# klausondrag/FOSVOS

Measured on AMD Instinct MI355X. Metric: online fine-tune frames/sec (854x480), higher is better.
Workload: dtype bf16; 1 GPU; OSVOS_VGG train_online one-shot fine-tune: 1x3x480x854 frame per step, fwd + class-balanced BCE + bwd, fused SGD step every 5 steps (BASELINE.json configs[1]); batch=1, avg_grad_every_n=5, activations=bf16 NHWC, fp32 accumulate, fp32 master weights, parallelism=single GPU

## Files before the change

fosvos_amd/csrc/common.hpp:

```cpp
#pragma once
#include <hip/hip_runtime.h>
#include <stdarg.h>
#include <algorithm>
#include <stdint.h>
#include <stdio.h>
#include <stdlib.h>
#include <string.h>

#include "../../include/fosvos_hip.h"

namespace fosvos {

extern thread_local char g_err[512];

inline int fail(int code, const char *fmt, ...) __attribute__((format(printf, 2, 3)));
inline int fail(int code, const char *fmt, ...) {
    va_list ap;
    va_start(ap, fmt);
    vsnprintf(g_err, sizeof(g_err), fmt, ap);
    va_end(ap);
    return code;
}

#define FOSVOS_HIP_CHECK(expr)                                                                         \
    do {                                                                                               \
        hipError_t e_ = (expr);                                                                        \
        if (e_ != hipSuccess)                                                                          \
            return ::fosvos::fail(FOSVOS_E_HIP, "%s: %s (%s:%d)", #expr, hipGetErrorString(e_), __FILE__, \
                                  __LINE__);                                                           \
    } while (0)

#define FOSVOS_REQUIRE(cond, code, ...)                    \
    do {                                                   \
        if (!(cond)) return ::fosvos::fail(code, __VA_ARGS__); \
    } while (0)

#define FOSVOS_ENTER(device) FOSVOS_HIP_CHECK(hipSetDevice(device))
extern bool g_prof_on;
void prof_begin(const char *name, hipStream_t st, double flops);
void prof_end();
#define FOSVOS_PROF(name, st, flops)                                        \
    do {                                                                    \
        if (::fosvos::g_prof_on) ::fosvos::prof_begin(name, (hipStream_t)(st), flops); \
    } while (0)
#define FOSVOS_LAUNCH_CHECK()                            \
    do {                                                 \
        if (::fosvos::g_prof_on) ::fosvos::prof_end();   \
        FOSVOS_HIP_CHECK(hipGetLastError());             \
    } while (0)

struct WgradReduceEntry {
    const float *slabs;
    float *dw, *db;
    const float *bias_part;
    int64_t E_real, E_pad;
    int S, S_bias, Co, Cor, accumulate;
    int block_begin, n_blocks;
    int fold_begin, fold_blocks;
};
constexpr int kWgradReduceMax = 20;
struct WgradReduceTable {
    int n;
    WgradReduceEntry e[kWgradReduceMax];
};
int wgrad_impl(const uint16_t *x, const uint16_t *dy, float *dw, float *db, int N, int H, int W, int Ci, int Co,
               int accumulate, void *workspace, size_t workspace_bytes, int device, void *stream,
               WgradReduceTable *reduce, bool alone = false);
int first_wgrad_impl(const float *frame, const uint16_t *dy, float *dw, float *db, int N, int H, int W, int Co,
                     int accumulate, void *workspace, size_t workspace_bytes, int device, void *stream,
                     WgradReduceTable *reduce);
int wgrad_reduce_all(WgradReduceTable *reduce, int device, void *stream);
int wgrad_queue_reduce(const float *slabs, const float *bias_part, float *dw, float *db, int S, int S_bias, int64_t E_real,
                       int64_t E_pad, int Co, int Cor, int accumulate, WgradReduceTable *reduce, int device, void *stream);
struct HeadBwdArgs {
    const float *const *side;
    const int *hs, *ws;
    const float *const *filt, *const *filt1;
    const float *dsn_w, *fuse_w, *d_fused;
    const float *const *d_side_out;
    uint16_t *const *d_side;
    float *d_fuse_w, *d_fuse_b, *d_dsn_w, *d_dsn_b;
    int N, H, W, accumulate;
    void *workspace;
    size_t workspace_bytes;
    int device;
    int filt_uniform;
};
int head_bwd_check(const HeadBwdArgs &a);
int head_bwd_scale(const HeadBwdArgs &a, int s, void *stream);
int head_bwd_finish(const HeadBwdArgs &a, void *stream);

}
constexpr int kFosvosVggEvents = 25, kFosvosResnetEvents = 12;
struct fosvos_ctx {
    uint32_t magic;
    int device;
    hipEvent_t vgg_ev[kFosvosVggEvents];
    hipEvent_t resnet_ev[kFosvosResnetEvents];
    bool buckets_recorded;
};
constexpr uint32_t kFosvosCtxMagic = 0x58544346u;
namespace fosvos {
inline int ctx_check(const fosvos_ctx *ctx, const char *who) {
    FOSVOS_REQUIRE(ctx != nullptr, FOSVOS_E_ARG, "%s: null context (fosvos_ctx_create)", who);
    FOSVOS_REQUIRE(ctx->magic == kFosvosCtxMagic, FOSVOS_E_ARG, "%s: not a live fosvos_ctx", who);
    return FOSVOS_OK;
}

#ifdef FOSVOS_LAB_BUILD
inline const char *lab_env(const char *name) { return getenv(name); }
#else
inline const char *lab_env(const char *) { return nullptr; }
#endif
inline int lab_env_int(const char *name, int dflt) {
    const char *e = lab_env(name);
    return e ? atoi(e) : dflt;
}

bool conv_pp_applicable(int N, int H, int W, int in_ch, int out_ch);
int conv_pp_workgroups();
int conv_pp_forward(const uint16_t *x, const uint16_t *w_packed, const float *bias, uint16_t *y, uint16_t *y_pool, int N,
                    int H, int W, int Cin_pad, int Cout, int Co_pad, bool relu, hipStream_t st,
                    const uint8_t *mask_bits = nullptr);

inline int64_t cdiv(int64_t a, int64_t b) { return (a + b - 1) / b; }
inline int roundup(int a, int b) { return (a + b - 1) / b * b; }

typedef uint16_t bf16_t;
typedef __attribute__((ext_vector_type(8))) __bf16 bf16x8;
typedef __attribute__((ext_vector_type(4))) float f32x4;
typedef __attribute__((ext_vector_type(4))) short s16x4;
typedef unsigned int u32x4 __attribute__((__vector_size__(16)));

__device__ __forceinline__ uint16_t f2bf(float f) {
    __bf16 b = (__bf16)f;
    return __builtin_bit_cast(uint16_t, b);
}
__device__ __forceinline__ float bf2f(uint16_t v) { return __uint_as_float(((uint32_t)v) << 16); }
__device__ __forceinline__ uint4 repack8(const float (&f)[8]) {
    uint4 v;
    v.x = __builtin_amdgcn_perm(__float_as_uint(f[1]), __float_as_uint(f[0]), 0x07060302u);
    v.y = __builtin_amdgcn_perm(__float_as_uint(f[3]), __float_as_uint(f[2]), 0x07060302u);
    v.z = __builtin_amdgcn_perm(__float_as_uint(f[5]), __float_as_uint(f[4]), 0x07060302u);
    v.w = __builtin_amdgcn_perm(__float_as_uint(f[7]), __float_as_uint(f[6]), 0x07060302u);
    return v;
}
typedef float fosvos_f32x2 __attribute__((ext_vector_type(2)));
typedef __bf16 fosvos_bf16x2 __attribute__((ext_vector_type(2)));
__device__ __forceinline__ uint32_t pack2bf(float lo, float hi) {
    const fosvos_f32x2 v = {lo, hi};
    return __builtin_bit_cast(uint32_t, __builtin_convertvector(v, fosvos_bf16x2));
}
__device__ __forceinline__ float relu_f(float v) { return __int_as_float(max(__float_as_int(v), 0)); }
__device__ __forceinline__ void unpack8(const uint4 &v, float (&f)[8]) {
    f[0] = __uint_as_float(v.x << 16);
    f[1] = __uint_as_float(v.x & 0xffff0000u);
    f[2] = __uint_as_float(v.y << 16);
    f[3] = __uint_as_float(v.y & 0xffff0000u);
    f[4] = __uint_as_float(v.z << 16);
    f[5] = __uint_as_float(v.z & 0xffff0000u);
    f[6] = __uint_as_float(v.w << 16);
    f[7] = __uint_as_float(v.w & 0xffff0000u);
}
__device__ __forceinline__ uint4 pack8(const float (&f)[8]) {
    uint4 v;
    v.x = pack2bf(f[0], f[1]);
    v.y = pack2bf(f[2], f[3]);
    v.z = pack2bf(f[4], f[5]);
    v.w = pack2bf(f[6], f[7]);
    return v;
}

typedef short fosvos_i16x2 __attribute__((ext_vector_type(2)));
typedef unsigned short fosvos_u16x2 __attribute__((ext_vector_type(2)));
__device__ __forceinline__ uint32_t keep_where_pos_bf16x2(uint32_t f, uint32_t m) {
    const fosvos_i16x2 zero = {0, 0}, one = {1, 1};
    const fosvos_i16x2 t = __builtin_elementwise_min(
        __builtin_elementwise_max(__builtin_bit_cast(fosvos_i16x2, m), zero), one);
    const fosvos_u16x2 all = {0xffff, 0xffff};
    return f & __builtin_bit_cast(uint32_t, __builtin_bit_cast(fosvos_u16x2, t) * all);
}
__device__ __forceinline__ uint4 keep_where_pos_bf16x8(const uint4 &f, const uint4 &m) {
    return make_uint4(keep_where_pos_bf16x2(f.x, m.x), keep_where_pos_bf16x2(f.y, m.y),
                      keep_where_pos_bf16x2(f.z, m.z), keep_where_pos_bf16x2(f.w, m.w));
}
__device__ __forceinline__ uint32_t max_nonneg_bf16x2(uint32_t a, uint32_t b) {
    return __builtin_bit_cast(uint32_t, __builtin_elementwise_max(__builtin_bit_cast(fosvos_u16x2, a),
                                                                 __builtin_bit_cast(fosvos_u16x2, b)));
}
__device__ __forceinline__ uint4 max_nonneg_bf16x8(const uint4 &a, const uint4 &b) {
    return make_uint4(max_nonneg_bf16x2(a.x, b.x), max_nonneg_bf16x2(a.y, b.y), max_nonneg_bf16x2(a.z, b.z),
                      max_nonneg_bf16x2(a.w, b.w));
}

__device__ __forceinline__ float wave_sum(float v) {
#pragma unroll
    for (int o = 32; o > 0; o >>= 1) v += __shfl_xor(v, o, 64);
    return v;
}
__device__ __forceinline__ double wave_sum(double v) {
#pragma unroll
    for (int o = 32; o > 0; o >>= 1) v += __shfl_xor(v, o, 64);
    return v;
}

}
```

fosvos_amd/csrc/conv_igemm.hip:

```cpp
#include <stdlib.h>

#include "common.hpp"

using namespace fosvos;

namespace {

constexpr unsigned kReluAfterAdd = 0x100u;
constexpr unsigned kSubsample2 = 0x200u;
constexpr unsigned kNoSplitK = 0x400u;

struct ConvArgs {
    const uint16_t *x;
    const uint16_t *w;
    const float *bias;
    const uint16_t *relu_src;
    const uint8_t *relu_bits;
    const uint16_t *addend;
    void *y;
    uint16_t *y_pool;
    const uint16_t *unpool_g;
    int N, H, W, Cin, Cout, Co_pad;
    int tiles_x, tiles_y;
    unsigned flags;
    int swizzle;
    int k_splits;
    int chunks_per_split;
    float *partial;
    unsigned m_ncb, m_nt, m_tx, m_ty;
    int n_t;
#ifdef FOSVOS_STAMP
    unsigned long long *stamps;
#endif
};

#ifdef FOSVOS_STAMP
unsigned long long *g_stamps = nullptr;
#define FOSVOS_STAMP_AT(i)                                                                               \
    if (a.stamps && threadIdx.x == 0)                                                                    \
        a.stamps[((((int64_t)blockIdx.z * gridDim.y + blockIdx.y) * gridDim.x + blockIdx.x) << 4) + (i)] = \
            __builtin_amdgcn_s_memtime();
#define FOSVOS_STAMP_RT(i)                                                                               \
    if (a.stamps && threadIdx.x == 0)                                                                    \
        a.stamps[((((int64_t)blockIdx.z * gridDim.y + blockIdx.y) * gridDim.x + blockIdx.x) << 4) + (i)] = \
            __builtin_amdgcn_s_memrealtime();
#else
#define FOSVOS_STAMP_AT(i)
#define FOSVOS_STAMP_RT(i)
#endif

__device__ __forceinline__ unsigned fast_div(unsigned n, unsigned d, unsigned m) { return m ? __umulhi(n, m) : n / d; }
unsigned recip_mul(int64_t n_max, int64_t d) {
    return (d >= 2 && n_max * d < (int64_t(1) << 32)) ? (unsigned)((int64_t(1) << 32) / d + 1) : 0u;
}

template <int TH_, int TW_, int BN_, int WM_, int WN_>
struct Tile {
    static constexpr int TH = TH_, TW = TW_, BN = BN_, WM = WM_, WN = WN_;
    static constexpr int BM = TH * TW;
    static constexpr int HALO_W = TW + 2, HALO_H = TH + 2;
    static constexpr int NPIX = HALO_W * HALO_H;
    static constexpr int NPIX8 = (NPIX + 7) / 8 * 8;
    static constexpr int NPIX_PAD = (NPIX + 15) / 16 * 16;
    static constexpr int WAVE_M = BM / WM, WAVE_N = BN / WN;
    static constexpr int MF = WAVE_M / 16, NF = WAVE_N / 16;
    static constexpr int A_SLOTS = 4 * NPIX_PAD;
    static constexpr int B_SLOTS = 36 * BN;
    static constexpr int NT = 64 * WM * WN;
    static constexpr int A_IT = (NPIX8 * 4 + NT - 1) / NT;
    static constexpr int B_IT = (B_SLOTS + NT - 1) / NT;
    static constexpr int OUT_LD = BN + 8;
    static constexpr int LDS_MAIN = (A_SLOTS + B_SLOTS) * 16;
    static constexpr int LDS_OUT = BM * OUT_LD * 2;
    static constexpr int LDS_BYTES = LDS_MAIN > LDS_OUT ? LDS_MAIN : LDS_OUT;
#ifndef FOSVOS_MID_WPE
#define FOSVOS_MID_WPE 3
#endif
    static constexpr int WPE = (BM >= 256 || BN < 64) ? 2 : FOSVOS_MID_WPE;
    static_assert(WM * WN == 4 || WM * WN == 8, "4 or 8 waves per workgroup");
    static_assert(TW % 16 == 0 && WAVE_M % 16 == 0 && WAVE_N % 16 == 0, "fragment alignment");
    static_assert(BM % WM == 0 && BN % WN == 0, "wave split");
};

template <int MF, int NF>
struct TapPlan {
    static constexpr int rows_b = MF / 2 > 0 ? MF / 2 : 1;
    static constexpr int per_row = (NF + rows_b - 1) / rows_b;
    static constexpr int nb(int i) {
        const int left = NF - i * per_row;
        return left <= 0 ? 0 : (left < per_row ? left : per_row);
    }
};
template <int MF, int NF, int I, bool NEXT, int V>
__device__ __forceinline__ void sched_row() {
    if constexpr (I < MF) {
        __builtin_amdgcn_sched_group_barrier(0x008, NF, 0);
        if constexpr (NEXT) __builtin_amdgcn_sched_group_barrier(0x100, 1 + TapPlan<MF, NF>::nb(I), 0);
        constexpr int rows_v = V < MF ? V : MF;
        constexpr int nv = I < MF - rows_v ? 0 : (I == MF - 1 ? V - (rows_v - 1) : 1);
        if constexpr (nv > 0) __builtin_amdgcn_sched_group_barrier(0x020, nv, 0);
    }
}
template <int MF, int NF, bool NEXT, int V>
__device__ __forceinline__ void sched_tap() {
    static_assert(MF <= 8, "sched_tap rows");
    sched_row<MF, NF, 0, NEXT, V>(); sched_row<MF, NF, 1, NEXT, V>(); sched_row<MF, NF, 2, NEXT, V>();
    sched_row<MF, NF, 3, NEXT, V>(); sched_row<MF, NF, 4, NEXT, V>(); sched_row<MF, NF, 5, NEXT, V>();
    sched_row<MF, NF, 6, NEXT, V>(); sched_row<MF, NF, 7, NEXT, V>();
}

template <class T, bool OUT_F32, bool UNPOOL = false>
__global__ __launch_bounds__(T::NT) __attribute__((amdgpu_waves_per_eu(2, T::WPE))) void k_conv3x3_igemm(const ConvArgs a) {
    extern __shared__ __attribute__((aligned(16))) uint4 smem[];
    uint4 *sA = smem;
    uint4 *sB = smem + T::A_SLOTS;
#ifdef FOSVOS_IGEMM_PRIO
    __builtin_amdgcn_s_setprio(FOSVOS_IGEMM_PRIO);
#endif

    const int tid = threadIdx.x, lane = tid & 63;
    const int wave = __builtin_amdgcn_readfirstlane(tid >> 6);
    const int wm = wave / T::WN, wn = wave % T::WN;
    int t = blockIdx.x;
    int cb = blockIdx.y;
    if (a.swizzle) {
        const int n_wg = gridDim.x, n_cb = a.Cout / T::BN, n_t = a.n_t;
        const int q8 = n_wg >> 3, r8 = n_wg & 7, xcd = t & 7;
        const int swz = (xcd < r8 ? xcd * (q8 + 1) : r8 * (q8 + 1) + (xcd - r8) * q8) + (t >> 3);
        if (a.swizzle == 1) { t = fast_div(swz, n_cb, a.m_ncb); cb = swz - t * n_cb; }
        else { cb = fast_div(swz, n_t, a.m_nt); t = swz - cb * n_t; }
    }
    const int t_row = fast_div(t, a.tiles_x, a.m_tx);
    const int tx_i = t - t_row * a.tiles_x;
    const int n = fast_div(t_row, a.tiles_y, a.m_ty);
    const int ty_i = t_row - n * a.tiles_y;
    const int y0 = ty_i * T::TH, x0 = tx_i * T::TW;
    const int n0 = cb * T::BN;
    const int H = a.H, W = a.W, Cin = a.Cin;
    const int n_chunks = Cin >> 5;
    const uint16_t *xn = a.x + (int64_t)n * H * W * Cin;

    int a_goff[T::A_IT];
    int a_slot[T::A_IT];
#pragma unroll
    for (int it = 0; it < T::A_IT; ++it) {
        const int idx = it * T::NT + tid;
        const int oct = idx >> 5, within = idx & 31;
        const int kg = within >> 3;
        const int P = oct * 8 + (within & 7);
        a_slot[it] = -1;
        a_goff[it] = -1;
        if (P < T::NPIX) {
            const int hy = P / T::HALO_W, hx = P - hy * T::HALO_W;
            const int gy = y0 + hy - 1, gx = x0 + hx - 1;
            a_slot[it] = kg * T::NPIX_PAD + P;
            if (gy >= 0 && gy < H && gx >= 0 && gx < W) a_goff[it] = ((gy * W + gx) * Cin + kg * 8) * 2;
        }
    }

    f32x4 acc[T::MF][T::NF];
#pragma unroll
    for (int i = 0; i < T::MF; ++i)
#pragma unroll
        for (int j = 0; j < T::NF; ++j) acc[i][j] = f32x4{0.f, 0.f, 0.f, 0.f};

    int a_base[T::MF];
#pragma unroll
    for (int i = 0; i < T::MF; ++i) {
        const int pb = wm * T::WAVE_M + i * 16;
        const int ty = pb / T::TW, tx = pb % T::TW;
        a_base[i] = (lane >> 4) * T::NPIX_PAD + ty * T::HALO_W + tx + (lane & 15);
    }
// ... 138 lines not shown
        return;
    }
    constexpr int VEC_PER_PIX = T::BN / 8;
    constexpr int OUT_N = T::BM * VEC_PER_PIX;
    constexpr int OUT_IT = (OUT_N + T::NT - 1) / T::NT;
    constexpr int PIX_STEP = T::NT / VEC_PER_PIX;
    static_assert(T::NT % VEC_PER_PIX == 0 && PIX_STEP % T::TW == 0, "a thread's output vectors must share a column");
    constexpr int ROW_STEP = PIX_STEP / T::TW;
    const int o_cg = tid % VEC_PER_PIX, o_pix = tid / VEC_PER_PIX;
    const int o_ly = o_pix / T::TW, o_gx = x0 + o_pix % T::TW;
    const int img_bytes = H * W * a.Cout * 2;
    uint16_t *yo = reinterpret_cast<uint16_t *>(a.y);
    int voff[OUT_IT];
#pragma unroll
    for (int it = 0; it < OUT_IT; ++it) {
        const int gy = y0 + o_ly + it * ROW_STEP;
        const bool ok = it * T::NT + tid < OUT_N && gy < H && o_gx < W;
        voff[it] = ok ? ((gy * W + o_gx) * a.Cout + n0 + o_cg * 8) * 2 : -1;
    }
    const bool masked = (a.relu_src || a.relu_bits || a.addend) && !(a.flags & kSubsample2);
    uint4 mk[OUT_IT], ad[OUT_IT];
#pragma unroll
    for (int it = 0; it < OUT_IT; ++it) mk[it] = ad[it] = make_uint4(0, 0, 0, 0);
    if constexpr (UNPOOL) {
        const int OH = (H + 1) >> 1, OW = (W + 1) >> 1;
        auto m_rsrc = __builtin_amdgcn_make_buffer_rsrc(const_cast<uint16_t *>(a.relu_src + (int64_t)n * H * W * a.Cout), 0,
                                                        img_bytes, 0x00020000);
        auto g_rsrc = __builtin_amdgcn_make_buffer_rsrc(const_cast<uint16_t *>(a.unpool_g + (int64_t)n * OH * OW * a.Cout), 0,
                                                        OH * OW * a.Cout * 2, 0x00020000);
#pragma unroll
        for (int it = 0; it < OUT_IT; ++it)
            mk[it] = __builtin_bit_cast(uint4, __builtin_amdgcn_raw_buffer_load_b128(m_rsrc, voff[it], 0, 0));
#pragma unroll
        for (int it = 0; it < OUT_IT; ++it) {
            const int gy = y0 + o_ly + it * ROW_STEP;
            const int goff = voff[it] < 0 ? -1 : (((gy >> 1) * OW + (o_gx >> 1)) * a.Cout + n0 + o_cg * 8) * 2;
            ad[it] = __builtin_bit_cast(uint4, __builtin_amdgcn_raw_buffer_load_b128(g_rsrc, goff, 0, 0));
        }
    } else if (masked && a.relu_bits) {
        auto b_rsrc = __builtin_amdgcn_make_buffer_rsrc(const_cast<uint8_t *>(a.relu_bits + (int64_t)n * H * W * (a.Cout >> 3)), 0,
                                                        img_bytes >> 4, 0x00020000);
#pragma unroll
        for (int it = 0; it < OUT_IT; ++it) {
            const unsigned b = __builtin_amdgcn_raw_buffer_load_b8(b_rsrc, voff[it] < 0 ? -1 : voff[it] >> 4, 0, 0);
            mk[it] = make_uint4((b & 1u) | ((b & 2u) << 15), ((b >> 2) & 1u) | ((b & 8u) << 13), ((b >> 4) & 1u) | ((b & 32u) << 11),
                                ((b >> 6) & 1u) | ((b & 128u) << 9));
        }
        if (a.addend) {
            auto ad_rsrc = __builtin_amdgcn_make_buffer_rsrc(const_cast<uint16_t *>(a.addend + (int64_t)n * H * W * a.Cout), 0,
                                                             img_bytes, 0x00020000);
#pragma unroll
            for (int it = 0; it < OUT_IT; ++it)
                ad[it] = __builtin_bit_cast(uint4, __builtin_amdgcn_raw_buffer_load_b128(ad_rsrc, voff[it], 0, 0));
        }
    } else if (masked) {
        auto m_rsrc = __builtin_amdgcn_make_buffer_rsrc(
            const_cast<uint16_t *>(a.relu_src ? a.relu_src + (int64_t)n * H * W * a.Cout : yo), 0,
            a.relu_src ? img_bytes : 0, 0x00020000);
        auto ad_rsrc = __builtin_amdgcn_make_buffer_rsrc(
            const_cast<uint16_t *>(a.addend ? a.addend + (int64_t)n * H * W * a.Cout : yo), 0,
            a.addend ? img_bytes : 0, 0x00020000);
#pragma unroll
        for (int it = 0; it < OUT_IT; ++it)
            mk[it] = __builtin_bit_cast(uint4, __builtin_amdgcn_raw_buffer_load_b128(m_rsrc, voff[it], 0, 0));
#pragma unroll
        for (int it = 0; it < OUT_IT; ++it)
            ad[it] = __builtin_bit_cast(uint4, __builtin_amdgcn_raw_buffer_load_b128(ad_rsrc, voff[it], 0, 0));
    }
    float4 bias_r[T::NF];
#pragma unroll
    for (int j = 0; j < T::NF; ++j)
        bias_r[j] = a.bias ? *reinterpret_cast<const float4 *>(a.bias + n0 + wn * T::WAVE_N + j * 16 + q * 4)
                           : make_float4(0.f, 0.f, 0.f, 0.f);
    __syncthreads();
    uint16_t *sO = reinterpret_cast<uint16_t *>(smem);
#pragma unroll
    for (int j = 0; j < T::NF; ++j) {
        const int col = wn * T::WAVE_N + j * 16 + q * 4;
        const float4 b = bias_r[j];
#pragma unroll
        for (int i = 0; i < T::MF; ++i) {
            const int pix = wm * T::WAVE_M + i * 16 + cl;
            float v0 = acc[i][j][0] + b.x, v1 = acc[i][j][1] + b.y, v2 = acc[i][j][2] + b.z, v3 = acc[i][j][3] + b.w;
            if (a.flags & FOSVOS_CONV_RELU) {
                v0 = relu_f(v0); v1 = relu_f(v1); v2 = relu_f(v2); v3 = relu_f(v3);
            }
            *reinterpret_cast<uint2 *>(sO + pix * T::OUT_LD + col) = make_uint2(pack2bf(v0, v1), pack2bf(v2, v3));
        }
    }
    if constexpr (UNPOOL) {
        uint16_t *sX = sO + T::BM * T::OUT_LD;
#pragma unroll
        for (int it = 0; it < OUT_IT; ++it)
            if (it * T::NT + tid < OUT_N)
                *reinterpret_cast<uint4 *>(sX + (o_pix + it * PIX_STEP) * T::OUT_LD + o_cg * 8) = mk[it];
    }
    __syncthreads();
    FOSVOS_STAMP_AT(9)
    const uint16_t *s_vec = sO + o_pix * T::OUT_LD + o_cg * 8;
    auto y_rsrc = __builtin_amdgcn_make_buffer_rsrc(yo + (int64_t)n * H * W * a.Cout, 0, img_bytes, 0x00020000);
    if constexpr (UNPOOL) {
        static_assert((T::TW & (T::TW - 1)) == 0 && T::TH % 2 == 0, "window partners are pix ^ 1 and pix ^ TW");
        const uint16_t *sX = sO + T::BM * T::OUT_LD;
        const fosvos_i16x2 one2 = {1, 1}, zero2 = {0, 0};
        const fosvos_i16x2 late_x = (o_pix & 1) ? zero2 : one2;
#pragma unroll
        for (int it = 0; it < OUT_IT; ++it) {
            const int pix = o_pix + it * PIX_STEP;
            if (it * T::NT + tid >= OUT_N) continue;
            const fosvos_i16x2 late_y = (pix & T::TW) ? zero2 : one2;
            const uint4 cv = keep_where_pos_bf16x8(*reinterpret_cast<const uint4 *>(s_vec + it * PIX_STEP * T::OUT_LD), mk[it]);
            const uint4 x1 = *reinterpret_cast<const uint4 *>(sX + (pix ^ 1) * T::OUT_LD + o_cg * 8);
            const uint4 x2 = *reinterpret_cast<const uint4 *>(sX + (pix ^ T::TW) * T::OUT_LD + o_cg * 8);
            const uint4 x3 = *reinterpret_cast<const uint4 *>(sX + (pix ^ T::TW ^ 1) * T::OUT_LD + o_cg * 8);
            auto win = [&](unsigned own_, unsigned p1, unsigned p2, unsigned p3) {
                const fosvos_i16x2 own = __builtin_bit_cast(fosvos_i16x2, own_);
                const fosvos_i16x2 s = (zero2 - own) & (__builtin_bit_cast(fosvos_i16x2, p1) - own - late_x) &
                                       (__builtin_bit_cast(fosvos_i16x2, p2) - own - late_y) &
                                       (__builtin_bit_cast(fosvos_i16x2, p3) - own - late_y);
                return __builtin_bit_cast(unsigned, s >> 15);
            };
            const uint4 routed = make_uint4(ad[it].x & win(mk[it].x, x1.x, x2.x, x3.x), ad[it].y & win(mk[it].y, x1.y, x2.y, x3.y),
                                            ad[it].z & win(mk[it].z, x1.z, x2.z, x3.z), ad[it].w & win(mk[it].w, x1.w, x2.w, x3.w));
            float f[8], r[8];
            unpack8(cv, f);
            unpack8(routed, r);
#pragma unroll
            for (int e = 0; e < 8; ++e) f[e] += r[e];
            __builtin_amdgcn_raw_buffer_store_b128(__builtin_bit_cast(u32x4, pack8(f)), y_rsrc, voff[it], 0, 0);
        }
    } else if (!(a.flags & kSubsample2)) {
        if (masked) {
#pragma unroll
            for (int it = 0; it < OUT_IT; ++it) {
                uint4 v = *reinterpret_cast<const uint4 *>(s_vec + it * PIX_STEP * T::OUT_LD);
                if (a.relu_src || a.relu_bits) v = keep_where_pos_bf16x8(v, mk[it]);
                if (a.addend || (a.flags & kReluAfterAdd)) {
                    float f[8];
                    unpack8(v, f);
                    if (a.addend) {
                        float av[8];
                        unpack8(ad[it], av);
#pragma unroll
                        for (int e = 0; e < 8; ++e) f[e] += av[e];
                    }
                    if (a.flags & kReluAfterAdd) {
#pragma unroll
                        for (int e = 0; e < 8; ++e) f[e] = relu_f(f[e]);
                    }
                    v = pack8(f);
                }
                __builtin_amdgcn_raw_buffer_store_b128(__builtin_bit_cast(u32x4, v), y_rsrc, voff[it], 0, 0);
            }
        } else {
#pragma unroll
            for (int it = 0; it < OUT_IT; ++it)
                __builtin_amdgcn_raw_buffer_store_b128(
                    __builtin_bit_cast(u32x4, *reinterpret_cast<const uint4 *>(s_vec + it * PIX_STEP * T::OUT_LD)), y_rsrc,
                    voff[it], 0, 0);
        }
    } else {
#pragma unroll
        for (int it = 0; it < OUT_IT; ++it) {
            const int gy = y0 + o_ly + it * ROW_STEP;
            if (it * T::NT + tid >= OUT_N || gy >= H || o_gx >= W || ((gy | o_gx) & 1)) continue;
            const int64_t off =
                (((int64_t)n * ((H + 1) >> 1) + (gy >> 1)) * ((W + 1) >> 1) + (o_gx >> 1)) * a.Cout + n0 + o_cg * 8;
            *reinterpret_cast<uint4 *>(yo + off) = *reinterpret_cast<const uint4 *>(s_vec + it * PIX_STEP * T::OUT_LD);
        }
    }
    if (a.y_pool) {
        static_assert(T::TH % 2 == 0 && T::TW % 2 == 0, "pooling windows must not straddle tiles");
        constexpr int PW = T::TW / 2, PN = (T::TH / 2) * PW;
        const int OH = (H + 1) >> 1, OW = (W + 1) >> 1;
        auto p_rsrc = __builtin_amdgcn_make_buffer_rsrc(a.y_pool + (int64_t)n * OH * OW * a.Cout, 0, OH * OW * a.Cout * 2,
                                                        0x00020000);
        for (int idx = tid; idx < PN * VEC_PER_PIX; idx += T::NT) {
            const int pp = idx / VEC_PER_PIX, cg = idx % VEC_PER_PIX;
            const int py = pp / PW, px = pp % PW;
            const int oy = (y0 >> 1) + py, ox = (x0 >> 1) + px;
            if (oy >= OH || ox >= OW) continue;
            const int poff = ((oy * OW + ox) * a.Cout + n0 + cg * 8) * 2;
            if (a.flags & FOSVOS_CONV_RELU) {
                uint4 mx = make_uint4(0, 0, 0, 0);
#pragma unroll
                for (int t = 0; t < 4; ++t) {
                    const int ly = 2 * py + (t >> 1), lx = 2 * px + (t & 1);
                    if (y0 + ly < H && x0 + lx < W)
                        mx = max_nonneg_bf16x8(mx, *reinterpret_cast<const uint4 *>(sO + (ly * T::TW + lx) * T::OUT_LD + cg * 8));
                }
                __builtin_amdgcn_raw_buffer_store_b128(__builtin_bit_cast(u32x4, mx), p_rsrc, poff, 0, 0);
                continue;
            }
            float m[8];
#pragma unroll
            for (int j = 0; j < 8; ++j) m[j] = -INFINITY;
#pragma unroll
            for (int t = 0; t < 4; ++t) {
                const int ly = 2 * py + (t >> 1), lx = 2 * px + (t & 1);
                if (y0 + ly < H && x0 + lx < W) {
                    float f[8];
                    unpack8(*reinterpret_cast<const uint4 *>(sO + (ly * T::TW + lx) * T::OUT_LD + cg * 8), f);
#pragma unroll
                    for (int j = 0; j < 8; ++j) m[j] = f[j] > m[j] ? f[j] : m[j];
                }
            }
            __builtin_amdgcn_raw_buffer_store_b128(__builtin_bit_cast(u32x4, pack8(m)), p_rsrc, poff, 0, 0);
        }
    }
    FOSVOS_STAMP_AT(10)
    FOSVOS_STAMP_RT(12)
}

__global__ __launch_bounds__(256) void k_splitk_epilogue(const ConvArgs a, int64_t total8) {
    const int groups = a.Cout >> 3;
    const int64_t plane = (int64_t)a.N * a.H * a.W * a.Cout;
    for (int64_t i = blockIdx.x * 256LL + threadIdx.x; i < total8; i += (int64_t)gridDim.x * 256) {
        const int g = (int)(i % groups);
        int64_t off = i * 8;
        if (a.flags & kSubsample2) {
            const int Ho = (a.H + 1) >> 1, Wo = (a.W + 1) >> 1;
            int64_t pq = i / groups;
            const int ox = (int)(pq % Wo);
            pq /= Wo;
            const int oy = (int)(pq % Ho), n = (int)(pq / Ho);
            off = (((int64_t)n * a.H + 2 * oy) * a.W + 2 * ox) * a.Cout + g * 8;
        }
        float f[8];
#pragma unroll
        for (int e = 0; e < 8; ++e) f[e] = 0.f;
        for (int z0 = 0; z0 < a.k_splits; z0 += 4) {
            float4 v0[4], v1[4];
#pragma unroll
            for (int j = 0; j < 4; ++j) {
                const int z = min(z0 + j, a.k_splits - 1);
                v0[j] = *reinterpret_cast<const float4 *>(a.partial + z * plane + off);
                v1[j] = *reinterpret_cast<const float4 *>(a.partial + z * plane + off + 4);
            }
#pragma unroll
            for (int j = 0; j < 4; ++j) {
                if (z0 + j < a.k_splits) {
                    f[0] += v0[j].x; f[1] += v0[j].y; f[2] += v0[j].z; f[3] += v0[j].w;
                    f[4] += v1[j].x; f[5] += v1[j].y; f[6] += v1[j].z; f[7] += v1[j].w;
                }
            }
        }
        if (a.bias) {
#pragma unroll
            for (int e = 0; e < 8; ++e) f[e] += a.bias[g * 8 + e];
        }
        if (a.flags & FOSVOS_CONV_RELU) {
#pragma unroll
            for (int e = 0; e < 8; ++e) f[e] = relu_f(f[e]);
        }
        if (a.flags & FOSVOS_CONV_OUT_F32) {
            float *yo = reinterpret_cast<float *>(a.y) + off;
            *reinterpret_cast<float4 *>(yo) = make_float4(f[0], f[1], f[2], f[3]);
            *reinterpret_cast<float4 *>(yo + 4) = make_float4(f[4], f[5], f[6], f[7]);
            continue;
        }
        if (a.relu_src || a.relu_bits || a.addend) {
            uint4 v = pack8(f);
            unpack8(v, f);
            if (a.relu_bits) {
                const unsigned b = a.relu_bits[off >> 3];
#pragma unroll
                for (int e = 0; e < 8; ++e) f[e] = ((b >> e) & 1u) ? f[e] : 0.f;
            }
            if (a.relu_src) {
                float m[8];
                unpack8(*reinterpret_cast<const uint4 *>(a.relu_src + off), m);
#pragma unroll
                for (int e = 0; e < 8; ++e) f[e] = m[e] > 0.f ? f[e] : 0.f;
            }
            if (a.addend) {
                float ad[8];
                unpack8(*reinterpret_cast<const uint4 *>(a.addend + off), ad);
#pragma unroll
                for (int e = 0; e < 8; ++e) f[e] += ad[e];
            }
            if (a.flags & kReluAfterAdd) {
#pragma unroll
                for (int e = 0; e < 8; ++e) f[e] = relu_f(f[e]);
            }
        }
        *reinterpret_cast<uint4 *>(reinterpret_cast<uint16_t *>(a.y) + i * 8) = pack8(f);
    }
}

using TileBig = Tile<8, 32, 64, 4, 1>;
using TileSquare = Tile<16, 16, 64, 4, 1>;
using TileMid = Tile<8, 16, 64, 2, 2>;
using TileSmall = Tile<4, 16, 64, 2, 2>;
using TileSide = Tile<8, 32, 16, 4, 1>;
using TileSideS = Tile<4, 16, 16, 4, 1>;
using TileHalf = Tile<8, 32, 32, 4, 1>;
using TileHalfS = Tile<4, 16, 32, 4, 1>;

enum TileId { kBig, kMid, kSmall, kSide, kSideS, kHalf, kHalfS, kSquare };

struct ConvPlan {
    TileId tile;
    int k_splits, chunks_per_split;
    size_t workspace_bytes;
};

constexpr int kMinBlocks = 512;

ConvPlan make_plan(int N, int H, int W, int in_ch, int out_ch) {
    ConvPlan p{};
    const int n_chunks = roundup(in_ch, 32) / 32;
    const int64_t pixels = (int64_t)N * H * W;
    auto blocks = [&](int th, int tw, int bn) { return cdiv(W, tw) * cdiv(H, th) * N * (int64_t)(out_ch / bn); };
    int64_t nb;
    if (out_ch % 64 == 0) {
        bool big = blocks(8, 32, 64) >= kMinBlocks / 2;
        if (big) {
            const int64_t area_wide = cdiv(H, 8) * 8 * cdiv(W, 32) * 32, area_sq = cdiv(H, 16) * 16 * cdiv(W, 16) * 16;
            static const bool allow_sq = lab_env_int("FOSVOS_NO_SQUARE_TILE", 0) == 0;
            if (allow_sq && area_sq < area_wide) { p.tile = kSquare; nb = blocks(16, 16, 64); }
            else { p.tile = kBig; nb = blocks(8, 32, 64); }
            static const bool one_round = lab_env_int("FOSVOS_MID_ONE_ROUND", 0) != 0;
            if (blocks(8, 16, 64) <= 768 && (one_round ? blocks(8, 32, 64) < kMinBlocks * 3 / 4 : nb < kMinBlocks / 2)) big = false;
        }
        if (!big) { p.tile = kMid; nb = blocks(8, 16, 64); }
    } else if (out_ch == 32) {
        if (pixels >= 256 * 256) { p.tile = kHalf; nb = blocks(8, 32, 32); }
        else { p.tile = kHalfS; nb = blocks(4, 16, 32); }
    } else {
        if (pixels >= 256 * 256) { p.tile = kSide; nb = blocks(8, 32, 16); }
        else { p.tile = kSideS; nb = blocks(4, 16, 16); }
    }
    if (out_ch % 64 == 0) {
        static const char *force = lab_env("FOSVOS_FORCE_TILE");
        if (force && ((atoi(force) >= 0 && atoi(force) <= 2) || atoi(force) == (int)kHalf)) {
            p.tile = (TileId)atoi(force);
            nb = p.tile == kBig ? blocks(8, 32, 64) : p.tile == kMid ? blocks(8, 16, 64)
                 : p.tile == kHalf ? blocks(8, 32, 32) : blocks(4, 16, 64);
        }
    }
    int ks = 1;
    if (nb < kMinBlocks * 3 / 4) {
        ks = (int)cdiv(kMinBlocks / 2, nb);
        if (ks < 2) ks = 1;
        if (ks > n_chunks) ks = n_chunks;
        if (ks > 16) ks = 16;
    }
#ifdef FOSVOS_STAMP
    if (const char *e = lab_env("FOSVOS_FORCE_KS")) ks = atoi(e);
#endif
    p.chunks_per_split = (int)cdiv(n_chunks, ks);
    p.k_splits = (int)cdiv(n_chunks, p.chunks_per_split);
    p.workspace_bytes = p.k_splits > 1 ? (size_t)p.k_splits * pixels * out_ch * sizeof(float) : 0;
    return p;
}

template <class T, bool OUT_F32, bool UNPOOL = false>
int launch(const ConvArgs &a0, const ConvPlan &plan, hipStream_t st, int in_ch) {
    constexpr int LDS = UNPOOL && 2 * T::LDS_OUT > T::LDS_MAIN ? 2 * T::LDS_OUT : T::LDS_BYTES;
    ConvArgs a = a0;
    a.tiles_x = (int)cdiv(a.W, T::TW);
    a.tiles_y = (int)cdiv(a.H, T::TH);
    a.k_splits = plan.k_splits;
    a.chunks_per_split = plan.chunks_per_split;
#ifdef FOSVOS_STAMP
    a.stamps = g_stamps;
#endif
    const int64_t tiles = (int64_t)a.tiles_x * a.tiles_y * a.N;
    FOSVOS_REQUIRE(tiles <= 0x7fffffff && a.Cout % T::BN == 0, FOSVOS_E_SHAPE, "conv3x3: tile grid");
    if constexpr (LDS > 64 * 1024) {
        static bool once[64];
        int dev = 0;
        FOSVOS_HIP_CHECK(hipGetDevice(&dev));
        if (dev >= 0 && dev < 64 && !once[dev]) {
            FOSVOS_HIP_CHECK(hipFuncSetAttribute(reinterpret_cast<const void *>(k_conv3x3_igemm<T, OUT_F32, UNPOOL>),
                                                 hipFuncAttributeMaxDynamicSharedMemorySize, LDS));
            once[dev] = true;
        }
    }
    if (g_prof_on) {
        static char name[80];
        snprintf(name, sizeof(name), "k_conv3x3_igemm<Tile<%d, %d, %d, %d, %d>, %s, %s>", T::TH, T::TW, T::BN, T::WM, T::WN,
                 OUT_F32 ? "true" : "false", UNPOOL ? "true" : "false");
        prof_begin(name, st, 2.0 * a.N * a.H * a.W * 9.0 * in_ch * a.Cout);
    }
    {
        static const int swz_env = lab_env_int("FOSVOS_IGEMM_SWIZZLE", -1);
        const int n_cb = a.Cout / T::BN;
        a.swizzle = swz_env >= 0 ? swz_env : (tiles * n_cb >= 64 ? 1 : 0);
        if (tiles * n_cb > 0x7fffffff) a.swizzle = 0;
    }
    {
        const int64_t n_cb = a.Cout / T::BN, n_wg = tiles * n_cb;
        a.n_t = (int)tiles;
        a.m_ncb = recip_mul(n_wg, n_cb);
        a.m_nt = recip_mul(n_wg, tiles);
        a.m_tx = recip_mul(tiles, a.tiles_x);
        a.m_ty = recip_mul(tiles, a.tiles_y);
    }
    const dim3 grid = a.swizzle ? dim3((unsigned)(tiles * (a.Cout / T::BN)), 1u, (unsigned)plan.k_splits)
                                : dim3((unsigned)tiles, (unsigned)(a.Cout / T::BN), (unsigned)plan.k_splits);
    hipLaunchKernelGGL((k_conv3x3_igemm<T, OUT_F32, UNPOOL>), grid, dim3(T::NT), LDS, st, a);
    FOSVOS_LAUNCH_CHECK();
    if (plan.k_splits > 1) {
        const int64_t total8 = (a.flags & kSubsample2) ? (int64_t)a.N * ((a.H + 1) >> 1) * ((a.W + 1) >> 1) * (a.Cout / 8)
                                                       : (int64_t)a.N * a.H * a.W * (a.Cout / 8);
        int64_t g = cdiv(total8, 256);
        if (g > 4096) g = 4096;
        FOSVOS_PROF("k_splitk_epilogue", st, 0.0);
        hipLaunchKernelGGL(k_splitk_epilogue, dim3((unsigned)g), dim3(256), 0, st, a, total8);
        FOSVOS_LAUNCH_CHECK();
    }
    return FOSVOS_OK;
}

int dispatch(ConvArgs a, int in_ch, void *workspace, size_t workspace_bytes, hipStream_t st) {
    const bool f32 = (a.flags & FOSVOS_CONV_OUT_F32) != 0;
    if (a.Cout == 32) {
        FOSVOS_REQUIRE(!f32, FOSVOS_E_ARG, "conv3x3: fp32 output is only built for 16-channel outputs");
    } else if (a.Cout % 64 != 0) {
        FOSVOS_REQUIRE(a.Cout == 16, FOSVOS_E_SHAPE, "conv3x3: output channels must be 16, 32 or a multiple of 64 (got %d)",
                       a.Cout);
        FOSVOS_REQUIRE(a.relu_src == nullptr && a.addend == nullptr, FOSVOS_E_ARG,
                       "conv3x3: 16-channel output has no mask/add epilogue");
    } else {
        FOSVOS_REQUIRE(!f32, FOSVOS_E_ARG, "conv3x3: fp32 output is only built for 16-channel outputs");
    }
    ConvPlan plan = make_plan(a.N, a.H, a.W, in_ch, a.Cout);
    if (a.flags & kNoSplitK) {
        plan.k_splits = 1;
        plan.chunks_per_split = roundup(in_ch, 32) / 32;
        plan.workspace_bytes = 0;
    }
    if (plan.k_splits > 1) {
        FOSVOS_REQUIRE(workspace && workspace_bytes >= plan.workspace_bytes, FOSVOS_E_WORKSPACE,
                       "conv3x3: split-K needs %zu workspace bytes, got %zu", plan.workspace_bytes, workspace_bytes);
        a.partial = reinterpret_cast<float *>(workspace);
    }
    if (a.unpool_g) {
        switch (plan.tile) {
            case kBig: return launch<TileBig, false, true>(a, plan, st, in_ch);
            case kSquare: return launch<TileSquare, false, true>(a, plan, st, in_ch);
            case kMid: return launch<TileMid, false, true>(a, plan, st, in_ch);
            default: return fail(FOSVOS_E_ARG, "conv3x3: no fused pool backward for this tile");
        }
    }
    switch (plan.tile) {
        case kBig: return launch<TileBig, false>(a, plan, st, in_ch);
        case kSquare: return launch<TileSquare, false>(a, plan, st, in_ch);
        case kMid: return launch<TileMid, false>(a, plan, st, in_ch);
        case kSmall: return launch<TileSmall, false>(a, plan, st, in_ch);
        case kSide: return f32 ? launch<TileSide, true>(a, plan, st, in_ch) : launch<TileSide, false>(a, plan, st, in_ch);
        case kSideS: return f32 ? launch<TileSideS, true>(a, plan, st, in_ch) : launch<TileSideS, false>(a, plan, st, in_ch);
        case kHalf: return launch<TileHalf, false>(a, plan, st, in_ch);
        case kHalfS: return launch<TileHalfS, false>(a, plan, st, in_ch);
    }
    return fail(FOSVOS_E_ARG, "conv3x3: bad plan");
}

bool forward_takes_pp(int N, int H, int W, int in_ch, int out_ch, unsigned flags) {
    if (flags & ~FOSVOS_CONV_RELU) return false;
    static const int mode = lab_env_int("FOSVOS_PP", -1);
    if (mode == 0) return false;
    return conv_pp_applicable(N, H, W, roundup(in_ch, 32), out_ch);
}

int check_common(const void *x, const void *w, const void *y, int N, int H, int W, int in_ch, int out_ch,
                 const char *who) {
    FOSVOS_REQUIRE(x && w && y, FOSVOS_E_ARG, "%s: null pointer", who);
    FOSVOS_REQUIRE(N > 0 && H > 0 && W > 0 && in_ch > 0 && out_ch > 0, FOSVOS_E_SHAPE, "%s: bad shape N=%d H=%d W=%d in=%d out=%d",
                   who, N, H, W, in_ch, out_ch);
    FOSVOS_REQUIRE(out_ch % 16 == 0, FOSVOS_E_SHAPE, "%s: output channels %d not a multiple of 16", who, out_ch);
    FOSVOS_REQUIRE((int64_t)H * W * roundup(in_ch, 32) * 2 < 0x7fffffffLL && (int64_t)H * W * out_ch * 4 < 0x7fffffffLL,
                   FOSVOS_E_SHAPE, "%s: one image exceeds 2^31 bytes", who);
    return FOSVOS_OK;
}
}

extern "C" size_t fosvos_conv3x3_workspace_bytes(int N, int H, int W, int in_ch, int out_ch) {
    if (N <= 0 || H <= 0 || W <= 0 || in_ch <= 0 || out_ch <= 0 || (out_ch % 64 != 0 && out_ch != 16)) return 0;
    return make_plan(N, H, W, in_ch, out_ch).workspace_bytes;
}

extern "C" int fosvos_conv3x3_plan(int N, int H, int W, int in_ch, int out_ch, fosvos_conv3x3_plan_info *out) {
    FOSVOS_REQUIRE(out, FOSVOS_E_ARG, "conv3x3_plan: null output");
    FOSVOS_REQUIRE(N > 0 && H > 0 && W > 0 && in_ch > 0 && out_ch > 0 && (out_ch % 64 == 0 || out_ch == 32 || out_ch == 16),
                   FOSVOS_E_SHAPE, "conv3x3_plan: bad shape N=%d H=%d W=%d in=%d out=%d", N, H, W, in_ch, out_ch);
    const ConvPlan p = make_plan(N, H, W, in_ch, out_ch);
    int th = 0, tw = 0, bn = 0;
    switch (p.tile) {
        case kBig: th = TileBig::TH; tw = TileBig::TW; bn = TileBig::BN; break;
        case kSquare: th = TileSquare::TH; tw = TileSquare::TW; bn = TileSquare::BN; break;
        case kMid: th = TileMid::TH; tw = TileMid::TW; bn = TileMid::BN; break;
        case kSmall: th = TileSmall::TH; tw = TileSmall::TW; bn = TileSmall::BN; break;
        case kSide: th = TileSide::TH; tw = TileSide::TW; bn = TileSide::BN; break;
        case kSideS: th = TileSideS::TH; tw = TileSideS::TW; bn = TileSideS::BN; break;
        case kHalf: th = TileHalf::TH; tw = TileHalf::TW; bn = TileHalf::BN; break;
        case kHalfS: th = TileHalfS::TH; tw = TileHalfS::TW; bn = TileHalfS::BN; break;
    }
    out->tile_h = th; out->tile_w = tw; out->tile_co = bn;
    out->k_splits = p.k_splits;
    out->workgroups = (int)(cdiv(W, tw) * cdiv(H, th) * N * (out_ch / bn));
    out->persistent = 0;
    return FOSVOS_OK;
}

extern "C" int fosvos_conv3x3_fwd_plan(int N, int H, int W, int in_ch, int out_ch, unsigned flags,
                                       fosvos_conv3x3_plan_info *out) {
    if (int rc = fosvos_conv3x3_plan(N, H, W, in_ch, out_ch, out)) return rc;
    if (out_ch % 64 == 0 && forward_takes_pp(N, H, W, in_ch, out_ch, flags)) {
        out->tile_h = 8; out->tile_w = 32; out->tile_co = 64;
        out->k_splits = 1;
        out->workgroups = conv_pp_workgroups();
        out->persistent = 1;
    }
    return FOSVOS_OK;
}

extern "C" int fosvos_conv3x3_fwd(const uint16_t *x, const uint16_t *w_packed, const float *bias, void *y, int N, int H,
                                  int W, int Ci, int Co, unsigned flags, void *workspace, size_t workspace_bytes,
                                  int device, void *stream) {
    if (int rc = check_common(x, w_packed, y, N, H, W, Ci, Co, "conv3x3_fwd")) return rc;
    FOSVOS_REQUIRE((flags & ~(FOSVOS_CONV_RELU | FOSVOS_CONV_OUT_F32)) == 0, FOSVOS_E_ARG, "conv3x3_fwd: unknown flags 0x%x", flags);
    FOSVOS_ENTER(device);
    if (Co % 64 == 0 && forward_takes_pp(N, H, W, Ci, Co, flags))
        return conv_pp_forward(x, w_packed, bias, (uint16_t *)y, nullptr, N, H, W, roundup(Ci, 32), Co, roundup(Co, 16),
                               (flags & FOSVOS_CONV_RELU) != 0, (hipStream_t)stream);
    ConvArgs a{};
    a.x = x; a.w = w_packed; a.bias = bias; a.relu_src = nullptr; a.addend = nullptr; a.y = y;
    a.N = N; a.H = H; a.W = W; a.Cin = roundup(Ci, 32); a.Cout = Co; a.Co_pad = roundup(Co, 16); a.flags = flags;
    return dispatch(a, Ci, workspace, workspace_bytes, (hipStream_t)stream);
}

extern "C" int fosvos_conv3x3_fwd_add(const uint16_t *x, const uint16_t *w_packed, const float *bias,
                                      const uint16_t *addend, void *y, int N, int H, int W, int Ci, int Co,
                                      unsigned flags, void *workspace, size_t workspace_bytes, int device,
                                      void *stream) {
    if (int rc = check_common(x, w_packed, y, N, H, W, Ci, Co, "conv3x3_fwd_add")) return rc;
    FOSVOS_REQUIRE((flags & ~(FOSVOS_CONV_RELU | FOSVOS_CONV_OUT_F32)) == 0, FOSVOS_E_ARG, "conv3x3_fwd_add: unknown flags 0x%x",
                   flags);
    FOSVOS_REQUIRE(Co % 64 == 0 || Co == 32 || (Co == 16 && !addend), FOSVOS_E_SHAPE,
                   "conv3x3_fwd_add: Co=%d must be 32 or a multiple of 64 (16 without an addend)", Co);
    FOSVOS_REQUIRE(!(flags & FOSVOS_CONV_OUT_F32) || (Co == 16 && !addend), FOSVOS_E_ARG,
                   "conv3x3_fwd_add: fp32 output is the 16-channel side_prep form");
    FOSVOS_ENTER(device);
    ConvArgs a{};
    a.x = x; a.w = w_packed; a.bias = bias; a.relu_src = nullptr; a.addend = addend; a.y = y;
    a.N = N; a.H = H; a.W = W; a.Cin = roundup(Ci, 32); a.Cout = Co; a.Co_pad = roundup(Co, 16);
    a.flags = kNoSplitK | (addend ? ((flags & FOSVOS_CONV_RELU) ? kReluAfterAdd : 0u) : flags);
    return dispatch(a, Ci, workspace, workspace_bytes, (hipStream_t)stream);
}

extern "C" int fosvos_conv3x3_s2_fwd(const uint16_t *x, const uint16_t *w_packed, const float *bias, uint16_t *y, int N,
                                     int H, int W, int Ci, int Co, unsigned flags, void *workspace, size_t workspace_bytes,
                                     int device, void *stream) {
    if (int rc = check_common(x, w_packed, y, N, H, W, Ci, Co, "conv3x3_s2_fwd")) return rc;
    FOSVOS_REQUIRE((flags & ~FOSVOS_CONV_RELU) == 0, FOSVOS_E_ARG, "conv3x3_s2_fwd: unknown flags 0x%x", flags);
    FOSVOS_REQUIRE(Co % 64 == 0 || Co == 32, FOSVOS_E_SHAPE, "conv3x3_s2_fwd: Co=%d must be 32 or a multiple of 64", Co);
    FOSVOS_ENTER(device);
    ConvArgs a{};
    a.x = x; a.w = w_packed; a.bias = bias; a.relu_src = nullptr; a.addend = nullptr; a.y = y;
    a.N = N; a.H = H; a.W = W; a.Cin = roundup(Ci, 32); a.Cout = Co; a.Co_pad = roundup(Co, 16);
    a.flags = flags | kSubsample2 | kNoSplitK;
    return dispatch(a, Ci, workspace, workspace_bytes, (hipStream_t)stream);
}

extern "C" int fosvos_conv3x3_fwd_pool(const uint16_t *x, const uint16_t *w_packed, const float *bias, uint16_t *y,
                                       uint16_t *y_pool, int N, int H, int W, int Ci, int Co, unsigned flags,
                                       void *workspace, size_t workspace_bytes, int device, void *stream) {
    if (int rc = check_common(x, w_packed, y, N, H, W, Ci, Co, "conv3x3_fwd_pool")) return rc;
    FOSVOS_REQUIRE(y_pool, FOSVOS_E_ARG, "conv3x3_fwd_pool: null pooled output");
    FOSVOS_REQUIRE((flags & ~FOSVOS_CONV_RELU) == 0, FOSVOS_E_ARG, "conv3x3_fwd_pool: unknown flags 0x%x", flags);
    FOSVOS_REQUIRE(Co % 64 == 0, FOSVOS_E_SHAPE, "conv3x3_fwd_pool: Co=%d must be a multiple of 64", Co);
    if ((flags & FOSVOS_CONV_RELU) && forward_takes_pp(N, H, W, Ci, Co, flags)) {
        FOSVOS_ENTER(device);
        return conv_pp_forward(x, w_packed, bias, y, y_pool, N, H, W, roundup(Ci, 32), Co, roundup(Co, 16), true,
                               (hipStream_t)stream);
    }
    if (make_plan(N, H, W, Ci, Co).k_splits > 1) {
        if (int rc = fosvos_conv3x3_fwd(x, w_packed, bias, y, N, H, W, Ci, Co, flags, workspace, workspace_bytes, device, stream))
            return rc;
        return fosvos_maxpool2x2_ceil_fwd(y, y_pool, N, H, W, Co, device, stream);
    }
    FOSVOS_ENTER(device);
    ConvArgs a{};
    a.x = x; a.w = w_packed; a.bias = bias; a.relu_src = nullptr; a.addend = nullptr; a.y = y; a.y_pool = y_pool;
    a.N = N; a.H = H; a.W = W; a.Cin = roundup(Ci, 32); a.Cout = Co; a.Co_pad = roundup(Co, 16); a.flags = flags;
    return dispatch(a, Ci, workspace, workspace_bytes, (hipStream_t)stream);
}

extern "C" int fosvos_conv3x3_dgrad_bits(const uint16_t *dy, const uint16_t *w_dgrad_packed, const uint8_t *relu_bits,
                                         const uint16_t *addend, uint16_t *dx, int N, int H, int W, int Ci, int Co,
                                         void *workspace, size_t workspace_bytes, int device, void *stream) {
    if (int rc = check_common(dy, w_dgrad_packed, dx, N, H, W, Co, Ci, "conv3x3_dgrad_bits")) return rc;
    FOSVOS_REQUIRE(relu_bits && Ci % 8 == 0, FOSVOS_E_ARG, "conv3x3_dgrad_bits: null mask or Ci=%d not a multiple of 8", Ci);
    FOSVOS_ENTER(device);
    if (!addend && lab_env_int("FOSVOS_PP_DGRAD", 1) != 0 && lab_env_int("FOSVOS_PP", -1) != 0 &&
        conv_pp_applicable(N, H, W, roundup(Co, 32), Ci))
        return conv_pp_forward(dy, w_dgrad_packed, nullptr, dx, nullptr, N, H, W, roundup(Co, 32), Ci, roundup(Ci, 16), false,
                               (hipStream_t)stream, relu_bits);
    ConvArgs a{};
    a.x = dy; a.w = w_dgrad_packed; a.bias = nullptr; a.relu_src = nullptr; a.relu_bits = relu_bits; a.addend = addend; a.y = dx;
    a.N = N; a.H = H; a.W = W; a.Cin = roundup(Co, 32); a.Cout = Ci; a.Co_pad = roundup(Ci, 16); a.flags = 0;
    return dispatch(a, Co, workspace, workspace_bytes, (hipStream_t)stream);
}

extern "C" int fosvos_conv3x3_dgrad_unpool(const uint16_t *dy, const uint16_t *w_dgrad_packed, const uint16_t *x,
                                           const uint16_t *d_pooled, uint16_t *dx, int N, int H, int W, int Ci, int Co,
                                           void *workspace, size_t workspace_bytes, int device, void *stream) {
    if (int rc = check_common(dy, w_dgrad_packed, dx, N, H, W, Co, Ci, "conv3x3_dgrad_unpool")) return rc;
    FOSVOS_REQUIRE(x && d_pooled && x != dx, FOSVOS_E_ARG, "conv3x3_dgrad_unpool: null or aliased pooled-map operands");
    FOSVOS_ENTER(device);
    const ConvPlan plan = make_plan(N, H, W, Co, Ci);
    const bool fused = Ci % 64 == 0 && plan.k_splits == 1 && (plan.tile == kBig || plan.tile == kSquare || plan.tile == kMid) &&
                       lab_env_int("FOSVOS_UNPOOL_FUSED", 1) != 0;
    if (!fused) {
        if (int rc = fosvos_maxpool2x2_ceil_bwd(x, d_pooled, dx, N, H, W, Ci, 1, device, stream)) return rc;
        return fosvos_conv3x3_dgrad(dy, w_dgrad_packed, x, dx, dx, N, H, W, Ci, Co, workspace, workspace_bytes, device, stream);
    }
    ConvArgs a{};
    a.x = dy; a.w = w_dgrad_packed; a.relu_src = x; a.unpool_g = d_pooled; a.y = dx;
    a.N = N; a.H = H; a.W = W; a.Cin = roundup(Co, 32); a.Cout = Ci; a.Co_pad = roundup(Ci, 16); a.flags = 0;
    return dispatch(a, Co, workspace, workspace_bytes, (hipStream_t)stream);
}

extern "C" int fosvos_conv3x3_dgrad(const uint16_t *dy, const uint16_t *w_dgrad_packed, const uint16_t *relu_src,
                                    const uint16_t *addend, uint16_t *dx, int N, int H, int W, int Ci, int Co,
                                    void *workspace, size_t workspace_bytes, int device, void *stream) {
    if (int rc = check_common(dy, w_dgrad_packed, dx, N, H, W, Co, Ci, "conv3x3_dgrad")) return rc;
    FOSVOS_ENTER(device);
    ConvArgs a{};
    a.x = dy; a.w = w_dgrad_packed; a.bias = nullptr; a.relu_src = relu_src; a.addend = addend; a.y = dx;
    a.N = N; a.H = H; a.W = W; a.Cin = roundup(Co, 32); a.Cout = Ci; a.Co_pad = roundup(Ci, 16); a.flags = 0;
    return dispatch(a, Co, workspace, workspace_bytes, (hipStream_t)stream);
}
```

fosvos_amd/csrc/conv_pp.hip:

```cpp
#include <stdlib.h>

#include "common.hpp"

using namespace fosvos;

namespace fosvos {
namespace pp {

constexpr int TH = 8, TW = 32, BN = 64;
constexpr int HALO_W = TW + 2, HALO_H = TH + 2, NPIX = HALO_W * HALO_H;
constexpr int A_BYTES = NPIX * 64;
constexpr int A_PIECES = (NPIX * 4 + 63) / 64;
constexpr int W_BYTES = 36 * BN * 16;
constexpr int LDS_W = 0, LDS_A = 2 * W_BYTES, LDS_BIAS = LDS_A + 4 * A_BYTES, LDS_BYTES = LDS_BIAS + BN * 4;
constexpr int NT = 512;
static_assert(LDS_BYTES <= 160 * 1024, "one workgroup per CU");

struct Args {
    const uint16_t *x;
    const uint16_t *w;
    const float *bias;
    uint16_t *y;
    uint16_t *y_pool;
    const uint8_t *mask_bits;
    int N, H, W, Cin, Cout, Co_pad;
    int tiles_x, tiles_y, n_tiles;
    int n_cb;
    unsigned long long *stamps;
    int lab;
};
#ifdef FOSVOS_LAB_BUILD
#define PP_LAB(bit) (a.lab & (bit))
#define PP_STAMP(idx_)                                                                                            \
    if (a.stamps && blockIdx.x < 8 && wm == 0 && lane == 0 && (idx_) < 512)                                       \
        a.stamps[(blockIdx.x * 2 + g) * 512 + (idx_)] = __builtin_amdgcn_s_memtime();
#else
#define PP_LAB(bit) 0
#define PP_STAMP(idx_)
#endif

#pragma clang diagnostic push
#pragma clang diagnostic ignored "-Winline-asm"
__device__ __forceinline__ void dma16(const __amdgpu_buffer_rsrc_t rsrc, unsigned lds_dst, unsigned voff, unsigned soff) {
    asm volatile("s_mov_b32 m0, %0\n\ts_nop 4\n\tbuffer_load_dwordx4 %1, %2, %3 offen lds"
                 :: "s"(lds_dst), "v"(voff), "s"(rsrc), "s"(soff) : "memory", "m0");
}
__device__ __forceinline__ void wait_vm0() { asm volatile("s_waitcnt vmcnt(0)" ::: "memory"); }
__device__ __forceinline__ void wait_all() { asm volatile("s_waitcnt vmcnt(0) lgkmcnt(0)" ::: "memory"); }
__device__ __forceinline__ void pp_barrier() {
    asm volatile("" ::: "memory");
    __builtin_amdgcn_s_barrier();
    asm volatile("" ::: "memory");
}
#pragma clang diagnostic pop

typedef __attribute__((address_space(3))) void lds_void;
typedef __attribute__((address_space(3))) const uint4 *lds_u4_ptr;

struct TileIt {
    int idx, n, ty, tx;
    int d_n, d_ty, d_tx, stride;
    int tiles_x, tiles_y, end;
    __device__ __forceinline__ void init(int first, int stride_, int tiles_x_, int tiles_y_, int end_) {
        tiles_x = tiles_x_; tiles_y = tiles_y_; end = end_; stride = stride_;
        idx = first;
        const int per_img = tiles_x * tiles_y;
        n = first / per_img;
        const int r = first - n * per_img;
        ty = r / tiles_x;
        tx = r - ty * tiles_x;
        d_n = stride / per_img;
        const int rs = stride - d_n * per_img;
        d_ty = rs / tiles_x;
        d_tx = rs - d_ty * tiles_x;
    }
    __device__ __forceinline__ void next() {
        idx += stride;
        tx += d_tx;
        const int cx = tx >= tiles_x;
        tx -= cx ? tiles_x : 0;
        ty += d_ty + cx;
        const int cy = ty >= tiles_y;
        ty -= cy ? tiles_y : 0;
        n += d_n + cy;
    }
    __device__ __forceinline__ bool valid() const { return idx < end; }
    __device__ __forceinline__ int y0() const { return ty * TH; }
    __device__ __forceinline__ int x0() const { return tx * TW; }
};

template <bool RELU, bool POOL, bool MASK = false>
__global__ __launch_bounds__(NT) __attribute__((amdgpu_waves_per_eu(2, 2))) void k_conv3x3_pp(const Args a) {
    extern __shared__ __attribute__((aligned(16))) char smem_pp[];
    const unsigned lds0 = __builtin_amdgcn_readfirstlane((unsigned)(size_t)(lds_void *)smem_pp);
    const int tid = threadIdx.x, lane = tid & 63;
    const int wave = __builtin_amdgcn_readfirstlane(tid >> 6);
    const int g = wave >> 2, wm = wave & 3;
    const int cl = lane & 15, kq = lane >> 4;
    const int H = a.H, W = a.W, Cin = a.Cin, Cout = a.Cout;
    const int NC = Cin >> 5;

    const int b = blockIdx.x, n_wg8 = gridDim.x >> 3;
    const int xcd = b & 7, j8 = b >> 3;
    const int cb = j8 % a.n_cb, jj = j8 / a.n_cb, S = n_wg8 / a.n_cb;
    const int t_begin = (int)(((int64_t)xcd * a.n_tiles) >> 3), t_end = (int)(((int64_t)(xcd + 1) * a.n_tiles) >> 3);
    const int span = t_end - t_begin;
    const int n_it = span > 2 * jj ? (span - 2 * jj + 2 * S - 1) / (2 * S) : 0;
    if (n_it == 0) return;
    const int K = n_it * NC;
    const int n0 = cb * BN;
    TileIt cur, ldt;
    cur.init(t_begin + 2 * jj + g, 2 * S, a.tiles_x, a.tiles_y, t_end);
    ldt = cur;

    const int pj = lane >> 4, pm = lane & 15;
    const unsigned w_voff = (unsigned)(32 * (pj >> 1) + 8 * (pm >> 2) + 4 * (pj & 1) + (pm & 3)) * 16u;
    const int w_row_bytes = a.Co_pad * 16;
    const auto w_rsrc = __builtin_amdgcn_make_buffer_rsrc(const_cast<uint16_t *>(a.w), 0, NC * 36 * w_row_bytes, 0x00020000);
    auto issue_w = [&](int chunk, int buf, int first, int stride) {
        if (PP_LAB(8)) return;
        for (int r = first; r < 36; r += stride)
            dma16(w_rsrc, lds0 + LDS_W + buf * W_BYTES + r * 1024, w_voff, (unsigned)((chunk * 36 + r) * w_row_bytes + n0 * 16));
    };

    constexpr int A_IT = (A_PIECES + 3) / 4;
    int a_rel[A_IT];
#pragma unroll
    for (int i = 0; i < A_IT; ++i) {
        const int pc = wm + 4 * i;
        const int P = pc * 16 + (lane >> 2), s4 = lane & 3;
        const int hy = P / HALO_W, hx = P - hy * HALO_W;
        const int kq_src = s4 ^ ((P >> 1) & 2);
        a_rel[i] = (hy * W + hx) * Cin * 2 + kq_src * 16;
    }
    int ld_k = 0, ld_c = 0;
    int ld_base = 0, ld_edge = 0;
    __amdgpu_buffer_rsrc_t ld_rsrc;
    auto ld_open_tile = [&]() {
        if (!ldt.valid()) return;
        const int y0 = ldt.y0(), x0 = ldt.x0();
        ld_rsrc = __builtin_amdgcn_make_buffer_rsrc(const_cast<uint16_t *>(a.x) + (int64_t)ldt.n * H * W * Cin, 0,
                                                    H * W * Cin * 2, 0x00020000);
        ld_base = ((y0 - 1) * W + (x0 - 1)) * Cin * 2;
        ld_edge = !(y0 > 0 && x0 > 0 && y0 + TH < H && x0 + TW < W);
    };
    auto ld_issue = [&]() {
        if (ld_k < K && ldt.valid() && !PP_LAB(4)) {
            const unsigned dst = lds0 + LDS_A + (g * 2 + (ld_k & 1)) * A_BYTES;
            constexpr int LAST_LANES = NPIX * 4 - (A_PIECES - 1) * 64;
            if (!ld_edge) {
                const unsigned soff = (unsigned)(ld_base + ld_c * 64);
#pragma unroll
                for (int i = 0; i < A_IT; ++i) {
                    const int pc = wm + 4 * i;
                    if (pc < A_PIECES - 1) dma16(ld_rsrc, dst + pc * 1024, (unsigned)a_rel[i], soff);
                    else if (pc == A_PIECES - 1 && lane < LAST_LANES) dma16(ld_rsrc, dst + pc * 1024, (unsigned)a_rel[i], soff);
                }
            } else {
                const int y0 = ldt.y0(), x0 = ldt.x0();
#pragma unroll
                for (int i = 0; i < A_IT; ++i) {
                    const int pc = wm + 4 * i;
                    const int P = pc * 16 + (lane >> 2);
                    const int hy = P / HALO_W, hx = P - hy * HALO_W;
                    const int gy = y0 + hy - 1, gx = x0 + hx - 1;
                    const bool ok = (unsigned)gy < (unsigned)H && (unsigned)gx < (unsigned)W;
                    const unsigned voff = ok ? (unsigned)(ld_base + a_rel[i]) : 0x80000000u;
                    if (pc < A_PIECES - 1) dma16(ld_rsrc, dst + pc * 1024, voff, (unsigned)(ld_c * 64));
                    else if (pc == A_PIECES - 1 && lane < LAST_LANES) dma16(ld_rsrc, dst + pc * 1024, voff, (unsigned)(ld_c * 64));
                }
            }
        }
        ++ld_k;
        if (++ld_c == NC) {
            ld_c = 0;
            ldt.next();
            if (ld_k < K) ld_open_tile();
        }
    };

    unsigned a_sw[4][3];
#pragma unroll
    for (int rr = 0; rr < 4; ++rr)
#pragma unroll
        for (int kx = 0; kx < 3; ++kx) {
            const int P = (2 * wm + rr) * HALO_W + kx + cl;
            a_sw[rr][kx] = (unsigned)(P * 64 + ((kq ^ ((P >> 1) & 2)) << 4));
        }
    const unsigned w_frag0 = lds0 + LDS_W + kq * 1024 + cl * 16;

    if (tid < BN) *(__attribute__((address_space(3))) float *)(size_t)(lds0 + LDS_BIAS + tid * 4) = a.bias ? a.bias[n0 + tid] : 0.f;
    const unsigned bias_at = lds0 + LDS_BIAS + kq * 32;

    f32x4 acc[4][4];
    int cp_c = 0;
    bf16x8 af[4], wf[2][4];
#define PP_RA(k_, tap_, i_)                                                                                   \
    af[i_] = __builtin_bit_cast(bf16x8, *(lds_u4_ptr)(size_t)(lds0 + LDS_A + (g * 2 + ((k_) & 1)) * A_BYTES +  \
                                                              a_sw[((i_) >> 1) + (tap_) / 3][(tap_) % 3] + ((i_) & 1) * 1024));
#define PP_RW(k_, tap_, s_, j_) \
    wf[s_][j_] = __builtin_bit_cast(bf16x8, *(lds_u4_ptr)(size_t)(w_frag0 + ((k_) & 1) * W_BYTES + (tap_) * 4096 + (j_) * 256));
#define PP_RBIAS()                                                                                            \
    _Pragma("unroll") for (int i = 0; i < 4; ++i) _Pragma("unroll") for (int j = 0; j < 4; ++j) acc[i][j] =    \
        *(__attribute__((address_space(3))) const f32x4 *)(size_t)(bias_at + (j >> 1) * 128 + (j & 1) * 16);

    uint4 pk[4][2];
    unsigned mb[MASK ? 4 : 1][2];
    int dn_n = 0, dn_y0 = 0, dn_x0 = 0;
    int st_pending = 0;
    auto pack_frag = [&](int i, int jp) {
        unsigned u[4];
#pragma unroll
        for (int e2 = 0; e2 < 4; ++e2) {
            const int e = 2 * e2;
            u[e2] = pack2bf(acc[i][2 * jp + (e >> 2)][e & 3], acc[i][2 * jp + (e >> 2)][(e & 3) + 1]);
            if constexpr (RELU) {
                const fosvos_i16x2 zero = {0, 0};
                u[e2] = __builtin_bit_cast(unsigned, __builtin_elementwise_max(__builtin_bit_cast(fosvos_i16x2, u[e2]), zero));
            }
        }
        return make_uint4(u[0], u[1], u[2], u[3]);
    };
    auto pack_tile = [&]() {
        if (!cur.valid() || PP_LAB(2)) return;
        dn_n = cur.n; dn_y0 = cur.y0(); dn_x0 = cur.x0();
        st_pending = 1;
#pragma unroll
        for (int i = 0; i < 4; ++i) {
            pk[i][0] = pack_frag(i, 0);
            pk[i][1] = pack_frag(i, 1);
        }
        if constexpr (MASK) {
            const auto m_rsrc = __builtin_amdgcn_make_buffer_rsrc(const_cast<uint8_t *>(a.mask_bits) + (int64_t)dn_n * H * W * (Cout >> 3),
                                                                  0, H * W * (Cout >> 3), 0x00020000);
#pragma unroll
            for (int i = 0; i < 4; ++i) {
                const int gy = dn_y0 + 2 * wm + (i >> 1), gx = dn_x0 + (i & 1) * 16 + cl;
                const unsigned off = (gy < H && gx < W) ? (unsigned)((gy * W + gx) * (Cout >> 3) + (n0 >> 3) + kq) : 0x80000000u;
                mb[i][0] = __builtin_amdgcn_raw_buffer_load_b8(m_rsrc, off, 0, 0);
                mb[i][1] = __builtin_amdgcn_raw_buffer_load_b8(m_rsrc, off + 4, 0, 0);
            }
        }
    };
    auto mask_bits_of = [](unsigned b) {
        return make_uint4((b & 1u) | ((b & 2u) << 15), ((b >> 2) & 1u) | ((b & 8u) << 13), ((b >> 4) & 1u) | ((b & 32u) << 11),
                          ((b >> 6) & 1u) | ((b & 128u) << 9));
    };
    auto store_slot = [&](int slot) {
        if (!st_pending) return;
        if (slot < 4) {
            const auto y_rsrc = __builtin_amdgcn_make_buffer_rsrc(a.y + (int64_t)dn_n * H * W * Cout, 0, H * W * Cout * 2, 0x00020000);
            const int gy = dn_y0 + 2 * wm + (slot >> 1), gx = dn_x0 + (slot & 1) * 16 + cl;
            const unsigned off = (gy < H && gx < W) ? (unsigned)(((gy * W + gx) * Cout + n0 + kq * 8) * 2) : 0x80000000u;
            uint4 v0 = pk[slot][0], v1 = pk[slot][1];
            if constexpr (MASK) {
                v0 = keep_where_pos_bf16x8(v0, mask_bits_of(mb[slot][0]));
                v1 = keep_where_pos_bf16x8(v1, mask_bits_of(mb[slot][1]));
            }
            __builtin_amdgcn_raw_buffer_store_b128(__builtin_bit_cast(u32x4, v0), y_rsrc, off, 0, 0);
            __builtin_amdgcn_raw_buffer_store_b128(__builtin_bit_cast(u32x4, v1), y_rsrc, off + 64, 0, 0);
        } else if constexpr (POOL) {
            const int ih = slot - 4;
            const int OH = (H + 1) >> 1, OW = (W + 1) >> 1;
            const bool edge = dn_y0 + TH > H || dn_x0 + TW > W;
            const auto p_rsrc = __builtin_amdgcn_make_buffer_rsrc(a.y_pool + (int64_t)dn_n * OH * OW * Cout, 0,
                                                                  OH * OW * Cout * 2, 0x00020000);
            const int oy = (dn_y0 >> 1) + wm, ox = (dn_x0 >> 1) + ih * 8 + (cl >> 1);
            const bool ok = !(cl & 1) && oy < OH && ox < OW;
            const unsigned off = ok ? (unsigned)(((oy * OW + ox) * Cout + n0 + kq * 8) * 2) : 0x80000000u;
#pragma unroll
            for (int jp = 0; jp < 2; ++jp) {
                uint4 top = pk[ih][jp], bot = pk[ih + 2][jp];
                if (edge) {
                    const int gy = dn_y0 + 2 * wm, gx = dn_x0 + ih * 16 + cl;
                    if (!(gy < H && gx < W)) top = make_uint4(0, 0, 0, 0);
                    if (!(gy + 1 < H && gx < W)) bot = make_uint4(0, 0, 0, 0);
                }
                const uint4 m = max_nonneg_bf16x8(top, bot);
                uint4 o;
                o.x = (unsigned)__builtin_amdgcn_update_dpp(0, (int)m.x, 0xB1, 0xF, 0xF, true);
                o.y = (unsigned)__builtin_amdgcn_update_dpp(0, (int)m.y, 0xB1, 0xF, 0xF, true);
                o.z = (unsigned)__builtin_amdgcn_update_dpp(0, (int)m.z, 0xB1, 0xF, 0xF, true);
                o.w = (unsigned)__builtin_amdgcn_update_dpp(0, (int)m.w, 0xB1, 0xF, 0xF, true);
                __builtin_amdgcn_raw_buffer_store_b128(__builtin_bit_cast(u32x4, max_nonneg_bf16x8(m, o)), p_rsrc, off + jp * 64, 0, 0);
            }
        }
    };
    constexpr int N_SLOTS = POOL ? 6 : 4;

    auto request_next = [&](int k) {
        if (k + 1 < K && (NC > 2 || k + 1 < 2)) issue_w((k + 1) % NC, (k + 1) & 1, wave, 8);
        ld_issue();
    };

    issue_w(0, 0, wave, 8);
    ld_open_tile();
    ld_issue();
    wait_all();
    pp_barrier();

#define PP_MM(tap_, i_, j_) \
    acc[i_][j_] = __builtin_amdgcn_mfma_f32_16x16x32_bf16(wf[(tap_) & 1][j_], af[i_], acc[i_][j_], 0, 0, 0);
#define PP_ROW_READS(n_, i_)                                                                                  \
    PP_RA(k, n_, i_)                                                                                          \
    if constexpr ((i_) < 2) {                                                                                 \
        PP_RW(k, n_, (n_) & 1, 2 * (i_))                                                                      \
        PP_RW(k, n_, (n_) & 1, 2 * (i_) + 1)                                                                  \
    }                                                                                                         \
    __builtin_amdgcn_sched_group_barrier(0x008, 4, 0);                                                        \
    __builtin_amdgcn_sched_group_barrier(0x002, 1, 0);                                                        \
    __builtin_amdgcn_sched_group_barrier(0x100, (i_) < 2 ? 3 : 1, 0);
#define PP_ROW(tap_, i_)                                                                                      \
    PP_MM(tap_, i_, 0) PP_MM(tap_, i_, 1) PP_MM(tap_, i_, 2) PP_MM(tap_, i_, 3)                               \
    PP_ROW_READS((tap_) + 1, i_)
#define PP_TAP(tap_) { PP_ROW(tap_, 0) PP_ROW(tap_, 1) PP_ROW(tap_, 2) PP_ROW(tap_, 3) }
#define PP_TAP_LAST()                                                                                         \
    {                                                                                                         \
        _Pragma("unroll") for (int i = 0; i < 4; ++i) _Pragma("unroll") for (int j = 0; j < 4; ++j) acc[i][j] = \
            __builtin_amdgcn_mfma_f32_16x16x32_bf16(wf[0][j], af[i], acc[i][j], 0, 0, 0);                      \
        __builtin_amdgcn_sched_group_barrier(0x008, 16, 0);                                                   \
    }
#define PP_BETWEEN(tap_)                                                                                      \
    if (g == 0) {                                                                                             \
        if constexpr ((tap_) >= 3 && (tap_) - 3 < N_SLOTS) store_slot((tap_) - 3);                            \
    } else {                                                                                                  \
        if constexpr ((tap_) < 3) {                                                                           \
            store_slot(2 * (tap_));                                                                           \
            if constexpr (2 * (tap_) + 1 < N_SLOTS) store_slot(2 * (tap_) + 1);                               \
        }                                                                                                     \
        if constexpr ((tap_) == 4) request_next(k);                                                           \
    }

    for (int k = 0; k < K; ++k) {
        PP_STAMP(4 * k)
        if (g == 0) request_next(k);
        PP_STAMP(4 * k + 1)
        if (cur.valid() && !PP_LAB(1)) {
            if (cp_c == 0) { PP_RBIAS() }
            PP_RA(k, 0, 0) PP_RA(k, 0, 1) PP_RA(k, 0, 2) PP_RA(k, 0, 3)
            PP_RW(k, 0, 0, 0) PP_RW(k, 0, 0, 1) PP_RW(k, 0, 0, 2) PP_RW(k, 0, 0, 3)
            PP_TAP(0) PP_BETWEEN(0) PP_TAP(1) PP_BETWEEN(1) PP_TAP(2) PP_BETWEEN(2) PP_TAP(3) PP_BETWEEN(3) PP_TAP(4) PP_BETWEEN(4)
            PP_TAP(5) PP_BETWEEN(5) PP_TAP(6) PP_BETWEEN(6) PP_TAP(7) PP_BETWEEN(7) PP_TAP_LAST() PP_BETWEEN(8)
        } else {
            PP_BETWEEN(0) PP_BETWEEN(1) PP_BETWEEN(2) PP_BETWEEN(3) PP_BETWEEN(4) PP_BETWEEN(5) PP_BETWEEN(6) PP_BETWEEN(7) PP_BETWEEN(8)
        }
        st_pending = 0;
        if (++cp_c == NC) {
            cp_c = 0;
            pack_tile();
            cur.next();
        }
        PP_STAMP(4 * k + 2)
        wait_vm0();
        PP_STAMP(4 * k + 3)
        pp_barrier();
    }
    PP_STAMP(4 * K)
#pragma unroll
    for (int slot = 0; slot < N_SLOTS; ++slot) store_slot(slot);
#undef PP_MM
#undef PP_ROW_READS
#undef PP_ROW
#undef PP_TAP
#undef PP_TAP_LAST
#undef PP_BETWEEN
#undef PP_RA
#undef PP_RW
#undef PP_RBIAS
}

}
}

namespace fosvos {
int conv_pp_workgroups() { return 256; }
#ifdef FOSVOS_LAB_BUILD
static unsigned long long *g_pp_stamps = nullptr;
extern "C" void fosvos_lab_set_pp_stamps(void *p) { g_pp_stamps = (unsigned long long *)p; }
#endif

bool conv_pp_applicable(int N, int H, int W, int in_ch, int out_ch) {
    if (out_ch % 64 != 0 || in_ch % 32 != 0) return false;
    const int n_cb = out_ch / 64;
    if (n_cb != 1 && n_cb != 2 && n_cb != 4 && n_cb != 8) return false;
    const int64_t tiles = cdiv(W, pp::TW) * cdiv(H, pp::TH) * N;
    if (tiles > 0x3fffffff) return false;
    const int64_t units = tiles * n_cb, slots = 2 * conv_pp_workgroups();
    if (units < slots) return false;
    static const int mode = lab_env_int("FOSVOS_PP", -1);
    if (mode == 1 || in_ch <= 64) return true;
    return units * 10 >= cdiv(units, slots) * slots * 9;
}



int conv_pp_forward(const uint16_t *x, const uint16_t *w_packed, const float *bias, uint16_t *y, uint16_t *y_pool, int N,
                    int H, int W, int Cin_pad, int Cout, int Co_pad, bool relu, hipStream_t st, const uint8_t *mask_bits) {
    FOSVOS_REQUIRE(!y_pool || relu, FOSVOS_E_ARG, "conv3x3 (persistent): the fused pool takes post-ReLU values");
    FOSVOS_REQUIRE(!mask_bits || (!relu && !y_pool && !bias), FOSVOS_E_ARG, "conv3x3 (persistent): the bit mask is the data gradient's epilogue");
    pp::Args a{};
    a.x = x; a.w = w_packed; a.bias = bias; a.y = y; a.y_pool = y_pool; a.mask_bits = mask_bits;
    a.N = N; a.H = H; a.W = W; a.Cin = Cin_pad; a.Cout = Cout; a.Co_pad = Co_pad;
    a.tiles_x = (int)cdiv(W, pp::TW);
    a.tiles_y = (int)cdiv(H, pp::TH);
    a.n_tiles = a.tiles_x * a.tiles_y * N;
    a.n_cb = Cout / 64;
    a.lab = lab_env_int("FOSVOS_PP_LAB", 0);
#ifdef FOSVOS_LAB_BUILD
    a.stamps = g_pp_stamps;
#endif
    void (*kern)(const pp::Args) = mask_bits ? pp::k_conv3x3_pp<false, false, true>
                                   : y_pool  ? pp::k_conv3x3_pp<true, true>
                                   : relu    ? pp::k_conv3x3_pp<true, false> : pp::k_conv3x3_pp<false, false>;
    const int which = mask_bits ? 3 : y_pool ? 2 : relu ? 1 : 0;
    static bool once[64][4];
    int dev = 0;
    FOSVOS_HIP_CHECK(hipGetDevice(&dev));
    if (dev >= 0 && dev < 64 && !once[dev][which]) {
        FOSVOS_HIP_CHECK(hipFuncSetAttribute(reinterpret_cast<const void *>(kern), hipFuncAttributeMaxDynamicSharedMemorySize,
                                             pp::LDS_BYTES));
        once[dev][which] = true;
    }
    FOSVOS_PROF(mask_bits ? "k_conv3x3_pp<false, false, true>" : y_pool ? "k_conv3x3_pp<true, true, false>"
                : relu    ? "k_conv3x3_pp<true, false, false>" : "k_conv3x3_pp<false, false, false>", st,
                2.0 * N * H * W * 9.0 * Cin_pad * Cout);
    hipLaunchKernelGGL(kern, dim3(conv_pp_workgroups()), dim3(pp::NT), pp::LDS_BYTES, st, a);
    FOSVOS_LAUNCH_CHECK();
    return FOSVOS_OK;
}

}
```

fosvos_amd/csrc/vgg_net.hip:

```cpp
#include <stdlib.h>

#include "common.hpp"

using namespace fosvos;

namespace {
constexpr int kNConv = 13;
constexpr int kStageOf[kNConv] = {0, 0, 1, 1, 2, 2, 2, 3, 3, 3, 4, 4, 4};
constexpr int kCin[kNConv] = {3, 64, 64, 128, 128, 256, 256, 256, 512, 512, 512, 512, 512};
constexpr int kCout[kNConv] = {64, 64, 128, 128, 256, 256, 256, 512, 512, 512, 512, 512, 512};
constexpr int kFirstOfStage[5] = {0, 2, 4, 7, 10};
constexpr int kLastOfStage[5] = {1, 3, 6, 9, 12};
constexpr int kStageCh[5] = {64, 128, 256, 512, 512};

inline size_t up256(size_t v) { return (v + 255) / 256 * 256; }

struct Arena {
    int sh[5], sw[5];
    size_t act[kNConv];
    size_t gact[kNConv];
    size_t pooled[4];
    size_t gpooled[4];
    size_t side[4];
    size_t dside[4];
    size_t bits0;
    size_t ws, ws_bytes;
    size_t hws, hws_bytes;
    size_t wsa_conv[kNConv], wsa_conv_bytes[kNConv], wsa_side[4], wsa_side_bytes[4];
    size_t total;
};

Arena make_arena(int N, int H, int W) {
    Arena a{};
    a.sh[0] = H; a.sw[0] = W;
    for (int s = 1; s < 5; ++s) { a.sh[s] = (a.sh[s - 1] + 1) / 2; a.sw[s] = (a.sw[s - 1] + 1) / 2; }
    size_t off = 0;
    auto take = [&](size_t bytes) { const size_t o = off; off += up256(bytes); return o; };
    for (int c = 0; c < kNConv; ++c) {
        const int s = kStageOf[c];
        const size_t bytes = (size_t)N * a.sh[s] * a.sw[s] * kCout[c] * 2;
        a.act[c] = take(bytes);
        a.gact[c] = take(bytes);
    }
    for (int s = 1; s < 5; ++s) {
        const size_t bytes = (size_t)N * a.sh[s] * a.sw[s] * kStageCh[s - 1] * 2;
        a.pooled[s - 1] = take(bytes);
        a.gpooled[s - 1] = take(bytes);
        a.side[s - 1] = take((size_t)N * a.sh[s] * a.sw[s] * 16 * 4);
        a.dside[s - 1] = take((size_t)N * a.sh[s] * a.sw[s] * 32 * 2);
    }
    a.bits0 = take((size_t)N * H * W * (kCout[0] / 8));
    a.hws_bytes = up256(fosvos_head_bwd_workspace_bytes(N, H, W));
    a.hws = take(a.hws_bytes);
    size_t ws = 256;
    a.wsa_conv_bytes[0] = up256(fosvos_conv3x3_first_wgrad_workspace_bytes(N, H, W, 64));
    for (int c = 1; c < kNConv; ++c) {
        const int s = kStageOf[c];
        a.wsa_conv_bytes[c] = fosvos_conv3x3_wgrad_workspace_bytes(N, a.sh[s], a.sw[s], kCin[c], kCout[c]);
        if (N >= 2)
            a.wsa_conv_bytes[c] = std::max(a.wsa_conv_bytes[c],
                                           fosvos_conv3x3_workspace_bytes(N - (N + 1) / 2, a.sh[s], a.sw[s], kCin[c], kCout[c]));
        a.wsa_conv_bytes[c] = up256(a.wsa_conv_bytes[c]);
        ws = std::max(ws, fosvos_conv3x3_workspace_bytes(N, a.sh[s], a.sw[s], kCin[c], kCout[c]));
        if (N >= 2)
            ws = std::max(ws, fosvos_conv3x3_workspace_bytes((N + 1) / 2, a.sh[s], a.sw[s], kCin[c], kCout[c]));
        ws = std::max(ws, fosvos_conv3x3_workspace_bytes(N, a.sh[s], a.sw[s], kCout[c], kCin[c]));
    }
    for (int s = 1; s < 5; ++s) {
        a.wsa_side_bytes[s - 1] = up256(std::max({fosvos_conv3x3_wgrad_workspace_bytes(N, a.sh[s], a.sw[s], kStageCh[s], 16),
                                                  fosvos_conv3x3_workspace_bytes(N, a.sh[s], a.sw[s], kStageCh[s], 16),
                                                  N >= 2 ? fosvos_conv3x3_workspace_bytes(N - (N + 1) / 2, a.sh[s], a.sw[s], kStageCh[s], 16) : (size_t)0}));
        ws = std::max(ws, fosvos_conv3x3_workspace_bytes(N, a.sh[s], a.sw[s], kStageCh[s], 16));
        if (N >= 2) ws = std::max(ws, fosvos_conv3x3_workspace_bytes((N + 1) / 2, a.sh[s], a.sw[s], kStageCh[s], 16));
        ws = std::max(ws, fosvos_conv3x3_workspace_bytes(N, a.sh[s], a.sw[s], 16, kStageCh[s]));
    }
    a.ws_bytes = up256(ws);
    a.ws = take(a.ws_bytes);
    for (int c = 0; c < kNConv; ++c) a.wsa_conv[c] = take(a.wsa_conv_bytes[c]);
    for (int i = 0; i < 4; ++i) a.wsa_side[i] = take(a.wsa_side_bytes[i]);
    a.total = off;
    return a;
}

static_assert(kFosvosVggEvents == 25, "event slots below");
constexpr int kBucketFinalEvent = 22;
constexpr int kStage2WgradEvent = 23;
constexpr int kMainTailEvent = 24;
constexpr int kBucketEvent0 = 19;

#define FOSVOS_TRY(expr)          \
    do {                          \
        const int rc_ = (expr);   \
        if (rc_ != FOSVOS_OK) return rc_; \
    } while (0)

int check_net(const void *w, const void *frame, const void *arena, int N, int H, int W, size_t arena_bytes,
              const Arena &a, const char *who) {
    FOSVOS_REQUIRE(w && frame && arena, FOSVOS_E_ARG, "%s: null pointer", who);
    FOSVOS_REQUIRE(N > 0 && H > 0 && W > 0, FOSVOS_E_SHAPE, "%s: bad shape N=%d H=%d W=%d", who, N, H, W);
    FOSVOS_REQUIRE(arena_bytes >= a.total, FOSVOS_E_WORKSPACE, "%s: arena %zu < %zu bytes", who, arena_bytes, a.total);
    FOSVOS_REQUIRE(((uintptr_t)arena & 255) == 0, FOSVOS_E_ARG, "%s: arena must be 256-byte aligned", who);
    return FOSVOS_OK;
}
}

extern "C" size_t fosvos_vgg_arena_bytes(int N, int H, int W) {
    if (N <= 0 || H <= 0 || W <= 0) return 0;
    return make_arena(N, H, W).total;
}

extern "C" int fosvos_vgg_arena_layout(int N, int H, int W, fosvos_vgg_arena_layout_info *out) {
    FOSVOS_REQUIRE(out, FOSVOS_E_ARG, "vgg_arena_layout: null output");
    FOSVOS_REQUIRE(N > 0 && H > 0 && W > 0, FOSVOS_E_SHAPE, "vgg_arena_layout: bad shape N=%d H=%d W=%d", N, H, W);
    const Arena a = make_arena(N, H, W);
    *out = fosvos_vgg_arena_layout_info{};
    out->total = a.total;
    for (int s = 0; s < 5; ++s) { out->stage_h[s] = a.sh[s]; out->stage_w[s] = a.sw[s]; }
    for (int c = 0; c < kNConv; ++c) {
        const int s = kStageOf[c];
        out->act[c] = a.act[c];
        out->gact[c] = a.gact[c];
        out->act_bytes[c] = (size_t)N * a.sh[s] * a.sw[s] * kCout[c] * 2;
        out->wsa_conv[c] = a.wsa_conv[c];
        out->wsa_conv_bytes[c] = a.wsa_conv_bytes[c];
    }
    for (int s = 1; s < 5; ++s) {
        const size_t px = (size_t)N * a.sh[s] * a.sw[s];
        out->pooled[s - 1] = a.pooled[s - 1];
        out->gpooled[s - 1] = a.gpooled[s - 1];
        out->pooled_bytes[s - 1] = px * kStageCh[s - 1] * 2;
        out->side[s - 1] = a.side[s - 1];
        out->side_bytes[s - 1] = px * 16 * 4;
        out->dside[s - 1] = a.dside[s - 1];
        out->dside_bytes[s - 1] = px * 32 * 2;
        out->wsa_side[s - 1] = a.wsa_side[s - 1];
        out->wsa_side_bytes[s - 1] = a.wsa_side_bytes[s - 1];
    }
    out->bits0 = a.bits0;
    out->bits0_bytes = (size_t)N * H * W * (kCout[0] / 8);
    out->ws = a.ws; out->ws_bytes = a.ws_bytes;
    out->hws = a.hws; out->hws_bytes = a.hws_bytes;
    return FOSVOS_OK;
}

namespace {
int forward_impl(hipEvent_t *ev, const fosvos_vgg_weights *w, const float *frame, int N, int H, int W, void *arena,
                 size_t arena_bytes, float *fused, float *const side_out[4], int device, void *stream, void *aux_stream) {
    const Arena a = make_arena(N, H, W);
    FOSVOS_TRY(check_net(w, frame, arena, N, H, W, arena_bytes, a, "vgg_forward"));
    FOSVOS_REQUIRE(fused, FOSVOS_E_ARG, "vgg_forward: null output");
    char *base = reinterpret_cast<char *>(arena);
    auto act = [&](int c) { return reinterpret_cast<uint16_t *>(base + a.act[c]); };
    void *ws = base + a.ws;
    hipStream_t sm = (hipStream_t)stream;
    const bool par = ev != nullptr && aux_stream != nullptr && aux_stream != stream;
    hipStream_t sa = par ? (hipStream_t)aux_stream : sm;
    if (par) FOSVOS_ENTER(device);
    static const bool split_on = lab_env_int("FOSVOS_FWD_SPLIT", 1) != 0;
    if (split_on && N >= 2) {
        const int na = (N + 1) / 2;
        if (par) {
            FOSVOS_HIP_CHECK(hipEventRecord(ev[14], sm));
            FOSVOS_HIP_CHECK(hipStreamWaitEvent(sa, ev[14], 0));
        }
        for (int half = 0; half < 2; ++half) {
            const int f0 = half ? na : 0, nf = half ? N - na : na;
            hipStream_t st = half ? sa : sm;
            const uint16_t *xh = nullptr;
            for (int c = 0; c < kNConv; ++c) {
                const int s = kStageOf[c];
                const size_t px = (size_t)a.sh[s] * a.sw[s];
                uint16_t *yc = act(c) + (size_t)f0 * px * kCout[c];
                void *wsc = half ? base + a.wsa_conv[c] : ws;
                const size_t wsn = half ? a.wsa_conv_bytes[c] : a.ws_bytes;
                if (c == 0) {
                    FOSVOS_TRY(fosvos_conv3x3_first_fwd_bits(frame + (size_t)f0 * 3 * H * W, w->conv_w[0], w->conv_b[0], yc,
                                                             reinterpret_cast<uint8_t *>(base + a.bits0) + (size_t)f0 * px * (kCout[0] / 8),
                                                             nf, H, W, kCout[0], device, st));
                } else {
                    if (c == kFirstOfStage[s]) {
                        const size_t ppx = (size_t)a.sh[s] * a.sw[s];
                        xh = reinterpret_cast<uint16_t *>(base + a.pooled[s - 1]) + (size_t)f0 * ppx * kCin[c];
                    }
                    FOSVOS_REQUIRE(wsn >= fosvos_conv3x3_workspace_bytes(nf, a.sh[s], a.sw[s], kCin[c], kCout[c]),
                                   FOSVOS_E_WORKSPACE, "vgg_forward: split-K workspace of the second chain");
                    if (c == kLastOfStage[s] && s < 4) {
                        const size_t qpx = (size_t)a.sh[s + 1] * a.sw[s + 1];
                        FOSVOS_TRY(fosvos_conv3x3_fwd_pool(xh, w->conv_wf[c], w->conv_b[c], yc,
                                                           reinterpret_cast<uint16_t *>(base + a.pooled[s]) + (size_t)f0 * qpx * kCout[c],
                                                           nf, a.sh[s], a.sw[s], kCin[c], kCout[c], FOSVOS_CONV_RELU, wsc, wsn,
                                                           device, st));
                    } else {
                        FOSVOS_TRY(fosvos_conv3x3_fwd(xh, w->conv_wf[c], w->conv_b[c], yc, nf, a.sh[s], a.sw[s], kCin[c],
                                                      kCout[c], FOSVOS_CONV_RELU, wsc, wsn, device, st));
                    }
                }
                xh = yc;
                if (s > 0 && c == kLastOfStage[s]) {
                    float *so = reinterpret_cast<float *>(base + a.side[s - 1]) + (size_t)f0 * px * 16;
                    FOSVOS_TRY(fosvos_conv3x3_fwd(xh, w->side_wf[s - 1], w->side_b[s - 1], so, nf, a.sh[s], a.sw[s], kStageCh[s],
                                                  16, FOSVOS_CONV_OUT_F32, half ? base + a.wsa_side[s - 1] : ws,
                                                  half ? a.wsa_side_bytes[s - 1] : a.ws_bytes, device, st));
                }
            }
        }
        static const bool head_per_chain = lab_env_int("FOSVOS_HEAD_PER_CHAIN", 1) != 0;
        if (head_per_chain) {
            for (int half = 0; half < 2; ++half) {
                const int f0 = half ? na : 0, nf = half ? N - na : na;
                const float *sideh[4];
                float *soh[4] = {nullptr, nullptr, nullptr, nullptr};
                int hsh[4], wsh[4];
                for (int i = 0; i < 4; ++i) {
                    hsh[i] = a.sh[i + 1];
                    wsh[i] = a.sw[i + 1];
                    sideh[i] = reinterpret_cast<const float *>(base + a.side[i]) + (size_t)f0 * hsh[i] * wsh[i] * 16;
                    if (side_out && side_out[i]) soh[i] = side_out[i] + (size_t)f0 * H * W;
                }
                FOSVOS_TRY(fosvos_head_fwd(sideh, hsh, wsh, w->filt, w->filt1, w->dsn_w, w->dsn_b, w->fuse_w, w->fuse_b,
                                           fused + (size_t)f0 * H * W, (side_out && side_out[0]) ? soh : nullptr, nf, H, W,
                                           w->filt_uniform, device, half ? sa : sm));
            }
        }
        if (par) {
            FOSVOS_HIP_CHECK(hipEventRecord(ev[13], sa));
            FOSVOS_HIP_CHECK(hipStreamWaitEvent(sm, ev[13], 0));
        }
        if (head_per_chain) return FOSVOS_OK;
    } else {
    const uint16_t *x = nullptr;
    for (int c = 0; c < kNConv; ++c) {
        const int s = kStageOf[c];
        if (c == 0) {
            FOSVOS_TRY(fosvos_conv3x3_first_fwd_bits(frame, w->conv_w[0], w->conv_b[0], act(0),
                                                     reinterpret_cast<uint8_t *>(base + a.bits0), N, H, W, kCout[0], device, stream));
        } else {
            if (c == kFirstOfStage[s])
                x = reinterpret_cast<uint16_t *>(base + a.pooled[s - 1]);
            if (c == kLastOfStage[s] && s < 4) {
                FOSVOS_TRY(fosvos_conv3x3_fwd_pool(x, w->conv_wf[c], w->conv_b[c], act(c),
                                                   reinterpret_cast<uint16_t *>(base + a.pooled[s]), N, a.sh[s], a.sw[s],
                                                   kCin[c], kCout[c], FOSVOS_CONV_RELU, ws, a.ws_bytes, device, stream));
            } else {
                FOSVOS_TRY(fosvos_conv3x3_fwd(x, w->conv_wf[c], w->conv_b[c], act(c), N, a.sh[s], a.sw[s], kCin[c], kCout[c],
                                              FOSVOS_CONV_RELU, ws, a.ws_bytes, device, stream));
            }
        }
        x = act(c);
        if (s > 0 && c == kLastOfStage[s]) {
            const bool on_aux = par && s < 4;
            if (on_aux) {
                FOSVOS_HIP_CHECK(hipEventRecord(ev[c], sm));
                FOSVOS_HIP_CHECK(hipStreamWaitEvent(sa, ev[c], 0));
            }
            FOSVOS_TRY(fosvos_conv3x3_fwd(x, w->side_wf[s - 1], w->side_b[s - 1], base + a.side[s - 1], N, a.sh[s], a.sw[s],
                                          kStageCh[s], 16, FOSVOS_CONV_OUT_F32, on_aux ? base + a.wsa_side[s - 1] : ws,
                                          on_aux ? a.wsa_side_bytes[s - 1] : a.ws_bytes, device, on_aux ? sa : sm));
        }
    }
    if (par) {
        FOSVOS_HIP_CHECK(hipEventRecord(ev[13], sa));
        FOSVOS_HIP_CHECK(hipStreamWaitEvent(sm, ev[13], 0));
    }
    }
    const float *side[4];
    int hs[4], wsz[4];
    for (int i = 0; i < 4; ++i) {
        side[i] = reinterpret_cast<const float *>(base + a.side[i]);
        hs[i] = a.sh[i + 1];
        wsz[i] = a.sw[i + 1];
    }
    return fosvos_head_fwd(side, hs, wsz, w->filt, w->filt1, w->dsn_w, w->dsn_b, w->fuse_w, w->fuse_b, fused, side_out, N, H,
                           W, w->filt_uniform, device, stream);
}
}

extern "C" int fosvos_vgg_forward_streams(fosvos_ctx *ctx, const fosvos_vgg_weights *w, const float *frame, int N, int H,
                                          int W, void *arena, size_t arena_bytes, float *fused, float *const side_out[4],
                                          void *stream, void *aux_stream) {
    FOSVOS_TRY(ctx_check(ctx, "vgg_forward_streams"));
    return forward_impl(ctx->vgg_ev, w, frame, N, H, W, arena, arena_bytes, fused, side_out, ctx->device, stream, aux_stream);
}

extern "C" int fosvos_vgg_forward(const fosvos_vgg_weights *w, const float *frame, int N, int H, int W, void *arena,
                                  size_t arena_bytes, float *fused, float *const side_out[4], int device,
                                  void *stream) {
    return forward_impl(nullptr, w, frame, N, H, W, arena, arena_bytes, fused, side_out, device, stream, nullptr);
}

extern "C" int fosvos_vgg_backward(fosvos_ctx *ctx, const fosvos_vgg_weights *w, const fosvos_vgg_grads *g,
                                   const float *frame, int N, int H, int W, void *arena, size_t arena_bytes,
                                   const float *d_fused, const float *const d_side_out[4], void *stream,
                                   void *aux_stream) {
    FOSVOS_TRY(ctx_check(ctx, "vgg_backward"));
    const int device = ctx->device;
    const Arena a = make_arena(N, H, W);
    FOSVOS_TRY(check_net(w, frame, arena, N, H, W, arena_bytes, a, "vgg_backward"));
    FOSVOS_REQUIRE(g, FOSVOS_E_ARG, "vgg_backward: null gradient table");
    const bool with_so = d_side_out && d_side_out[0];
    FOSVOS_REQUIRE(d_fused || with_so, FOSVOS_E_ARG, "vgg_backward: no upstream gradient given");
    char *base = reinterpret_cast<char *>(arena);
    auto act = [&](int c) { return reinterpret_cast<uint16_t *>(base + a.act[c]); };
    auto gact = [&](int c) { return reinterpret_cast<uint16_t *>(base + a.gact[c]); };
    void *ws = base + a.ws;
    const int acc = g->accumulate ? 1 : 0;
    WgradReduceTable reduce;
    reduce.n = 0;
    WgradReduceTable reduce_m;
    reduce_m.n = 0;

    hipStream_t sm = (hipStream_t)stream;
    const bool par = aux_stream != nullptr && aux_stream != stream;
    hipStream_t sa = par ? (hipStream_t)aux_stream : sm;
    hipEvent_t *ev = ctx->vgg_ev;
    const bool buckets = g->bucket_events != 0;
    const bool tail = g->last_pass_of_cycle != 0;
    static const int tail_stages = lab_env_int("FOSVOS_TAIL_STAGES", 1);
    static const bool offload_on = lab_env_int("FOSVOS_TAIL_OFFLOAD", 1) != 0;
    const bool offload = tail && aux_stream != nullptr && aux_stream != stream && offload_on;
    FOSVOS_ENTER(device);
    ctx->buckets_recorded = false;
    if (par) {
        FOSVOS_HIP_CHECK(hipEventRecord(ev[14], sm));
        FOSVOS_HIP_CHECK(hipStreamWaitEvent(sa, ev[14], 0));
    }
    auto publish = [&](int e) -> int {
        if (!par) return FOSVOS_OK;
        FOSVOS_HIP_CHECK(hipEventRecord(ev[e], sm));
        FOSVOS_HIP_CHECK(hipStreamWaitEvent(sa, ev[e], 0));
        return FOSVOS_OK;
    };

    const float *side[4];
    uint16_t *dside[4];
    int hs[4], wsz[4];
    for (int i = 0; i < 4; ++i) {
        side[i] = reinterpret_cast<const float *>(base + a.side[i]);
        dside[i] = reinterpret_cast<uint16_t *>(base + a.dside[i]);
        hs[i] = a.sh[i + 1];
        wsz[i] = a.sw[i + 1];
    }
    const HeadBwdArgs ha{side, hs, wsz, w->filt, with_so ? w->filt1 : nullptr, with_so ? w->dsn_w : nullptr, w->fuse_w,
                         d_fused, with_so ? d_side_out : nullptr, dside, g->fuse_w, g->fuse_b,
                         with_so ? g->dsn_w : nullptr, with_so ? g->dsn_b : nullptr, N, H, W, acc, base + a.hws,
                         a.hws_bytes, device, w->filt_uniform & 15};
    FOSVOS_TRY(head_bwd_check(ha));
    FOSVOS_TRY(head_bwd_scale(ha, 3, sm));
    for (int i = 2; i >= 0; --i) {
        FOSVOS_TRY(head_bwd_scale(ha, i, sa));
        if (par) FOSVOS_HIP_CHECK(hipEventRecord(ev[16 + i], sa));
    }
    FOSVOS_TRY(publish(13));
    FOSVOS_TRY(head_bwd_finish(ha, sa));

    static const bool unpool_fused = lab_env_int("FOSVOS_UNPOOL", 1) != 0;
    for (int s = 4; s >= 0; --s) {
        const int hh = a.sh[s], ww = a.sw[s], last = kLastOfStage[s], first = kFirstOfStage[s];
        if (s > 0) {
            FOSVOS_TRY(wgrad_impl(act(last), dside[s - 1], g->side_w[s - 1], g->side_b[s - 1], N, hh, ww, kStageCh[s], 16,
                                  acc, base + a.wsa_side[s - 1], a.wsa_side_bytes[s - 1], device, sa,
                                  (offload && s == 1) ? &reduce_m : &reduce, tail && s <= tail_stages));
            const uint16_t *addend = (s < 4) ? gact(last) : nullptr;
            if (par && s < 4) FOSVOS_HIP_CHECK(hipStreamWaitEvent(sm, ev[16 + s - 1], 0));
            if (s < 4 && unpool_fused)
                FOSVOS_TRY(fosvos_conv3x3_dgrad_unpool(dside[s - 1], w->side_wd[s - 1], act(last),
                                                       reinterpret_cast<const uint16_t *>(base + a.gpooled[s]), gact(last), N, hh,
                                                       ww, kStageCh[s], 16, ws, a.ws_bytes, device, sm));
            else
                FOSVOS_TRY(fosvos_conv3x3_dgrad(dside[s - 1], w->side_wd[s - 1], act(last), addend, gact(last), N, hh, ww,
                                                kStageCh[s], 16, ws, a.ws_bytes, device, sm));
        }
        FOSVOS_TRY(publish(last));
        for (int c = last; c >= first; --c) {
            if (c == 0) {
                if (offload)
                    FOSVOS_TRY(first_wgrad_impl(frame, gact(0), g->conv_w[0], g->conv_b[0], N, H, W, kCout[0], acc,
                                                base + a.wsa_conv[0], a.wsa_conv_bytes[0], device, sm, &reduce_m));
                else
                    FOSVOS_TRY(first_wgrad_impl(frame, gact(0), g->conv_w[0], g->conv_b[0], N, H, W, kCout[0], acc,
                                                base + a.wsa_conv[0], a.wsa_conv_bytes[0], device, sa, &reduce));
                break;
            }
            const bool from_pool = (c == first) && s > 0;
            const uint16_t *xin = from_pool ? reinterpret_cast<const uint16_t *>(base + a.pooled[s - 1]) : act(c - 1);
            uint16_t *dx = from_pool ? reinterpret_cast<uint16_t *>(base + a.gpooled[s - 1]) : gact(c - 1);
            const uint16_t *mask = from_pool ? nullptr : act(c - 1);
            const bool middle = (last - first == 2) && c == last - 1;
            if (!middle)
                FOSVOS_TRY(wgrad_impl(xin, gact(c), g->conv_w[c], g->conv_b[c], N, hh, ww, kCin[c], kCout[c], acc,
                                      base + a.wsa_conv[c], a.wsa_conv_bytes[c], device, sa,
                                      (offload && s == 1) ? &reduce_m : &reduce, tail && s <= tail_stages));
            static const bool bits_on = lab_env_int("FOSVOS_RELU_BITS", 1) != 0;
            if (c == 1 && bits_on)
                FOSVOS_TRY(fosvos_conv3x3_dgrad_bits(gact(c), w->conv_wd[c], reinterpret_cast<const uint8_t *>(base + a.bits0), nullptr,
                                                     dx, N, hh, ww, kCin[c], kCout[c], ws, a.ws_bytes, device, sm));
            else
                FOSVOS_TRY(fosvos_conv3x3_dgrad(gact(c), w->conv_wd[c], mask, nullptr, dx, N, hh, ww, kCin[c], kCout[c], ws,
                                                a.ws_bytes, device, sm));
            const bool skip_event = (last - first == 2) && c == last;
            if (!from_pool && !skip_event) FOSVOS_TRY(publish(c - 1));
            if (middle)
                FOSVOS_TRY(wgrad_impl(xin, gact(c), g->conv_w[c], g->conv_b[c], N, hh, ww, kCin[c], kCout[c], acc,
                                      base + a.wsa_conv[c], a.wsa_conv_bytes[c], device, sa,
                                      (offload && s == 1) ? &reduce_m : &reduce, tail && s <= tail_stages));
        }
        if (s == 1 || (s > 0 && !unpool_fused))
            FOSVOS_TRY(fosvos_maxpool2x2_ceil_bwd(act(kLastOfStage[s - 1]), reinterpret_cast<const uint16_t *>(base + a.gpooled[s - 1]),
                                                  gact(kLastOfStage[s - 1]), N, a.sh[s - 1], a.sw[s - 1], kStageCh[s - 1], 1,
                                                  device, sm));
        if (s >= 1) {
            FOSVOS_TRY(wgrad_reduce_all(&reduce, device, sa));
            if (buckets && s >= 2) FOSVOS_HIP_CHECK(hipEventRecord(ev[kBucketEvent0 + (4 - s)], sa));
            if (offload && s == 1) FOSVOS_HIP_CHECK(hipEventRecord(ev[kStage2WgradEvent], sa));
        }
    }
    FOSVOS_TRY(wgrad_reduce_all(&reduce, device, sa));
    if (offload) {
        FOSVOS_HIP_CHECK(hipStreamWaitEvent(sm, ev[kStage2WgradEvent], 0));
        FOSVOS_TRY(wgrad_reduce_all(&reduce_m, device, sm));
    }
    if (buckets) FOSVOS_HIP_CHECK(hipEventRecord(ev[kMainTailEvent], sm));
    if (buckets) {
        FOSVOS_HIP_CHECK(hipEventRecord(ev[kBucketFinalEvent], sa));
        ctx->buckets_recorded = true;
    }
    if (par && !g->defer_join) {
        FOSVOS_HIP_CHECK(hipEventRecord(ev[15], sa));
        FOSVOS_HIP_CHECK(hipStreamWaitEvent(sm, ev[15], 0));
    }
    return FOSVOS_OK;
}

extern "C" int fosvos_vgg_grad_bucket_wait(fosvos_ctx *ctx, int bucket, void *stream) {
    FOSVOS_TRY(ctx_check(ctx, "vgg_grad_bucket_wait"));
    FOSVOS_REQUIRE(bucket >= 0 && bucket < 5, FOSVOS_E_ARG, "vgg_grad_bucket_wait: bucket %d not in 0..4", bucket);
    FOSVOS_ENTER(ctx->device);
    FOSVOS_REQUIRE(ctx->buckets_recorded, FOSVOS_E_ARG,
                   "vgg_grad_bucket_wait: the last fosvos_vgg_backward on this context did not set grads.bucket_events");
    hipEvent_t *ev = ctx->vgg_ev;
    if (bucket < 3) {
        FOSVOS_HIP_CHECK(hipStreamWaitEvent((hipStream_t)stream, ev[kBucketEvent0 + bucket], 0));
    } else {
        FOSVOS_HIP_CHECK(hipStreamWaitEvent((hipStream_t)stream, ev[kBucketFinalEvent], 0));
        FOSVOS_HIP_CHECK(hipStreamWaitEvent((hipStream_t)stream, ev[kMainTailEvent], 0));
    }
    return FOSVOS_OK;
}
```

fosvos_amd/fosvos_hip/__init__.py:

```python
from __future__ import annotations

import ctypes
import os
import threading
from ctypes import POINTER, c_char_p, c_float, c_int, c_int64, c_size_t, c_uint, c_void_p

_HERE = os.path.dirname(os.path.abspath(__file__))
PKG_ROOT = os.path.dirname(_HERE)
LIB_PATH = os.environ.get("FOSVOS_HIP_LIB") or os.path.join(PKG_ROOT, "lib", "libfosvos_hip.so")
HEADER_PATH = os.path.join(os.path.dirname(PKG_ROOT), "include", "fosvos_hip.h")

ABI_VERSION = 22
CONV_RELU = 1
CONV_OUT_F32 = 2


class FosvosHipError(RuntimeError):
    pass


class SgdEntry(ctypes.Structure):
    _fields_ = [("param", c_void_p), ("grad", c_void_p), ("momentum_buf", c_void_p), ("numel", c_int64),
                ("lr", c_float), ("weight_decay", c_float)]


_P4 = c_void_p * 4
_I4 = c_int * 4
_P13 = c_void_p * 13


class VggWeights(ctypes.Structure):
    _fields_ = [("conv_w", _P13), ("conv_b", _P13), ("conv_wf", _P13), ("conv_wd", _P13),
                ("side_b", _P4), ("side_wf", _P4), ("side_wd", _P4), ("filt", _P4), ("filt1", _P4),
                ("dsn_w", c_void_p), ("dsn_b", c_void_p), ("fuse_w", c_void_p), ("fuse_b", c_void_p),
                ("filt_uniform", c_int)]


class VggGrads(ctypes.Structure):
    _fields_ = [("conv_w", _P13), ("conv_b", _P13), ("side_w", _P4), ("side_b", _P4),
                ("dsn_w", c_void_p), ("dsn_b", c_void_p), ("fuse_w", c_void_p), ("fuse_b", c_void_p),
                ("accumulate", c_int), ("defer_join", c_int), ("bucket_events", c_int), ("last_pass_of_cycle", c_int)]

_Z4 = c_size_t * 4
_Z13 = c_size_t * 13


class VggArenaLayout(ctypes.Structure):
    _fields_ = [("total", c_size_t), ("stage_h", c_int * 5), ("stage_w", c_int * 5),
                ("act", _Z13), ("gact", _Z13), ("act_bytes", _Z13),
                ("pooled", _Z4), ("gpooled", _Z4), ("pooled_bytes", _Z4),
                ("side", _Z4), ("side_bytes", _Z4), ("dside", _Z4), ("dside_bytes", _Z4),
                ("bits0", c_size_t), ("bits0_bytes", c_size_t),
                ("ws", c_size_t), ("ws_bytes", c_size_t), ("hws", c_size_t), ("hws_bytes", c_size_t),
                ("wsa_conv", _Z13), ("wsa_conv_bytes", _Z13), ("wsa_side", _Z4), ("wsa_side_bytes", _Z4)]


class Conv3x3PlanInfo(ctypes.Structure):
    _fields_ = [("tile_h", c_int), ("tile_w", c_int), ("tile_co", c_int), ("k_splits", c_int), ("workgroups", c_int),
                ("persistent", c_int)]


class Conv2dPlanInfo(ctypes.Structure):
    _fields_ = [("cob", c_int), ("threads", c_int), ("slices", c_int), ("workgroups", c_int), ("mfma_frag_blocks", c_int),
                ("mfma_workgroups", c_int)]


class ProfileRecord(ctypes.Structure):
    _fields_ = [("name", ctypes.c_char * 96), ("launches", c_int), ("ms", ctypes.c_double), ("flops", ctypes.c_double)]


class PackEntry(ctypes.Structure):
    _fields_ = [("w", c_void_p), ("w_fwd", c_void_p), ("w_dgrad", c_void_p), ("Co", c_int), ("Ci", c_int)]



class Conv2dDesc(ctypes.Structure):
    _fields_ = [("w_packed", c_void_p), ("bias", c_void_p), ("Ci", c_int), ("Co", c_int), ("k", c_int), ("stride", c_int),
                ("kind", c_int)]


class ResnetBlock(ctypes.Structure):
    _fields_ = [("conv", Conv2dDesc * 3), ("n_convs", c_int), ("has_down", c_int), ("down", Conv2dDesc)]


class ResnetNet(ctypes.Structure):
    _fields_ = [("first_w", c_void_p), ("first_b", c_void_p), ("first_co", c_int), ("first_fp32_math", c_int), ("first_unfused", c_int),
                ("blocks_per_stage", c_int * 4),
                ("blocks", POINTER(ResnetBlock)), ("side", Conv2dDesc * 4), ("filt", c_void_p * 4),
                ("filt1", c_void_p * 4), ("stride", c_int * 4), ("dsn_w", c_void_p), ("dsn_b", c_void_p),
                ("fuse_b", c_void_p)]

SIGNATURES = {
    "fosvos_abi_version": (c_int, []),
    "fosvos_last_error": (c_char_p, []),
    "fosvos_build_arch": (c_char_p, []),
    "fosvos_ctx_create": (c_int, [c_int, POINTER(c_void_p)]),
    "fosvos_ctx_destroy": (c_int, [c_void_p]),
    "fosvos_ctx_device": (c_int, [c_void_p]),
    "fosvos_conv3x3_plan": (c_int, [c_int, c_int, c_int, c_int, c_int, POINTER(Conv3x3PlanInfo)]),
    "fosvos_conv3x3_fwd_plan": (c_int, [c_int, c_int, c_int, c_int, c_int, ctypes.c_uint, POINTER(Conv3x3PlanInfo)]),
    "fosvos_conv3x3_first_plan": (c_int, [c_int, c_int, c_int, POINTER(c_int), POINTER(c_int)]),
    "fosvos_nchw_f32_to_nhwc_bf16": (c_int, [c_void_p, c_void_p, c_int, c_int, c_int, c_int, c_int, c_int, c_void_p]),
    "fosvos_nhwc_bf16_to_nchw_f32": (c_int, [c_void_p, c_void_p, c_int, c_int, c_int, c_int, c_int, c_int, c_void_p]),
    "fosvos_nhwc_f32_to_nchw_f32": (c_int, [c_void_p, c_void_p, c_int, c_int, c_int, c_int, c_int, c_void_p]),
    "fosvos_nchw_f32_to_nhwc_f32": (c_int, [c_void_p, c_void_p, c_int, c_int, c_int, c_int, c_int, c_void_p]),
    "fosvos_pack_conv3x3_weights": (c_int, [c_void_p, c_int, c_int, c_void_p, c_void_p, c_int, c_void_p]),
    "fosvos_packed_weight_elems": (c_size_t, [c_int, c_int]),
    "fosvos_pack_conv3x3_weights_multi": (c_int, [POINTER(PackEntry), c_int, c_int, c_void_p]),
    "fosvos_conv3x3_first_fwd": (c_int, [c_void_p, c_void_p, c_void_p, c_void_p, c_int, c_int, c_int, c_int, c_int,
                                         c_void_p]),
    "fosvos_conv3x3_first_fwd_bits": (c_int, [c_void_p, c_void_p, c_void_p, c_void_p, c_void_p, c_int, c_int, c_int, c_int, c_int,
                                              c_void_p]),
    "fosvos_conv3x3_dgrad_bits": (c_int, [c_void_p, c_void_p, c_void_p, c_void_p, c_void_p, c_int, c_int, c_int, c_int,
                                          c_int, c_void_p, c_size_t, c_int, c_void_p]),
    "fosvos_conv3x3_dgrad_unpool": (c_int, [c_void_p, c_void_p, c_void_p, c_void_p, c_void_p, c_int, c_int, c_int, c_int,
                                            c_int, c_void_p, c_size_t, c_int, c_void_p]),
    "fosvos_conv3x3_first_wgrad": (c_int, [c_void_p, c_void_p, c_void_p, c_void_p, c_int, c_int, c_int, c_int,
                                           c_void_p, c_size_t, c_int, c_void_p]),
    "fosvos_conv3x3_first_wgrad_workspace_bytes": (c_size_t, [c_int, c_int, c_int, c_int]),
    "fosvos_conv3x3_fwd": (c_int, [c_void_p, c_void_p, c_void_p, c_void_p, c_int, c_int, c_int, c_int, c_int, c_uint,
                                   c_void_p, c_size_t, c_int, c_void_p]),
    "fosvos_conv3x3_fwd_pool": (c_int, [c_void_p, c_void_p, c_void_p, c_void_p, c_void_p, c_int, c_int, c_int, c_int,
                                        c_int, c_uint, c_void_p, c_size_t, c_int, c_void_p]),
    "fosvos_conv3x3_workspace_bytes": (c_size_t, [c_int, c_int, c_int, c_int, c_int]),
    "fosvos_conv3x3_dgrad": (c_int, [c_void_p, c_void_p, c_void_p, c_void_p, c_void_p, c_int, c_int, c_int, c_int,
                                     c_int, c_void_p, c_size_t, c_int, c_void_p]),
    "fosvos_conv3x3_wgrad": (c_int, [c_void_p, c_void_p, c_void_p, c_void_p, c_int, c_int, c_int, c_int, c_int, c_int,
                                     c_void_p, c_size_t, c_int, c_void_p]),
    "fosvos_conv3x3_wgrad_slabs": (c_int, [c_void_p, c_void_p, c_int, c_int, c_int, c_int, c_int, c_int, c_void_p, c_size_t,
                                           c_int, c_void_p]),
    "fosvos_conv3x3_wgrad_reduce": (c_int, [c_void_p, c_void_p, c_int, c_int, c_int, c_int, c_int, c_int, c_void_p,
                                            c_size_t, c_int, c_void_p]),
    "fosvos_conv3x3_wgrad_workspace_bytes": (c_size_t, [c_int, c_int, c_int, c_int, c_int]),
    "fosvos_maxpool2x2_ceil_fwd": (c_int, [c_void_p, c_void_p, c_int, c_int, c_int, c_int, c_int, c_void_p]),
    "fosvos_maxpool2x2_ceil_bwd": (c_int, [c_void_p, c_void_p, c_void_p, c_int, c_int, c_int, c_int, c_int, c_int,
                                           c_void_p]),
    "fosvos_head_fwd": (c_int, [POINTER(c_void_p), POINTER(c_int), POINTER(c_int), POINTER(c_void_p),
                                POINTER(c_void_p), c_void_p, c_void_p, c_void_p, c_void_p, c_void_p,
                                POINTER(c_void_p), c_int, c_int, c_int, c_int, c_int, c_void_p]),
    "fosvos_head_bwd": (c_int, [POINTER(c_void_p), POINTER(c_int), POINTER(c_int), POINTER(c_void_p),
                                POINTER(c_void_p), c_void_p, c_void_p, c_void_p, POINTER(c_void_p),
                                POINTER(c_void_p), c_void_p, c_void_p, c_void_p, c_void_p, c_int, c_int, c_int, c_int,
                                c_void_p, c_size_t, c_int, c_void_p]),
    "fosvos_head_bwd_workspace_bytes": (c_size_t, [c_int, c_int, c_int]),
    "fosvos_cbce_loss": (c_int, [c_void_p, c_void_p, c_int64, c_int, c_float, c_void_p, c_void_p, c_void_p, c_size_t,
                                 c_int, c_void_p]),
    "fosvos_cbce_workspace_bytes": (c_size_t, [c_int64]),
    "fosvos_cbce_loss_frames": (c_int, [c_void_p, c_void_p, c_int64, c_int, c_int, c_float, c_void_p, c_void_p, c_void_p,
                                        c_size_t, c_int, c_void_p]),
    "fosvos_cbce_loss_frames_parts": (c_int, [c_void_p, c_void_p, c_int64, c_int, c_int, c_float, c_void_p, c_void_p,
                                              c_void_p, c_size_t, c_int, c_int, c_void_p]),
    "fosvos_cbce_loss_batch_counts": (c_int, [c_void_p, c_void_p, c_int64, c_int, c_float, c_void_p, c_void_p, c_void_p,
                                              c_void_p, c_size_t, c_int, c_void_p]),
    "fosvos_sgd_momentum_step": (c_int, [c_void_p, c_int, c_int64, c_float, c_int, c_int, c_void_p]),
    "fosvos_conv3x3_s2_fwd": (c_int, [c_void_p, c_void_p, c_void_p, c_void_p, c_int, c_int, c_int, c_int, c_int, c_uint,
                                      c_void_p, c_size_t, c_int, c_void_p]),
    "fosvos_conv3x3_fwd_add": (c_int, [c_void_p, c_void_p, c_void_p, c_void_p, c_void_p, c_int, c_int, c_int, c_int, c_int,
                                       c_uint, c_void_p, c_size_t, c_int, c_void_p]),
    "fosvos_fold_conv_bn": (c_int, [c_void_p, c_int, c_int, c_int, c_void_p, c_void_p, c_void_p, c_void_p, c_void_p,
                                    c_float, c_void_p, c_void_p, c_int, c_void_p]),
    "fosvos_conv2d_packed_dwords": (c_size_t, [c_int, c_int, c_int]),
    "fosvos_conv2d_bias_elems": (c_size_t, [c_int]),
    "fosvos_pack_conv2d_bn": (c_int, [c_void_p, c_int, c_int, c_int, c_void_p, c_void_p, c_void_p, c_void_p, c_void_p,
                                      c_float, c_void_p, c_void_p, c_int, c_void_p]),
    "fosvos_conv2d_plan": (c_int, [c_int, c_int, c_int, c_int, c_int, c_int, c_int, POINTER(Conv2dPlanInfo)]),
    "fosvos_conv2d_fwd": (c_int, [c_void_p, c_void_p, c_void_p, c_void_p, c_void_p, c_int, c_int, c_int, c_int, c_int,
                                  c_int, c_int, c_uint, c_int, c_void_p]),
    "fosvos_conv7x7_packed_elems": (c_size_t, [c_int]),
    "fosvos_pack_conv7x7_bn": (c_int, [c_void_p, c_int, c_void_p, c_void_p, c_void_p, c_void_p, c_float, c_void_p,
                                       c_void_p, c_int, c_void_p]),
    "fosvos_conv7x7s2_first_fwd": (c_int, [c_void_p, c_void_p, c_void_p, c_void_p, c_int, c_int, c_int, c_int, c_uint,
                                           c_int, c_void_p]),
    "fosvos_conv7x7s2_pool_first_fwd": (c_int, [c_void_p, c_void_p, c_void_p, c_void_p, c_int, c_int, c_int, c_int, c_int,
                                                c_void_p]),
    "fosvos_maxpool3x3s2_fwd": (c_int, [c_void_p, c_void_p, c_int, c_int, c_int, c_int, c_int, c_void_p]),
    "fosvos_deconv_head_fwd": (c_int, [POINTER(c_void_p), POINTER(c_int), POINTER(c_int), POINTER(c_int),
                                       POINTER(c_void_p), POINTER(c_void_p), c_void_p, c_void_p, c_void_p, c_void_p,
                                       POINTER(c_void_p), c_int, c_int, c_int, c_int, c_void_p]),
    "fosvos_resnet_arena_bytes": (c_size_t, [POINTER(ResnetNet), c_int, c_int, c_int]),
    "fosvos_resnet_forward": (c_int, [POINTER(ResnetNet), c_void_p, c_int, c_int, c_int, c_void_p, c_size_t, c_void_p,
                                      POINTER(c_void_p), c_int, c_void_p, c_void_p, c_void_p]),
    "fosvos_vgg_arena_bytes": (c_size_t, [c_int, c_int, c_int]),
    "fosvos_vgg_arena_layout": (c_int, [c_int, c_int, c_int, POINTER(VggArenaLayout)]),
    "fosvos_vgg_grad_bucket_wait": (c_int, [c_void_p, c_int, c_void_p]),
    "fosvos_profile_start": (c_int, [c_int, c_int]),
    "fosvos_profile_stop": (c_int, [c_int, POINTER(ProfileRecord), c_int, POINTER(c_int)]),
    "fosvos_vgg_forward": (c_int, [POINTER(VggWeights), c_void_p, c_int, c_int, c_int, c_void_p, c_size_t, c_void_p,
                                   POINTER(c_void_p), c_int, c_void_p]),
    "fosvos_vgg_forward_streams": (c_int, [c_void_p, POINTER(VggWeights), c_void_p, c_int, c_int, c_int, c_void_p, c_size_t,
                                           c_void_p, POINTER(c_void_p), c_void_p, c_void_p]),
    "fosvos_augment_sample": (c_int, [c_void_p, c_void_p, c_int, c_int, c_int, c_void_p, c_void_p, c_void_p, c_void_p,
                                      c_void_p, c_void_p, c_int, c_int, c_void_p, c_void_p, c_void_p, c_void_p, c_int,
                                      c_void_p]),
    "fosvos_prob_bytes": (c_int, [c_void_p, c_int, c_int, c_int, c_void_p, c_void_p, c_int, c_void_p]),
    "fosvos_jf_workspace_bytes": (c_size_t, [c_int, c_int, c_int]),
    "fosvos_jf_counts": (c_int, [c_void_p, c_void_p, c_int, c_int, c_int, c_int, c_void_p, c_void_p, c_size_t, c_int,
                                 c_void_p]),
    "fosvos_png_capacity_bytes": (c_size_t, [c_int, c_int, c_int]),
    "fosvos_png_workspace_bytes": (c_size_t, [c_int, c_int, c_int]),
    "fosvos_png_encode": (c_int, [c_void_p, c_int, c_int, c_int, c_void_p, c_size_t, c_void_p, c_void_p, c_size_t, c_int,
                                  c_void_p]),
    "fosvos_vgg_backward": (c_int, [c_void_p, POINTER(VggWeights), POINTER(VggGrads), c_void_p, c_int, c_int, c_int, c_void_p,
                                    c_size_t, c_void_p, POINTER(c_void_p), c_void_p, c_void_p]),
}

_lib = None
_lock = threading.Lock()


def lib() -> ctypes.CDLL:
    global _lib
    if _lib is not None:
        return _lib
    with _lock:
        if _lib is not None:
            return _lib
        if not os.path.exists(LIB_PATH):
            raise FosvosHipError(
                f"{LIB_PATH} not found: build it with `python -c 'import __graft_entry__ as g; g.build()'` "
                f"or `make -C fosvos_amd/csrc`.  There is no CPU fallback.")
        import torch
        handle = ctypes.CDLL(LIB_PATH)
        for name, (restype, argtypes) in SIGNATURES.items():
            fn = getattr(handle, name)
            fn.restype = restype
            fn.argtypes = argtypes
        got = handle.fosvos_abi_version()
        if got != ABI_VERSION:
            raise FosvosHipError(f"libfosvos_hip.so ABI {got} != binding ABI {ABI_VERSION}: rebuild")
        _lib = handle
    return _lib


def check(rc: int, what: str) -> None:
    if rc != 0:
        msg = lib().fosvos_last_error()
        raise FosvosHipError(f"{what} failed (code {rc}): {msg.decode(errors='replace') if msg else ''}")


class LaunchProfile:

    def __init__(self, device: int, max_launches: int = 65536):
        self.device, self.max_launches, self.records = int(device), int(max_launches), {}

    def __enter__(self):
        check(lib().fosvos_profile_start(self.device, self.max_launches), "profile_start")
        return self

    def __exit__(self, *exc):
        buf = (ProfileRecord * 128)()
        n = c_int(0)
        check(lib().fosvos_profile_stop(self.device, buf, 128, ctypes.byref(n)), "profile_stop")
        self.records = {buf[i].name.decode(): {"launches": buf[i].launches, "ms": buf[i].ms, "flops": buf[i].flops}
                        for i in range(n.value)}
        return False


class Context:

    def __init__(self, device: int):
        h = c_void_p()
        check(lib().fosvos_ctx_create(int(device), ctypes.byref(h)), "ctx_create")
        self.handle, self.device = h, int(device)

    def close(self) -> None:
        h, self.handle = self.handle, None
        if h is not None and _lib is not None:
            _lib.fosvos_ctx_destroy(h)

    def __del__(self):
        try:
            self.close()
        except Exception:
            pass
# ... 9 lines not shown
```

fosvos_amd/fosvos_hip/engine.py:

```python
from __future__ import annotations

import ctypes
import time
from dataclasses import dataclass
from typing import Dict, List, Optional, Sequence, Tuple

import torch

from . import Context, VggGrads, VggWeights, check, lib, ops, ptr_array4
from .options import EngineOptions, native_loop_from_env

STAGE_CHANNELS = ((64, 64), (128, 128), (256, 256, 256), (512, 512, 512), (512, 512, 512))
STAGE_IN = (3, 64, 128, 256, 512)
SIDE_CH = 16


def conv_module_index(stage: int, k: int) -> int:
    return 2 * k + (0 if stage == 0 else 1)


def param_names() -> List[str]:
    names = [f"upscale.{i}.weight" for i in range(4)] + [f"upscale_.{i}.weight" for i in range(4)]
    for s, chans in enumerate(STAGE_CHANNELS):
        for j in range(len(chans)):
# ... 273 lines not shown
        t0 = time.perf_counter()
        for st in streams:
            with torch.cuda.stream(st):
                torch.cuda._sleep(_PROBE_CYCLES)
        torch.cuda.synchronize(dev)
        return (time.perf_counter() - t0) * 1e3

    run([a]); run([a, b])
    alone = min(run([a]) for _ in range(3))
    pair = min(run([a, b]) for _ in range(3))
    return pair < 1.5 * alone, alone, pair


def shared_stream(device_index: int, role: str, probe: Optional[bool] = None) -> "torch.cuda.Stream":
    key = (device_index, role)
    st = _SHARED_STREAMS.get(key)
    if st is None:
        order = ("aux", "pass", "comm")
        for earlier in order[:order.index(role)] if role in order else ():
            shared_stream(device_index, earlier)
        others = {"caller": torch.cuda.current_stream(device_index)}
        for r in order:
            if (device_index, r) in _SHARED_STREAMS:
                others[r] = _SHARED_STREAMS[(device_index, r)]
        if probe is None:
            probe = EngineOptions.from_env().stream_probe
        probe_on = probe and role != "comm" and hasattr(torch.cuda, "_sleep")
        parked, result = [], {"overlaps_with": {}, "tries": 0, "ms": {}}
        for attempt in range(6):
            st = torch.cuda.Stream(device=device_index)
            result["tries"] = attempt + 1
            if not probe_on:
                break
            ok = True
            for name, other in others.items():
                if other.cuda_stream == st.cuda_stream:
                    continue
                good, alone, pair = _streams_overlap(device_index, other, st)
                result["overlaps_with"][name] = bool(good)
                result["ms"][name] = [round(alone, 3), round(pair, 3)]
                ok = ok and good
            if ok:
                break
            parked.append(st)
        _SHARED_STREAMS[("parked", role, device_index)] = parked
        STREAM_PROBE[key] = result
        _SHARED_STREAMS[key] = st
    return st


class ArenaPool:

    def __init__(self) -> None:
        self._free: Dict[Tuple[int, int, int, int], List[torch.Tensor]] = {}
        self._aux: Dict[int, "torch.cuda.Stream"] = {}
        self._ctx: Dict[int, "Context"] = {}
        self._pending: List[Tuple[int, int, int, torch.Tensor, Optional[torch.Tensor]]] = []
        self._home: Dict[int, Tuple[int, int, int, int]] = {}
        self.reserve_frames = 0

    def aux_stream(self, device_index: int) -> int:
        st = self._aux.get(device_index)
        if st is None:
            st = self._aux[device_index] = shared_stream(device_index, "aux")
        return st.cuda_stream

    def ctx(self, device_index: int):
        c = self._ctx.get(device_index)
        if c is None:
            c = self._ctx[device_index] = Context(device_index)
        return c.handle

    def take(self, n: int, h: int, w: int, device: torch.device) -> torch.Tensor:
        dev = device.index if device.index is not None else torch.cuda.current_device()
        key = (n, h, w, dev)
        free = self._free.setdefault(key, [])
        if free:
            return free.pop()
        nbytes = lib().fosvos_vgg_arena_bytes(n, h, w)
        for (n2, h2, w2, d2), lst in self._free.items():
            if lst and h2 == h and w2 == w and d2 == dev and n2 > n and lst[-1].numel() >= nbytes + 256:
                return lst.pop()
        n_top = max(n, int(self.reserve_frames))
        for m in range(n + 1, n_top + 1):
            nbytes = max(nbytes, lib().fosvos_vgg_arena_bytes(m, h, w))
        arena = torch.empty(nbytes + 256, dtype=torch.uint8, device=device)
        self._home[arena.data_ptr()] = (n_top, h, w, dev)
        return arena

    def hold(self, n: int, h: int, w: int, arena: torch.Tensor, frame: Optional[torch.Tensor] = None) -> None:
        self._pending.append((n, h, w, arena, frame))

    def join(self) -> None:
        for idx, st in self._aux.items():
            torch.cuda.current_stream(idx).wait_stream(st)
        for n, h, w, arena, _frame in self._pending:
            self.give(n, h, w, arena)
        self._pending.clear()

    def give(self, n: int, h: int, w: int, arena: torch.Tensor) -> None:
        key = self._home.get(arena.data_ptr(), (n, h, w, arena.device.index))
        free = self._free.setdefault(key, [])
        if len(free) < 6:
            free.append(arena)
        else:
            self._home.pop(arena.data_ptr(), None)


def _aligned_ptr(arena: torch.Tensor) -> Tuple[int, int]:
    p = arena.data_ptr()
    ap = (p + 255) // 256 * 256
    return ap, arena.numel() - (ap - p)


def _weights_struct(P: Dict[str, torch.Tensor], packs: PackedWeights):
    w = VggWeights()
    keep = []
    named = [(wn, P[wn]) for c, (wn, _) in enumerate(_CONV_NAMES) if c > 0]
    named += [(f"side_prep.{i}.weight", P[f"side_prep.{i}.weight"]) for i in range(4)]
    images = packs.conv_many(named)
    for c, (wn, bn) in enumerate(_CONV_NAMES):
        w.conv_w[c] = P[wn].data_ptr()
        w.conv_b[c] = P[bn].data_ptr()
        if c > 0:
            wf, wd = images[c - 1]
            w.conv_wf[c], w.conv_wd[c] = wf.data_ptr(), wd.data_ptr()
    for i in range(4):
        wf, wd = images[len(_CONV_NAMES) - 1 + i]
        w.side_wf[i], w.side_wd[i] = wf.data_ptr(), wd.data_ptr()
        w.side_b[i] = P[f"side_prep.{i}.bias"].data_ptr()
        f = packs.deconv_diag(f"upscale.{i}.weight", P[f"upscale.{i}.weight"])
        f1 = packs.deconv_diag(f"upscale_.{i}.weight", P[f"upscale_.{i}.weight"])
        w.filt[i], w.filt1[i] = f.data_ptr(), f1.data_ptr()
    dsn_w = packs.small("dsn_w", [P[f"score_dsn.{i}.weight"] for i in range(4)])
    dsn_b = packs.small("dsn_b", [P[f"score_dsn.{i}.bias"] for i in range(4)])
    w.dsn_w, w.dsn_b = dsn_w.data_ptr(), dsn_b.data_ptr()
    w.fuse_w, w.fuse_b = P["fuse.weight"].data_ptr(), P["fuse.bias"].data_ptr()
    w.filt_uniform = packs.head_uniform_mask(P)
    keep += [dsn_w, dsn_b]
    return w, keep


def native_forward(P, packs, pool: ArenaPool, x: torch.Tensor, with_side_out: bool, keep: bool):
    _check_frame(x)
    for name in ("stages.0.0.weight", "fuse.weight"):
        if not P[name].is_cuda or P[name].dtype != torch.float32:
            raise RuntimeError("OSVOS_VGG parameters must be fp32 tensors on the GPU")
    x = x.contiguous().float()
    N, _, H, W = x.shape
    dev = x.device
    arena = pool.take(N, H, W, dev)
    ap, an = _aligned_ptr(arena)
    w, keep_alive = _weights_struct(P, packs)
    fused = torch.empty((N, 1, H, W), dtype=torch.float32, device=dev)
    outs = [torch.empty((N, 1, H, W), dtype=torch.float32, device=dev) for _ in range(4)] if with_side_out else None
    so = ptr_array4([o.data_ptr() for o in outs]) if with_side_out else None
    idx = dev.index if dev.index is not None else torch.cuda.current_device()
    t0 = ops._pb()
    opts = packs.options
    aux = (pool.aux_stream(idx) if N >= 2 and opts.fwd_aux and opts.two_streams and not packs.flags.forward_one_stream
           else 0)
    if aux:
        check(lib().fosvos_vgg_forward_streams(pool.ctx(idx), ctypes.byref(w), x.data_ptr(), N, H, W, ap, an, fused.data_ptr(),
                                               so, torch.cuda.current_stream(idx).cuda_stream, aux), "vgg_forward_streams")
    else:
        check(lib().fosvos_vgg_forward(ctypes.byref(w), x.data_ptr(), N, H, W, ap, an, fused.data_ptr(), so, idx,
                                       torch.cuda.current_stream(idx).cuda_stream), "vgg_forward")
    ops._pe(t0, "vgg_forward", 2.0 * 129.114e9 * N * H * W / (480 * 854), 0.0)
    if not keep:
        pool.give(N, H, W, arena)
        arena = None
    return (outs if outs is not None else [None] * 4) + [fused], (arena, x, w, keep_alive, (N, H, W))


def native_backward(P, packs, saved, d_outs, inplace: bool) -> Dict[str, torch.Tensor]:
    arena, x, w, keep_alive, (N, H, W) = saved
    dev = x.device
    d_fused = d_outs[4]
    d_so, with_so = _side_grads(d_outs)
    grads: Dict[str, torch.Tensor] = {}
    if d_fused is None and not with_so:
        return grads
    g = VggGrads()
    hold = []

    def slot(name: str) -> int:
        p = P[name]
        if inplace:
            if p.grad is None or p.grad.dtype != torch.float32 or not p.grad.is_contiguous():
                p.grad = torch.zeros_like(p, memory_format=torch.contiguous_format)
            torch.autograd.graph.increment_version(p.grad)
            return p.grad.data_ptr()
        t = torch.empty_like(p, memory_format=torch.contiguous_format)
        grads[name] = t
        return t.data_ptr()

    for c, (wn, bn) in enumerate(_CONV_NAMES):
        g.conv_w[c], g.conv_b[c] = slot(wn), slot(bn)
    for i in range(4):
        g.side_w[i], g.side_b[i] = slot(f"side_prep.{i}.weight"), slot(f"side_prep.{i}.bias")
    g.fuse_w, g.fuse_b = slot("fuse.weight"), slot("fuse.bias")
    dsn_tmp = None
    if with_so:
        dsn_tmp = (torch.zeros((4, 16), dtype=torch.float32, device=dev), torch.zeros((4,), dtype=torch.float32, device=dev))
        g.dsn_w, g.dsn_b = dsn_tmp[0].data_ptr(), dsn_tmp[1].data_ptr()
    flags = packs.flags
    overwrite = inplace and flags.overwrite_grads
    if overwrite and with_so:
        raise RuntimeError("OSVOS_VGG backward: overwrite_grads with side-output gradients (score_dsn accumulates through a scratch)")
    g.accumulate = 1 if inplace and not overwrite else 0
    idx = dev.index if dev.index is not None else torch.cuda.current_device()
    aux = packs.arenas.aux_stream(idx) if packs.options.two_streams else 0
    g.defer_join = 1 if (flags.defer_wgrad_join and inplace and aux) else 0
    g.bucket_events = 1 if flags.publish_grad_buckets else 0
    g.last_pass_of_cycle = 1 if flags.last_pass_of_cycle else 0
    if d_fused is not None:
        d_fused = d_fused.contiguous().float()
        hold.append(d_fused)
    dso = None
    if with_so:
        d_so = [t.contiguous().float() for t in d_so]
        hold += d_so
        dso = ptr_array4([t.data_ptr() for t in d_so])
    ap, an = _aligned_ptr(arena)
    t0 = ops._pb()
    check(lib().fosvos_vgg_backward(packs.arenas.ctx(idx), ctypes.byref(w), ctypes.byref(g), x.data_ptr(), N, H, W, ap, an,
                                    d_fused.data_ptr() if d_fused is not None else None, dso,
                                    torch.cuda.current_stream(idx).cuda_stream, aux or None),
          "vgg_backward")
    ops._pe(t0, "vgg_backward", 2.0 * (2 * 129.114e9 - 0.708e9) * N * H * W / (480 * 854), 0.0)
    if with_so:
        for i in range(4):
            gw, gb = dsn_tmp[0][i].reshape(1, 16, 1, 1), dsn_tmp[1][i:i + 1]
            if inplace:
                for name, val in ((f"score_dsn.{i}.weight", gw), (f"score_dsn.{i}.bias", gb)):
                    p = P[name]
                    if p.grad is None:
                        p.grad = val.clone()
                    else:
                        p.grad.add_(val)
            else:
                grads[f"score_dsn.{i}.weight"], grads[f"score_dsn.{i}.bias"] = gw.clone(), gb.clone()
    del hold, keep_alive
    if g.defer_join:
        packs.arenas.hold(N, H, W, arena, x)
    else:
        packs.arenas.give(N, H, W, arena)
    return grads


class _OSVOSFunction(torch.autograd.Function):

    @staticmethod
    def forward(ctx, packs: PackedWeights, with_side_out: bool, inplace: bool, x: torch.Tensor, *params: torch.Tensor):
        P = dict(zip(PARAM_NAMES, params))
        if USE_NATIVE_LOOP:
            outs, sv = native_forward(P, packs, packs.arenas, x, with_side_out, keep=True)
        else:
            outs, sv = forward(P, packs, x, with_side_out=with_side_out, keep=True)
        ctx.sv = sv
        ctx.packs = packs
        ctx.P = P
        ctx.set_materialize_grads(False)
        ctx.with_side_out = with_side_out
        ctx.inplace = inplace
        if not with_side_out:
            outs = [torch.empty(0, device=x.device) for _ in range(4)] + [outs[4]]
            ctx.mark_non_differentiable(*outs[:4])
        return tuple(outs)

    @staticmethod
    def backward(ctx, *d_outs):
        if ctx.sv is None:
            raise RuntimeError("OSVOS_VGG backward called but no activations were kept")
        d = list(d_outs)
        if not ctx.with_side_out:
            d = [None] * 4 + [d[4]]
        if USE_NATIVE_LOOP:
            grads = native_backward(ctx.P, ctx.packs, ctx.sv, d, inplace=ctx.inplace)
        else:
            grads = backward(ctx.P, ctx.packs, ctx.sv, d, inplace=ctx.inplace)
        ctx.sv = None
        out = [None, None, None, None]
        for name in PARAM_NAMES:
            g = grads.get(name)
            p = ctx.P[name]
            if g is not None and tuple(g.shape) != tuple(p.shape):
                g = g.reshape(p.shape)
            out.append(g if p.requires_grad else None)
        return tuple(out)


def run(packs: PackedWeights, params: Sequence[torch.Tensor], x: torch.Tensor, with_side_out: bool = True,
        inplace_grad: bool = False):
    if torch.is_grad_enabled() and any(p.requires_grad for p in params):
        return list(_OSVOSFunction.apply(packs, with_side_out, inplace_grad, x, *params))
    if USE_NATIVE_LOOP:
        outs, _ = native_forward(dict(zip(PARAM_NAMES, params)), packs, packs.arenas, x, with_side_out, keep=False)
    else:
        outs, _ = forward(dict(zip(PARAM_NAMES, params)), packs, x, with_side_out=with_side_out, keep=False)
    if not with_side_out:
        outs = [torch.empty(0, device=x.device) for _ in range(4)] + [outs[4]]
    return outs
```

fosvos_amd/fosvos_hip/ops.py:

```python
from __future__ import annotations

from typing import List, Optional, Sequence, Tuple

import torch

from . import CONV_OUT_F32, CONV_RELU, check, int_array4, lib, ptr_array4

_BF16 = torch.bfloat16
_F32 = torch.float32


def _need(t: torch.Tensor, dtype, what: str) -> torch.Tensor:
    if not t.is_cuda:
        raise RuntimeError(f"{what}: tensor must live on the GPU (the HIP path has no CPU fallback)")
    if t.dtype != dtype:
        raise TypeError(f"{what}: expected {dtype}, got {t.dtype}")
    if not t.is_contiguous():
        raise ValueError(f"{what}: tensor must be contiguous")
    return t


def _ctx(t: torch.Tensor) -> Tuple[int, int]:
    dev = t.device.index if t.device.index is not None else torch.cuda.current_device()
    return dev, torch.cuda.current_stream(dev).cuda_stream
# ... 69 lines not shown
    _PROF.records.append((name, float(flops), float(nbytes), e0, e1))


def nchw_to_nhwc_bf16(x: torch.Tensor, c_pad: Optional[int] = None) -> torch.Tensor:
    _need(x, _F32, "nchw_to_nhwc_bf16")
    n, c, h, w = x.shape
    c_pad = _ru(c, 8) if c_pad is None else c_pad
    out = torch.empty((n, h, w, c_pad), dtype=_BF16, device=x.device)
    dev, st = _ctx(x)
    check(lib().fosvos_nchw_f32_to_nhwc_bf16(x.data_ptr(), out.data_ptr(), n, c, h, w, c_pad, dev, st), "nchw_f32_to_nhwc_bf16")
    return out


def nhwc_bf16_to_nchw(x: torch.Tensor, c: Optional[int] = None) -> torch.Tensor:
    _need(x, _BF16, "nhwc_bf16_to_nchw")
    n, h, w, c_pad = x.shape
    c = c_pad if c is None else c
    out = torch.empty((n, c, h, w), dtype=_F32, device=x.device)
    dev, st = _ctx(x)
    check(lib().fosvos_nhwc_bf16_to_nchw_f32(x.data_ptr(), out.data_ptr(), n, c, h, w, c_pad, dev, st), "nhwc_bf16_to_nchw_f32")
    return out


def nhwc_f32_to_nchw(x: torch.Tensor) -> torch.Tensor:
    _need(x, _F32, "nhwc_f32_to_nchw")
    n, h, w, c = x.shape
    out = torch.empty((n, c, h, w), dtype=_F32, device=x.device)
    dev, st = _ctx(x)
    check(lib().fosvos_nhwc_f32_to_nchw_f32(x.data_ptr(), out.data_ptr(), n, c, h, w, dev, st), "nhwc_f32_to_nchw_f32")
    return out


def nchw_to_nhwc_f32(x: torch.Tensor) -> torch.Tensor:
    _need(x, _F32, "nchw_to_nhwc_f32")
    n, c, h, w = x.shape
    out = torch.empty((n, h, w, c), dtype=_F32, device=x.device)
    dev, st = _ctx(x)
    check(lib().fosvos_nchw_f32_to_nhwc_f32(x.data_ptr(), out.data_ptr(), n, c, h, w, dev, st), "nchw_f32_to_nhwc_f32")
    return out


def pack_conv3x3_weights(w: torch.Tensor, want_fwd: bool = True, want_dgrad: bool = True):
    _need(w, _F32, "pack_conv3x3_weights")
    co, ci, kh, kw = w.shape
    if (kh, kw) != (3, 3):
        raise ValueError("pack_conv3x3_weights: 3x3 kernels only")
    L = lib()
    fwd = torch.empty(L.fosvos_packed_weight_elems(co, ci), dtype=_BF16, device=w.device) if want_fwd else None
    dgr = torch.empty(L.fosvos_packed_weight_elems(ci, co), dtype=_BF16, device=w.device) if want_dgrad else None
    dev, st = _ctx(w)
    t0 = _pb()
    check(L.fosvos_pack_conv3x3_weights(w.data_ptr(), co, ci, _p(fwd), _p(dgr), dev, st), "pack_conv3x3_weights")
    _pe(t0, "pack_weights", 0.0, w.numel() * 4 + 2 * ((fwd.numel() if fwd is not None else 0) + (dgr.numel() if dgr is not None else 0)))
    return fwd, dgr


def pack_conv3x3_weights_multi(ws: Sequence[torch.Tensor]):
    from . import PackEntry
    if not ws:
        return []
    L = lib()
    arr = (PackEntry * len(ws))()
    out = []
    nbytes = 0
    for i, w in enumerate(ws):
        _need(w, _F32, "pack_conv3x3_weights_multi")
        co, ci, kh, kw = w.shape
        if (kh, kw) != (3, 3) or w.device != ws[0].device:
            raise ValueError("pack_conv3x3_weights_multi: 3x3 kernels on one device only")
        fwd = torch.empty(L.fosvos_packed_weight_elems(co, ci), dtype=_BF16, device=w.device)
        dgr = torch.empty(L.fosvos_packed_weight_elems(ci, co), dtype=_BF16, device=w.device)
        arr[i].w, arr[i].w_fwd, arr[i].w_dgrad, arr[i].Co, arr[i].Ci = w.data_ptr(), fwd.data_ptr(), dgr.data_ptr(), co, ci
        out.append((fwd, dgr))
        nbytes += w.numel() * 4 + 2 * (fwd.numel() + dgr.numel())
    dev, st = _ctx(ws[0])
    t0 = _pb()
    check(L.fosvos_pack_conv3x3_weights_multi(arr, len(ws), dev, st), "pack_conv3x3_weights_multi")
    _pe(t0, "pack_weights", 0.0, nbytes)
    return out


def conv3x3_first_fwd(frame: torch.Tensor, w: torch.Tensor, b: torch.Tensor, want_bits: bool = False):
    _need(frame, _F32, "conv3x3_first_fwd frame"); _need(w, _F32, "conv3x3_first_fwd weight"); _need(b, _F32, "conv3x3_first_fwd bias")
    n, c, h, wd = frame.shape
    if c != 3 or tuple(w.shape[1:]) != (3, 3, 3):
        raise ValueError("conv3x3_first_fwd: expects a 3-channel frame and [Co,3,3,3] weights")
    co = w.shape[0]
    y = torch.empty((n, h, wd, co), dtype=_BF16, device=frame.device)
    dev, st = _ctx(frame)
    t0 = _pb()
    bits = torch.empty((n, h, wd, co // 8), dtype=torch.uint8, device=frame.device) if want_bits else None
    check(lib().fosvos_conv3x3_first_fwd_bits(frame.data_ptr(), w.data_ptr(), b.data_ptr(), y.data_ptr(), _p(bits), n, h, wd, co,
                                              dev, st), "conv3x3_first_fwd")
    _pe(t0, "conv1_1_fwd", 2.0 * n * h * wd * 27 * co, n * h * wd * (12 + 2 * co))
    return (y, bits) if want_bits else y


def conv3x3_first_wgrad(frame: torch.Tensor, dy: torch.Tensor) -> Tuple[torch.Tensor, torch.Tensor]:
    _need(frame, _F32, "conv3x3_first_wgrad frame"); _need(dy, _BF16, "conv3x3_first_wgrad dy")
    n, c, h, wd = frame.shape
    co = dy.shape[3]
    if tuple(dy.shape[:3]) != (n, h, wd):
        raise ValueError("conv3x3_first_wgrad: dy shape mismatch")
    L = lib()
    dw = torch.empty((co, 3, 3, 3), dtype=_F32, device=frame.device)
    db = torch.empty((co,), dtype=_F32, device=frame.device)
    ws, wsn = _WS.get(L.fosvos_conv3x3_first_wgrad_workspace_bytes(n, h, wd, co), frame.device)
    dev, st = _ctx(frame)
    t0 = _pb()
    check(L.fosvos_conv3x3_first_wgrad(frame.data_ptr(), dy.data_ptr(), dw.data_ptr(), db.data_ptr(), n, h, wd, co, ws, wsn,
                                       dev, st), "conv3x3_first_wgrad")
    _pe(t0, "conv1_1_wgrad", 2.0 * n * h * wd * 27 * co, n * h * wd * (12 + 2 * co))
    return dw, db


def conv3x3_plan(n: int, h: int, w: int, in_ch: int, out_ch: int) -> dict:
    import ctypes
    from . import Conv3x3PlanInfo
    info = Conv3x3PlanInfo()
    check(lib().fosvos_conv3x3_plan(n, h, w, in_ch, out_ch, ctypes.byref(info)), "conv3x3_plan")
    return {"tile": (info.tile_h, info.tile_w, info.tile_co), "k_splits": info.k_splits, "workgroups": info.workgroups,
            "persistent": bool(info.persistent)}


def conv3x3_fwd_plan(n: int, h: int, w: int, in_ch: int, out_ch: int, relu: bool = True) -> dict:
    import ctypes
    from . import Conv3x3PlanInfo
    info = Conv3x3PlanInfo()
    check(lib().fosvos_conv3x3_fwd_plan(n, h, w, in_ch, out_ch, CONV_RELU if relu else 0, ctypes.byref(info)), "conv3x3_fwd_plan")
    return {"tile": (info.tile_h, info.tile_w, info.tile_co), "k_splits": info.k_splits, "workgroups": info.workgroups,
            "persistent": bool(info.persistent)}


def vgg_arena_layout(n: int, h: int, w: int) -> dict:
    import ctypes
    from . import VggArenaLayout
    info = VggArenaLayout()
    check(lib().fosvos_vgg_arena_layout(n, h, w, ctypes.byref(info)), "vgg_arena_layout")
    out = {}
    for name, _ in VggArenaLayout._fields_:
        v = getattr(info, name)
        out[name] = list(v) if isinstance(v, ctypes.Array) else int(v)
    return out


def conv3x3_first_plan(n: int, h: int, w: int) -> Tuple[int, int]:
    import ctypes
    tiles, wgs = ctypes.c_int(), ctypes.c_int()
    check(lib().fosvos_conv3x3_first_plan(n, h, w, ctypes.byref(tiles), ctypes.byref(wgs)), "conv3x3_first_plan")
    return tiles.value, wgs.value


def conv3x3_fwd(x: torch.Tensor, w_packed: torch.Tensor, bias: Optional[torch.Tensor], ci: int, co: int,
                relu: bool = True, out_f32: bool = False) -> torch.Tensor:
    _need(x, _BF16, "conv3x3_fwd x"); _need(w_packed, _BF16, "conv3x3_fwd packed weight")
    n, h, wd, cx = x.shape
    if cx != _ru(ci, 32):
        raise ValueError(f"conv3x3_fwd: x has {cx} channels, expected {_ru(ci, 32)} (Ci={ci} padded to 32)")
    L = lib()
    if w_packed.numel() != L.fosvos_packed_weight_elems(co, ci):
        raise ValueError("conv3x3_fwd: packed weight size does not match (Co, Ci)")
    if bias is not None:
        _need(bias, _F32, "conv3x3_fwd bias")
        if bias.numel() != co:
            raise ValueError("conv3x3_fwd: bias size")
    y = torch.empty((n, h, wd, co), dtype=_F32 if out_f32 else _BF16, device=x.device)
    flags = (CONV_RELU if relu else 0) | (CONV_OUT_F32 if out_f32 else 0)
    ws, wsn = _WS.get(L.fosvos_conv3x3_workspace_bytes(n, h, wd, ci, co), x.device)
    dev, st = _ctx(x)
    t0 = _pb()
    check(L.fosvos_conv3x3_fwd(x.data_ptr(), w_packed.data_ptr(), _p(bias), y.data_ptr(), n, h, wd, ci, co, flags, ws, wsn,
                               dev, st), "conv3x3_fwd")
    _pe(t0, "conv3x3_fwd", 2.0 * n * h * wd * 9 * ci * co,
        n * h * wd * (2 * cx + (4 if out_f32 else 2) * co) + 2 * 9 * ci * co)
    return y


def conv3x3_fwd_pool(x: torch.Tensor, w_packed: torch.Tensor, bias: Optional[torch.Tensor], ci: int, co: int,
                     relu: bool = True) -> Tuple[torch.Tensor, torch.Tensor]:
    _need(x, _BF16, "conv3x3_fwd_pool x"); _need(w_packed, _BF16, "conv3x3_fwd_pool packed weight")
    n, h, wd, cx = x.shape
    if cx != _ru(ci, 32):
        raise ValueError(f"conv3x3_fwd_pool: x has {cx} channels, expected {_ru(ci, 32)}")
    L = lib()
    if w_packed.numel() != L.fosvos_packed_weight_elems(co, ci):
        raise ValueError("conv3x3_fwd_pool: packed weight size does not match (Co, Ci)")
    if bias is not None:
        _need(bias, _F32, "conv3x3_fwd_pool bias")
    y = torch.empty((n, h, wd, co), dtype=_BF16, device=x.device)
    yp = torch.empty((n, (h + 1) // 2, (wd + 1) // 2, co), dtype=_BF16, device=x.device)
    ws, wsn = _WS.get(L.fosvos_conv3x3_workspace_bytes(n, h, wd, ci, co), x.device)
    dev, st = _ctx(x)
    t0 = _pb()
    check(L.fosvos_conv3x3_fwd_pool(x.data_ptr(), w_packed.data_ptr(), _p(bias), y.data_ptr(), yp.data_ptr(), n, h, wd, ci,
                                    co, CONV_RELU if relu else 0, ws, wsn, dev, st), "conv3x3_fwd_pool")
    _pe(t0, "conv3x3_fwd", 2.0 * n * h * wd * 9 * ci * co, n * h * wd * (2 * cx + 2 * co) + 2 * 9 * ci * co + yp.numel() * 2)
    return y, yp


def conv3x3_dgrad(dy: torch.Tensor, w_dgrad_packed: torch.Tensor, ci: int, co: int,
                  relu_src: Optional[torch.Tensor] = None, addend: Optional[torch.Tensor] = None,
                  out: Optional[torch.Tensor] = None, relu_bits: Optional[torch.Tensor] = None) -> torch.Tensor:
    _need(dy, _BF16, "conv3x3_dgrad dy"); _need(w_dgrad_packed, _BF16, "conv3x3_dgrad packed weight")
    n, h, wd, cy = dy.shape
    if cy != _ru(co, 32):
        raise ValueError(f"conv3x3_dgrad: dy has {cy} channels, expected {_ru(co, 32)}")
    L = lib()
    if w_dgrad_packed.numel() != L.fosvos_packed_weight_elems(ci, co):
        raise ValueError("conv3x3_dgrad: packed weight size does not match (Ci, Co)")
    shape = (n, h, wd, ci)
    for t, nm in ((relu_src, "relu_src"), (addend, "addend"), (out, "out")):
        if t is not None:
            _need(t, _BF16, f"conv3x3_dgrad {nm}")
            if tuple(t.shape) != shape:
                raise ValueError(f"conv3x3_dgrad: {nm} shape {tuple(t.shape)} != {shape}")
    dx = out if out is not None else torch.empty(shape, dtype=_BF16, device=dy.device)
    ws, wsn = _WS.get(L.fosvos_conv3x3_workspace_bytes(n, h, wd, co, ci), dy.device)
    dev, st = _ctx(dy)
    t0 = _pb()
    if relu_bits is not None:
        if relu_src is not None or relu_bits.dtype != torch.uint8 or tuple(relu_bits.shape) != (n, h, wd, ci // 8) or \
                not relu_bits.is_contiguous() or not relu_bits.is_cuda:
            raise ValueError("conv3x3_dgrad: relu_bits must be a contiguous uint8 [N,H,W,Ci/8] GPU tensor, given instead of relu_src")
        check(L.fosvos_conv3x3_dgrad_bits(dy.data_ptr(), w_dgrad_packed.data_ptr(), relu_bits.data_ptr(), _p(addend),
                                          dx.data_ptr(), n, h, wd, ci, co, ws, wsn, dev, st), "conv3x3_dgrad_bits")
    else:
        check(L.fosvos_conv3x3_dgrad(dy.data_ptr(), w_dgrad_packed.data_ptr(), _p(relu_src), _p(addend), dx.data_ptr(), n, h, wd,
                                     ci, co, ws, wsn, dev, st), "conv3x3_dgrad")
    _pe(t0, "conv3x3_dgrad", 2.0 * n * h * wd * 9 * ci * co,
        n * h * wd * 2 * (cy + ci * (1 + (relu_src is not None) + (addend is not None))) + 2 * 9 * ci * co)
    return dx


def conv3x3_dgrad_unpool(dy: torch.Tensor, w_dgrad_packed: torch.Tensor, ci: int, co: int, x: torch.Tensor,
                         d_pooled: torch.Tensor, out: Optional[torch.Tensor] = None) -> torch.Tensor:
    _need(dy, _BF16, "conv3x3_dgrad_unpool dy"); _need(w_dgrad_packed, _BF16, "conv3x3_dgrad_unpool packed weight")
    _need(x, _BF16, "conv3x3_dgrad_unpool x"); _need(d_pooled, _BF16, "conv3x3_dgrad_unpool d_pooled")
    n, h, wd, cy = dy.shape
    if cy != _ru(co, 32):
        raise ValueError(f"conv3x3_dgrad_unpool: dy has {cy} channels, expected {_ru(co, 32)}")
    L = lib()
    if w_dgrad_packed.numel() != L.fosvos_packed_weight_elems(ci, co):
        raise ValueError("conv3x3_dgrad_unpool: packed weight size does not match (Ci, Co)")
    if tuple(x.shape) != (n, h, wd, ci) or tuple(d_pooled.shape) != (n, (h + 1) // 2, (wd + 1) // 2, ci):
        raise ValueError(f"conv3x3_dgrad_unpool: x {tuple(x.shape)} / d_pooled {tuple(d_pooled.shape)} do not match "
                         f"{(n, h, wd, ci)} and its ceil-mode pooled map")
    if out is not None:
        _need(out, _BF16, "conv3x3_dgrad_unpool out")
        if tuple(out.shape) != (n, h, wd, ci) or out.data_ptr() == x.data_ptr():
            raise ValueError("conv3x3_dgrad_unpool: out must have x's shape and must not alias it")
    dx = out if out is not None else torch.empty((n, h, wd, ci), dtype=_BF16, device=dy.device)
    ws, wsn = _WS.get(L.fosvos_conv3x3_workspace_bytes(n, h, wd, co, ci), dy.device)
    dev, st = _ctx(dy)
    t0 = _pb()
    check(L.fosvos_conv3x3_dgrad_unpool(dy.data_ptr(), w_dgrad_packed.data_ptr(), x.data_ptr(), d_pooled.data_ptr(), dx.data_ptr(),
                                        n, h, wd, ci, co, ws, wsn, dev, st), "conv3x3_dgrad_unpool")
    _pe(t0, "conv3x3_dgrad_unpool", 2.0 * n * h * wd * 9 * ci * co, n * h * wd * 2 * (cy + 2 * ci + ci // 4) + 2 * 9 * ci * co)
    return dx


def conv3x3_wgrad(x: torch.Tensor, dy: torch.Tensor, ci: int, co: int, with_bias: bool = True,
                  dw: Optional[torch.Tensor] = None, db: Optional[torch.Tensor] = None, accumulate: bool = False):
    _need(x, _BF16, "conv3x3_wgrad x"); _need(dy, _BF16, "conv3x3_wgrad dy")
    n, h, wd, cx = x.shape
    if cx != ci or tuple(dy.shape) != (n, h, wd, _ru(co, 32)):
        raise ValueError(f"conv3x3_wgrad: shapes x={tuple(x.shape)} dy={tuple(dy.shape)} do not match Ci={ci} Co={co}")
    L = lib()
    if dw is None:
        if accumulate:
            raise ValueError("conv3x3_wgrad: accumulate needs an existing dw")
        dw = torch.empty((co, ci, 3, 3), dtype=_F32, device=x.device)
    if with_bias and db is None:
        if accumulate:
            raise ValueError("conv3x3_wgrad: accumulate needs an existing db")
        db = torch.empty((co,), dtype=_F32, device=x.device)
    _need(dw, _F32, "conv3x3_wgrad dw")
    ws, wsn = _WS.get(L.fosvos_conv3x3_wgrad_workspace_bytes(n, h, wd, ci, co), x.device)
    dev, st = _ctx(x)
    t0 = _pb()
    check(L.fosvos_conv3x3_wgrad_slabs(x.data_ptr(), dy.data_ptr(), 1 if with_bias else 0, n, h, wd, ci, co, ws, wsn, dev, st),
          "conv3x3_wgrad_slabs")
    _pe(t0, "conv3x3_wgrad", 2.0 * n * h * wd * 9 * ci * co, n * h * wd * 2 * (ci + dy.shape[3]))
    t0 = _pb()
    check(L.fosvos_conv3x3_wgrad_reduce(dw.data_ptr(), _p(db) if with_bias else None, n, h, wd, ci, co,
                                        1 if accumulate else 0, ws, wsn, dev, st), "conv3x3_wgrad_reduce")
    _pe(t0, "wgrad_reduce", 0.0, 4 * 9 * ci * co * 3)
    return dw, (db if with_bias else None)


def conv3x3_wgrad_one_call(x: torch.Tensor, dy: torch.Tensor, ci: int, co: int, with_bias: bool = True):
    _need(x, _BF16, "conv3x3_wgrad x"); _need(dy, _BF16, "conv3x3_wgrad dy")
    n, h, wd, _ = x.shape
    L = lib()
    dw = torch.empty((co, ci, 3, 3), dtype=_F32, device=x.device)
    db = torch.empty((co,), dtype=_F32, device=x.device) if with_bias else None
    ws, wsn = _WS.get(L.fosvos_conv3x3_wgrad_workspace_bytes(n, h, wd, ci, co), x.device)
    dev, st = _ctx(x)
    check(L.fosvos_conv3x3_wgrad(x.data_ptr(), dy.data_ptr(), dw.data_ptr(), _p(db), n, h, wd, ci, co, 0, ws, wsn, dev, st),
          "conv3x3_wgrad")
    return dw, db


def maxpool_fwd(x: torch.Tensor) -> torch.Tensor:
    _need(x, _BF16, "maxpool_fwd")
    n, h, w, c = x.shape
    y = torch.empty((n, (h + 1) // 2, (w + 1) // 2, c), dtype=_BF16, device=x.device)
    dev, st = _ctx(x)
    t0 = _pb()
    check(lib().fosvos_maxpool2x2_ceil_fwd(x.data_ptr(), y.data_ptr(), n, h, w, c, dev, st), "maxpool2x2_ceil_fwd")
    _pe(t0, "maxpool_fwd", 0.0, 2 * (x.numel() + y.numel()))
    return y


def maxpool_bwd(x: torch.Tensor, dy: torch.Tensor, relu_mask: bool = True) -> torch.Tensor:
    _need(x, _BF16, "maxpool_bwd x"); _need(dy, _BF16, "maxpool_bwd dy")
    n, h, w, c = x.shape
    if tuple(dy.shape) != (n, (h + 1) // 2, (w + 1) // 2, c):
        raise ValueError("maxpool_bwd: dy shape mismatch")
    dx = torch.empty_like(x)
    dev, st = _ctx(x)
    t0 = _pb()
    check(lib().fosvos_maxpool2x2_ceil_bwd(x.data_ptr(), dy.data_ptr(), dx.data_ptr(), n, h, w, c, 1 if relu_mask else 0,
                                           dev, st), "maxpool2x2_ceil_bwd")
    _pe(t0, "maxpool_bwd", 0.0, 2 * (2 * x.numel() + dy.numel()))
    return dx


def head_fwd(side: Sequence[torch.Tensor], filt: Sequence[torch.Tensor], filt1: Optional[Sequence[torch.Tensor]],
# ... 585 lines not shown
```

include/fosvos_hip.h:

```cpp
#ifndef FOSVOS_HIP_H
#define FOSVOS_HIP_H

#include <stddef.h>
#include <stdint.h>

#ifdef __cplusplus
extern "C" {
#endif

#define FOSVOS_ABI_VERSION 22

#define FOSVOS_OK 0
#define FOSVOS_E_SHAPE (-1)
#define FOSVOS_E_ARG (-2)
#define FOSVOS_E_WORKSPACE (-3)
#define FOSVOS_E_HIP (-4)

#define FOSVOS_CONV_RELU 1u
#define FOSVOS_CONV_OUT_F32 2u
#define FOSVOS_CONV_FP32_MATH 4u

int fosvos_abi_version(void);

typedef struct fosvos_profile_record {
    char name[96];
    int launches;
    double ms;
    double flops;
} fosvos_profile_record;
int fosvos_profile_start(int device, int max_launches);
int fosvos_profile_stop(int device, fosvos_profile_record *out, int capacity, int *n_out);
const char *fosvos_last_error(void);
const char *fosvos_build_arch(void);

typedef struct fosvos_ctx fosvos_ctx;
int fosvos_ctx_create(int device, fosvos_ctx **ctx_out);
int fosvos_ctx_destroy(fosvos_ctx *ctx);
int fosvos_ctx_device(const fosvos_ctx *ctx);

int fosvos_nchw_f32_to_nhwc_bf16(const float *src, uint16_t *dst, int N, int C, int H, int W, int Cpad,
                                 int device, void *stream);
int fosvos_nhwc_bf16_to_nchw_f32(const uint16_t *src, float *dst, int N, int C, int H, int W, int Cpad,
                                 int device, void *stream);
int fosvos_nhwc_f32_to_nchw_f32(const float *src, float *dst, int N, int C, int H, int W, int device, void *stream);
int fosvos_nchw_f32_to_nhwc_f32(const float *src, float *dst, int N, int C, int H, int W, int device, void *stream);
typedef struct fosvos_vgg_arena_layout_info {
    size_t total;
    int stage_h[5], stage_w[5];
    size_t act[13], gact[13], act_bytes[13];
    size_t pooled[4], gpooled[4], pooled_bytes[4];
    size_t side[4], side_bytes[4];
    size_t dside[4], dside_bytes[4];
    size_t bits0, bits0_bytes;
    size_t ws, ws_bytes, hws, hws_bytes;
    size_t wsa_conv[13], wsa_conv_bytes[13], wsa_side[4], wsa_side_bytes[4];
} fosvos_vgg_arena_layout_info;
int fosvos_vgg_arena_layout(int N, int H, int W, fosvos_vgg_arena_layout_info *out);

int fosvos_pack_conv3x3_weights(const float *w_oihw, int Co, int Ci, uint16_t *w_fwd, uint16_t *w_dgrad,
                                int device, void *stream);
size_t fosvos_packed_weight_elems(int out_ch, int in_ch);

typedef struct fosvos_pack_entry {
    const float *w;
    uint16_t *w_fwd, *w_dgrad;
    int Co, Ci;
} fosvos_pack_entry;
int fosvos_pack_conv3x3_weights_multi(const fosvos_pack_entry *entries, int n, int device, void *stream);

int fosvos_conv3x3_first_fwd(const float *frame, const float *w_oihw, const float *bias, uint16_t *y, int N, int H,
                             int W, int Co, int device, void *stream);
int fosvos_conv3x3_first_fwd_bits(const float *frame, const float *w_oihw, const float *bias, uint16_t *y,
                                  uint8_t *relu_bits, int N, int H, int W, int Co, int device, void *stream);
int fosvos_conv3x3_first_plan(int N, int H, int W, int *tiles, int *workgroups);
int fosvos_conv3x3_first_wgrad(const float *frame, const uint16_t *dy, float *dw_oihw, float *dbias, int N, int H,
                               int W, int Co, void *workspace, size_t workspace_bytes, int device, void *stream);
size_t fosvos_conv3x3_first_wgrad_workspace_bytes(int N, int H, int W, int Co);

int fosvos_conv3x3_fwd(const uint16_t *x, const uint16_t *w_packed, const float *bias, void *y, int N, int H, int W,
                       int Ci, int Co, unsigned flags, void *workspace, size_t workspace_bytes, int device,
                       void *stream);

int fosvos_conv3x3_s2_fwd(const uint16_t *x, const uint16_t *w_packed, const float *bias, uint16_t *y, int N, int H, int W,
                          int Ci, int Co, unsigned flags, void *workspace, size_t workspace_bytes, int device, void *stream);
int fosvos_conv3x3_fwd_add(const uint16_t *x, const uint16_t *w_packed, const float *bias, const uint16_t *addend,
                           void *y, int N, int H, int W, int Ci, int Co, unsigned flags, void *workspace,
                           size_t workspace_bytes, int device, void *stream);
int fosvos_conv3x3_fwd_pool(const uint16_t *x, const uint16_t *w_packed, const float *bias, uint16_t *y,
                            uint16_t *y_pool, int N, int H, int W, int Ci, int Co, unsigned flags, void *workspace,
                            size_t workspace_bytes, int device, void *stream);
size_t fosvos_conv3x3_workspace_bytes(int N, int H, int W, int in_ch, int out_ch);
typedef struct fosvos_conv3x3_plan_info {
    int tile_h, tile_w, tile_co;
    int k_splits;
    int workgroups;
    int persistent;
} fosvos_conv3x3_plan_info;
int fosvos_conv3x3_plan(int N, int H, int W, int in_ch, int out_ch, fosvos_conv3x3_plan_info *out);
int fosvos_conv3x3_fwd_plan(int N, int H, int W, int in_ch, int out_ch, unsigned flags, fosvos_conv3x3_plan_info *out);
int fosvos_conv3x3_dgrad(const uint16_t *dy, const uint16_t *w_dgrad_packed, const uint16_t *relu_src,
                         const uint16_t *addend, uint16_t *dx, int N, int H, int W, int Ci, int Co, void *workspace,
                         size_t workspace_bytes, int device, void *stream);
int fosvos_conv3x3_dgrad_bits(const uint16_t *dy, const uint16_t *w_dgrad_packed, const uint8_t *relu_bits,
                              const uint16_t *addend, uint16_t *dx, int N, int H, int W, int Ci, int Co, void *workspace,
                              size_t workspace_bytes, int device, void *stream);
int fosvos_conv3x3_dgrad_unpool(const uint16_t *dy, const uint16_t *w_dgrad_packed, const uint16_t *x,
                                const uint16_t *d_pooled, uint16_t *dx, int N, int H, int W, int Ci, int Co,
                                void *workspace, size_t workspace_bytes, int device, void *stream);
int fosvos_conv3x3_wgrad(const uint16_t *x, const uint16_t *dy, float *dw_oihw, float *dbias, int N, int H, int W,
                         int Ci, int Co, int accumulate, void *workspace, size_t workspace_bytes, int device,
                         void *stream);
size_t fosvos_conv3x3_wgrad_workspace_bytes(int N, int H, int W, int Ci, int Co);
int fosvos_conv3x3_wgrad_slabs(const uint16_t *x, const uint16_t *dy, int with_bias, int N, int H, int W, int Ci, int Co,
                               void *workspace, size_t workspace_bytes, int device, void *stream);
int fosvos_conv3x3_wgrad_reduce(float *dw_oihw, float *dbias, int N, int H, int W, int Ci, int Co, int accumulate,
                                void *workspace, size_t workspace_bytes, int device, void *stream);

int fosvos_maxpool2x2_ceil_fwd(const uint16_t *x, uint16_t *y, int N, int H, int W, int C, int device, void *stream);
int fosvos_maxpool2x2_ceil_bwd(const uint16_t *x, const uint16_t *dy, uint16_t *dx, int N, int H, int W, int C,
                               int relu_mask, int device, void *stream);

int fosvos_head_fwd(const float *const side[4], const int hs[4], const int ws[4], const float *const filt[4],
                    const float *const filt1[4], const float *dsn_w , const float *dsn_b ,
                    const float *fuse_w , const float *fuse_b , float *fused,
                    float *const side_out[4] , int N, int H, int W, int filt_uniform, int device,
                    void *stream);
int fosvos_head_bwd(const float *const side[4], const int hs[4], const int ws[4], const float *const filt[4],
                    const float *const filt1[4], const float *dsn_w, const float *fuse_w, const float *d_fused,
                    const float *const d_side_out[4], uint16_t *const d_side[4], float *d_fuse_w, float *d_fuse_b,
                    float *d_dsn_w, float *d_dsn_b, int N, int H, int W, int filt_uniform ,
                    void *workspace, size_t workspace_bytes, int device, void *stream);
size_t fosvos_head_bwd_workspace_bytes(int N, int H, int W);

int fosvos_cbce_loss(const float *logits, const float *label, int64_t numel, int size_average, float grad_scale,
                     float *loss_out, float *grad, void *workspace, size_t workspace_bytes, int device,
                     void *stream);
size_t fosvos_cbce_workspace_bytes(int64_t numel);
int fosvos_cbce_loss_frames(const float *logits, const float *label, int64_t frame_numel, int n_frames, int size_average,
                            float grad_scale, float *loss_out, float *grad, void *workspace, size_t workspace_bytes,
                            int device, void *stream);
#define FOSVOS_CBCE_COUNT 1
#define FOSVOS_CBCE_LOSS 2
#define FOSVOS_CBCE_FINISH 4
int fosvos_cbce_loss_frames_parts(const float *logits, const float *label, int64_t frame_numel, int n_frames,
                                  int size_average, float grad_scale, float *loss_out, float *grad, void *workspace,
                                  size_t workspace_bytes, int parts, int device, void *stream);
int fosvos_cbce_loss_batch_counts(const float *logits, const float *label, int64_t numel, int size_average,
                                  float grad_scale, const double *batch_counts, float *loss_out, float *grad,
                                  void *workspace, size_t workspace_bytes, int device, void *stream);

#define FOSVOS_SGD_FIRST_STEP 1
#define FOSVOS_SGD_ZERO_GRAD 2
typedef struct fosvos_sgd_entry {
    float *param;
    const float *grad;
    float *momentum_buf;
    int64_t numel;
    float lr;
    float weight_decay;
} fosvos_sgd_entry;
int fosvos_sgd_momentum_step(const fosvos_sgd_entry *table, int n_tensors, int64_t max_numel, float momentum,
                             int first_step, int device, void *stream);

int fosvos_augment_sample(const uint8_t *frame, const uint8_t *mask, int H, int W, int flip, const int32_t *col_taps,
                          const float *col_w, const int32_t *row_taps, const float *row_w, const int32_t *col_near,
                          const int32_t *row_near, int OH, int OW, const float *img_lut, const float *gt_lut, float *image,
                          float *gt, int device, void *stream);

int fosvos_prob_bytes(const float *logits, int N, int H, int W, float *minmax, uint8_t *out, int device, void *stream);
size_t fosvos_jf_workspace_bytes(int N, int H, int W);
int fosvos_jf_counts(const float *logits, const uint8_t *gt, int N, int H, int W, int radius, int32_t *counts,
                     void *workspace, size_t workspace_bytes, int device, void *stream);

size_t fosvos_png_capacity_bytes(int N, int H, int W);
size_t fosvos_png_workspace_bytes(int N, int H, int W);
int fosvos_png_encode(const uint8_t *bytes, int N, int H, int W, uint8_t *out, size_t capacity, int32_t *lengths,
                      void *workspace, size_t workspace_bytes, int device, void *stream);

int fosvos_fold_conv_bn(const float *w_oihw, int Co, int Ci, int k, const float *conv_bias, const float *bn_weight,
                        const float *bn_bias, const float *bn_mean, const float *bn_var, float eps, float *w_folded,
                        float *bias_out, int device, void *stream);
size_t fosvos_conv2d_packed_dwords(int out_ch, int in_ch, int k);
size_t fosvos_conv2d_bias_elems(int out_ch);
int fosvos_pack_conv2d_bn(const float *w_oihw, int Co, int Ci, int k , const float *conv_bias,
                          const float *bn_weight, const float *bn_bias, const float *bn_mean, const float *bn_var,
                          float eps, uint32_t *w_packed, float *bias_out, int device, void *stream);
int fosvos_conv2d_fwd(const uint16_t *x, const uint32_t *w_packed, const float *bias, const uint16_t *addend, void *y,
                      int N, int H, int W, int Ci, int Co, int k, int stride, unsigned flags, int device, void *stream);
typedef struct fosvos_conv2d_plan_info {
    int cob, threads, slices, workgroups;
    int mfma_frag_blocks, mfma_workgroups;
} fosvos_conv2d_plan_info;
int fosvos_conv2d_plan(int N, int H, int W, int Ci, int Co, int k, int stride, fosvos_conv2d_plan_info *out);
size_t fosvos_conv7x7_packed_elems(int out_ch);
int fosvos_pack_conv7x7_bn(const float *w_oihw, int Co, const float *bn_weight, const float *bn_bias,
                           const float *bn_mean, const float *bn_var, float eps, float *w_packed, float *bias_out,
                           int device, void *stream);
int fosvos_conv7x7s2_first_fwd(const float *frame, const float *w_packed, const float *bias, uint16_t *y, int N, int H,
                               int W, int Co, unsigned flags, int device, void *stream);
int fosvos_conv7x7s2_pool_first_fwd(const float *frame, const float *w_packed, const float *bias, uint16_t *y_pooled, int N,
                                    int H, int W, int Co, int device, void *stream);
int fosvos_maxpool3x3s2_fwd(const uint16_t *x, uint16_t *y, int N, int H, int W, int C, int device, void *stream);
int fosvos_deconv_head_fwd(const float *const side[4], const int hs[4], const int ws[4], const int stride[4],
                           const float *const filt[4], const float *const filt1[4], const float *dsn_w ,
                           const float *dsn_b , const float *fuse_b , float *fused,
                           float *const side_out[4] , int N, int H, int W, int device,
                           void *stream);

typedef struct fosvos_conv2d_desc {
    const void *w_packed;
    const float *bias;
    int Ci, Co, k, stride;
    int kind;
} fosvos_conv2d_desc;
typedef struct fosvos_resnet_block {
    fosvos_conv2d_desc conv[3];
    int n_convs;
    int has_down;
    fosvos_conv2d_desc down;
} fosvos_resnet_block;
typedef struct fosvos_resnet_net {
    const float *first_w;
    const float *first_b;
    int first_co;
    int first_fp32_math;
    int first_unfused;
    int blocks_per_stage[4];
    const fosvos_resnet_block *blocks;
    fosvos_conv2d_desc side[4];
    const float *filt[4];
    const float *filt1[4];
    int stride[4];
    const float *dsn_w, *dsn_b, *fuse_b;
} fosvos_resnet_net;
size_t fosvos_resnet_arena_bytes(const fosvos_resnet_net *net, int N, int H, int W);
int fosvos_resnet_forward(const fosvos_resnet_net *net, const float *frame, int N, int H, int W, void *arena,
                          size_t arena_bytes, float *fused, float *const side_out[4], int device, void *stream,
                          fosvos_ctx *ctx, void *aux_stream);

typedef struct fosvos_vgg_weights {
    const float *conv_w[13];
    const float *conv_b[13];
    const uint16_t *conv_wf[13];
    const uint16_t *conv_wd[13];
    const float *side_b[4];
    const uint16_t *side_wf[4];
    const uint16_t *side_wd[4];
    const float *filt[4];
    const float *filt1[4];
    const float *dsn_w;
    const float *dsn_b;
    const float *fuse_w;
    const float *fuse_b;
    int filt_uniform;
} fosvos_vgg_weights;

typedef struct fosvos_vgg_grads {
    float *conv_w[13];
    float *conv_b[13];
    float *side_w[4];
    float *side_b[4];
    float *dsn_w;
    float *dsn_b;
    float *fuse_w;
    float *fuse_b;
    int accumulate;
    int defer_join;
    int bucket_events;
    int last_pass_of_cycle;
} fosvos_vgg_grads;

size_t fosvos_vgg_arena_bytes(int N, int H, int W);
int fosvos_vgg_forward(const fosvos_vgg_weights *w, const float *frame, int N, int H, int W, void *arena,
                       size_t arena_bytes, float *fused, float *const side_out[4], int device, void *stream);
int fosvos_vgg_forward_streams(fosvos_ctx *ctx, const fosvos_vgg_weights *w, const float *frame, int N, int H, int W,
                               void *arena, size_t arena_bytes, float *fused, float *const side_out[4], void *stream,
                               void *aux_stream);
int fosvos_vgg_backward(fosvos_ctx *ctx, const fosvos_vgg_weights *w, const fosvos_vgg_grads *g, const float *frame, int N,
                        int H, int W, void *arena, size_t arena_bytes, const float *d_fused,
                        const float *const d_side_out[4], void *stream, void *aux_stream);
int fosvos_vgg_grad_bucket_wait(fosvos_ctx *ctx, int bucket, void *stream);

#ifdef __cplusplus
}
#endif
#endif
```

Baseline: 1253 frames/s.

## Emit packed ReLU bitmasks in forward convs and use them in data-gradient epilogue

```diff
diff --git a/fosvos_amd/csrc/common.hpp b/fosvos_amd/csrc/common.hpp
--- a/fosvos_amd/csrc/common.hpp
+++ b/fosvos_amd/csrc/common.hpp
@@ -121,7 +121,10 @@
 int conv_pp_workgroups();
 int conv_pp_forward(const uint16_t *x, const uint16_t *w_packed, const float *bias, uint16_t *y, uint16_t *y_pool, int N,
                     int H, int W, int Cin_pad, int Cout, int Co_pad, bool relu, hipStream_t st,
-                    const uint8_t *mask_bits = nullptr);
+                    const uint8_t *mask_bits = nullptr, uint8_t *y_bits = nullptr);
+
+int dgrad_bits_igemm(const uint16_t *dy, const uint16_t *w_dgrad_packed, const uint8_t *relu_bits, uint16_t *dx, int N, int H,
+                     int W, int Ci, int Co, void *workspace, size_t workspace_bytes, int device, void *stream);
 
 inline int64_t cdiv(int64_t a, int64_t b) { return (a + b - 1) / b; }
 inline int roundup(int a, int b) { return (a + b - 1) / b * b; }
@@ -184,6 +187,15 @@
     return make_uint4(keep_where_pos_bf16x2(f.x, m.x), keep_where_pos_bf16x2(f.y, m.y),
                       keep_where_pos_bf16x2(f.z, m.z), keep_where_pos_bf16x2(f.w, m.w));
 }
+__device__ __forceinline__ uint32_t pos_bits_bf16x2(uint32_t u) {
+    const fosvos_i16x2 zero = {0, 0}, one = {1, 1};
+    const uint32_t t = __builtin_bit_cast(uint32_t, __builtin_elementwise_min(
+        __builtin_elementwise_max(__builtin_bit_cast(fosvos_i16x2, u), zero), one));
+    return (t | (t >> 15)) & 3u;
+}
+__device__ __forceinline__ uint32_t pos_bits_bf16x8(const uint4 &v) {
+    return pos_bits_bf16x2(v.x) | (pos_bits_bf16x2(v.y) << 2) | (pos_bits_bf16x2(v.z) << 4) | (pos_bits_bf16x2(v.w) << 6);
+}
 __device__ __forceinline__ uint32_t max_nonneg_bf16x2(uint32_t a, uint32_t b) {
     return __builtin_bit_cast(uint32_t, __builtin_elementwise_max(__builtin_bit_cast(fosvos_u16x2, a),
                                                                  __builtin_bit_cast(fosvos_u16x2, b)));
diff --git a/fosvos_amd/csrc/conv_igemm.hip b/fosvos_amd/csrc/conv_igemm.hip
--- a/fosvos_amd/csrc/conv_igemm.hip
+++ b/fosvos_amd/csrc/conv_igemm.hip
@@ -18,6 +18,7 @@
     const uint8_t *relu_bits;
     const uint16_t *addend;
     void *y;
+    uint8_t *y_bits;
     uint16_t *y_pool;
     const uint16_t *unpool_g;
     int N, H, W, Cin, Cout, Co_pad;
@@ -462,6 +463,14 @@
                 }
                 __builtin_amdgcn_raw_buffer_store_b128(__builtin_bit_cast(u32x4, v), y_rsrc, voff[it], 0, 0);
             }
+        } else if (a.y_bits) {
+            auto b_rsrc = __builtin_amdgcn_make_buffer_rsrc(a.y_bits + (int64_t)n * H * W * (a.Cout >> 3), 0, img_bytes >> 4, 0x00020000);
+#pragma unroll
+            for (int it = 0; it < OUT_IT; ++it) {
+                const uint4 v = *reinterpret_cast<const uint4 *>(s_vec + it * PIX_STEP * T::OUT_LD);
+                __builtin_amdgcn_raw_buffer_store_b128(__builtin_bit_cast(u32x4, v), y_rsrc, voff[it], 0, 0);
+                __builtin_amdgcn_raw_buffer_store_b8((unsigned char)pos_bits_bf16x8(v), b_rsrc, voff[it] < 0 ? -1 : voff[it] >> 4, 0, 0);
+            }
         } else {
 #pragma unroll
             for (int it = 0; it < OUT_IT; ++it)
@@ -594,7 +603,9 @@
                 for (int e = 0; e < 8; ++e) f[e] = relu_f(f[e]);
             }
         }
-        *reinterpret_cast<uint4 *>(reinterpret_cast<uint16_t *>(a.y) + i * 8) = pack8(f);
+        const uint4 yv = pack8(f);
+        *reinterpret_cast<uint4 *>(reinterpret_cast<uint16_t *>(a.y) + i * 8) = yv;
+        if (a.y_bits) a.y_bits[i] = (uint8_t)pos_bits_bf16x8(yv);
     }
 }
 
@@ -827,19 +838,27 @@
     return FOSVOS_OK;
 }
 
+extern "C" int fosvos_conv3x3_fwd_bits(const uint16_t *x, const uint16_t *w_packed, const float *bias, void *y,
+                                       uint8_t *relu_bits, int N, int H, int W, int Ci, int Co, unsigned flags, void *workspace,
+                                       size_t workspace_bytes, int device, void *stream) {
+    if (int rc = check_common(x, w_packed, y, N, H, W, Ci, Co, "conv3x3_fwd")) return rc;
+    FOSVOS_REQUIRE((flags & ~(FOSVOS_CONV_RELU | FOSVOS_CONV_OUT_F32)) == 0, FOSVOS_E_ARG, "conv3x3_fwd: unknown flags 0x%x", flags);
+    FOSVOS_REQUIRE(!relu_bits || (flags == FOSVOS_CONV_RELU && Co % 64 == 0 && ((uintptr_t)relu_bits & 7) == 0), FOSVOS_E_ARG,
+                   "conv3x3_fwd_bits: the ReLU bits need FOSVOS_CONV_RELU alone, Co %% 64 == 0 (got %d) and an 8-byte aligned buffer", Co);
+    FOSVOS_ENTER(device);
+    if (Co % 64 == 0 && forward_takes_pp(N, H, W, Ci, Co, flags))
+        return conv_pp_forward(x, w_packed, bias, (uint16_t *)y, nullptr, N, H, W, roundup(Ci, 32), Co, roundup(Co, 16),
+                               (flags & FOSVOS_CONV_RELU) != 0, (hipStream_t)stream, nullptr, relu_bits);
+    ConvArgs a{};
+    a.x = x; a.w = w_packed; a.bias = bias; a.relu_src = nullptr; a.addend = nullptr; a.y = y; a.y_bits = relu_bits;
+    a.N = N; a.H = H; a.W = W; a.Cin = roundup(Ci, 32); a.Cout = Co; a.Co_pad = roundup(Co, 16); a.flags = flags;
+    return dispatch(a, Ci, workspace, workspace_bytes, (hipStream_t)stream);
+}
+
 extern "C" int fosvos_conv3x3_fwd(const uint16_t *x, const uint16_t *w_packed, const float *bias, void *y, int N, int H,
                                   int W, int Ci, int Co, unsigned flags, void *workspace, size_t workspace_bytes,
                                   int device, void *stream) {
-    if (int rc = check_common(x, w_packed, y, N, H, W, Ci, Co, "conv3x3_fwd")) return rc;
-    FOSVOS_REQUIRE((flags & ~(FOSVOS_CONV_RELU | FOSVOS_CONV_OUT_F32)) == 0, FOSVOS_E_ARG, "conv3x3_fwd: unknown flags 0x%x", flags);
-    FOSVOS_ENTER(device);
-    if (Co % 64 == 0 && forward_takes_pp(N, H, W, Ci, Co, flags))
-        return conv_pp_forward(x, w_packed, bias, (uint16_t *)y, nullptr, N, H, W, roundup(Ci, 32), Co, roundup(Co, 16),
-                               (flags & FOSVOS_CONV_RELU) != 0, (hipStream_t)stream);
-    ConvArgs a{};
-    a.x = x; a.w = w_packed; a.bias = bias; a.relu_src = nullptr; a.addend = nullptr; a.y = y;
-    a.N = N; a.H = H; a.W = W; a.Cin = roundup(Ci, 32); a.Cout = Co; a.Co_pad = roundup(Co, 16); a.flags = flags;
-    return dispatch(a, Ci, workspace, workspace_bytes, (hipStream_t)stream);
+    return fosvos_conv3x3_fwd_bits(x, w_packed, bias, y, nullptr, N, H, W, Ci, Co, flags, workspace, workspace_bytes, device, stream);
 }
 
 extern "C" int fosvos_conv3x3_fwd_add(const uint16_t *x, const uint16_t *w_packed, const float *bias,
@@ -899,6 +918,19 @@
     return dispatch(a, Ci, workspace, workspace_bytes, (hipStream_t)stream);
 }
 
+namespace fosvos {
+int dgrad_bits_igemm(const uint16_t *dy, const uint16_t *w_dgrad_packed, const uint8_t *relu_bits, uint16_t *dx, int N, int H,
+                     int W, int Ci, int Co, void *workspace, size_t workspace_bytes, int device, void *stream) {
+    if (int rc = check_common(dy, w_dgrad_packed, dx, N, H, W, Co, Ci, "conv3x3_dgrad_bits")) return rc;
+    FOSVOS_REQUIRE(relu_bits && Ci % 8 == 0, FOSVOS_E_ARG, "conv3x3_dgrad_bits: null mask or Ci=%d not a multiple of 8", Ci);
+    FOSVOS_ENTER(device);
+    ConvArgs a{};
+    a.x = dy; a.w = w_dgrad_packed; a.relu_bits = relu_bits; a.y = dx;
+    a.N = N; a.H = H; a.W = W; a.Cin = roundup(Co, 32); a.Cout = Ci; a.Co_pad = roundup(Ci, 16); a.flags = 0;
+    return dispatch(a, Co, workspace, workspace_bytes, (hipStream_t)stream);
+}
+}
+
 extern "C" int fosvos_conv3x3_dgrad_bits(const uint16_t *dy, const uint16_t *w_dgrad_packed, const uint8_t *relu_bits,
                                          const uint16_t *addend, uint16_t *dx, int N, int H, int W, int Ci, int Co,
                                          void *workspace, size_t workspace_bytes, int device, void *stream) {
diff --git a/fosvos_amd/csrc/conv_pp.hip b/fosvos_amd/csrc/conv_pp.hip
--- a/fosvos_amd/csrc/conv_pp.hip
+++ b/fosvos_amd/csrc/conv_pp.hip
@@ -22,6 +22,7 @@
     const float *bias;
     uint16_t *y;
     uint16_t *y_pool;
+    uint8_t *y_bits;
     const uint8_t *mask_bits;
     int N, H, W, Cin, Cout, Co_pad;
     int tiles_x, tiles_y, n_tiles;
@@ -89,7 +90,7 @@
     __device__ __forceinline__ int x0() const { return tx * TW; }
 };
 
-template <bool RELU, bool POOL, bool MASK = false>
+template <bool RELU, bool POOL, bool MASK = false, bool BITS = false>
 __global__ __launch_bounds__(NT) __attribute__((amdgpu_waves_per_eu(2, 2))) void k_conv3x3_pp(const Args a) {
     extern __shared__ __attribute__((aligned(16))) char smem_pp[];
     const unsigned lds0 = __builtin_amdgcn_readfirstlane((unsigned)(size_t)(lds_void *)smem_pp);
@@ -259,6 +260,19 @@
             }
             __builtin_amdgcn_raw_buffer_store_b128(__builtin_bit_cast(u32x4, v0), y_rsrc, off, 0, 0);
             __builtin_amdgcn_raw_buffer_store_b128(__builtin_bit_cast(u32x4, v1), y_rsrc, off + 64, 0, 0);
+            if constexpr (BITS) {
+                unsigned m = (pos_bits_bf16x8(v0) | (pos_bits_bf16x8(v1) << 16)) << ((kq & 1) * 8);
+                m |= (unsigned)__shfl_xor((int)m, 16, 64);
+                const unsigned o = (unsigned)__shfl_xor((int)m, 32, 64);
+                if (kq == 0) {
+                    typedef unsigned int u32x2_t __attribute__((__vector_size__(8)));
+                    const u32x2_t d = {(m & 0xffffu) | (o << 16), (m >> 16) | (o & 0xffff0000u)};
+                    const auto b_rsrc = __builtin_amdgcn_make_buffer_rsrc(a.y_bits + (int64_t)dn_n * H * W * (Cout >> 3), 0,
+                                                                          H * W * (Cout >> 3), 0x00020000);
+                    const unsigned boff = (gy < H && gx < W) ? (unsigned)((gy * W + gx) * (Cout >> 3) + (n0 >> 3)) : 0x80000000u;
+                    __builtin_amdgcn_raw_buffer_store_b64(d, b_rsrc, boff, 0, 0);
+                }
+            }
         } else if constexpr (POOL) {
             const int ih = slot - 4;
             const int OH = (H + 1) >> 1, OW = (W + 1) >> 1;
@@ -395,11 +409,13 @@
 
 
 int conv_pp_forward(const uint16_t *x, const uint16_t *w_packed, const float *bias, uint16_t *y, uint16_t *y_pool, int N,
-                    int H, int W, int Cin_pad, int Cout, int Co_pad, bool relu, hipStream_t st, const uint8_t *mask_bits) {
+                    int H, int W, int Cin_pad, int Cout, int Co_pad, bool relu, hipStream_t st, const uint8_t *mask_bits,
+                    uint8_t *y_bits) {
     FOSVOS_REQUIRE(!y_pool || relu, FOSVOS_E_ARG, "conv3x3 (persistent): the fused pool takes post-ReLU values");
     FOSVOS_REQUIRE(!mask_bits || (!relu && !y_pool && !bias), FOSVOS_E_ARG, "conv3x3 (persistent): the bit mask is the data gradient's epilogue");
+    FOSVOS_REQUIRE(!y_bits || (relu && !y_pool && !mask_bits), FOSVOS_E_ARG, "conv3x3 (persistent): the ReLU bits are written by the plain ReLU form");
     pp::Args a{};
-    a.x = x; a.w = w_packed; a.bias = bias; a.y = y; a.y_pool = y_pool; a.mask_bits = mask_bits;
+    a.x = x; a.w = w_packed; a.bias = bias; a.y = y; a.y_pool = y_pool; a.mask_bits = mask_bits; a.y_bits = y_bits;
     a.N = N; a.H = H; a.W = W; a.Cin = Cin_pad; a.Cout = Cout; a.Co_pad = Co_pad;
     a.tiles_x = (int)cdiv(W, pp::TW);
     a.tiles_y = (int)cdiv(H, pp::TH);
@@ -410,10 +426,11 @@
     a.stamps = g_pp_stamps;
 #endif
     void (*kern)(const pp::Args) = mask_bits ? pp::k_conv3x3_pp<false, false, true>
+                                   : y_bits  ? pp::k_conv3x3_pp<true, false, false, true>
                                    : y_pool  ? pp::k_conv3x3_pp<true, true>
                                    : relu    ? pp::k_conv3x3_pp<true, false> : pp::k_conv3x3_pp<false, false>;
-    const int which = mask_bits ? 3 : y_pool ? 2 : relu ? 1 : 0;
-    static bool once[64][4];
+    const int which = mask_bits ? 3 : y_bits ? 4 : y_pool ? 2 : relu ? 1 : 0;
+    static bool once[64][5];
     int dev = 0;
     FOSVOS_HIP_CHECK(hipGetDevice(&dev));
     if (dev >= 0 && dev < 64 && !once[dev][which]) {
@@ -421,7 +438,8 @@
                                              pp::LDS_BYTES));
         once[dev][which] = true;
     }
-    FOSVOS_PROF(mask_bits ? "k_conv3x3_pp<false, false, true>" : y_pool ? "k_conv3x3_pp<true, true, false>"
+    FOSVOS_PROF(mask_bits ? "k_conv3x3_pp<false, false, true>" : y_bits ? "k_conv3x3_pp<true, false, false, true>"
+                : y_pool  ? "k_conv3x3_pp<true, true, false>"
                 : relu    ? "k_conv3x3_pp<true, false, false>" : "k_conv3x3_pp<false, false, false>", st,
                 2.0 * N * H * W * 9.0 * Cin_pad * Cout);
     hipLaunchKernelGGL(kern, dim3(conv_pp_workgroups()), dim3(pp::NT), pp::LDS_BYTES, st, a);
diff --git a/fosvos_amd/csrc/vgg_net.hip b/fosvos_amd/csrc/vgg_net.hip
--- a/fosvos_amd/csrc/vgg_net.hip
+++ b/fosvos_amd/csrc/vgg_net.hip
@@ -24,6 +24,7 @@
     size_t side[4];
     size_t dside[4];
     size_t bits0;
+    size_t bits[kNConv], bits_bytes[kNConv];
     size_t ws, ws_bytes;
     size_t hws, hws_bytes;
     size_t wsa_conv[kNConv], wsa_conv_bytes[kNConv], wsa_side[4], wsa_side_bytes[4];
@@ -50,6 +51,11 @@
         a.dside[s - 1] = take((size_t)N * a.sh[s] * a.sw[s] * 32 * 2);
     }
     a.bits0 = take((size_t)N * H * W * (kCout[0] / 8));
+    for (int c = 0; c < kNConv; ++c) {
+        const int s = kStageOf[c];
+        a.bits_bytes[c] = (s >= 1 && c != kLastOfStage[s]) ? (size_t)N * a.sh[s] * a.sw[s] * (kCout[c] / 8) : 0;
+        a.bits[c] = a.bits_bytes[c] ? take(a.bits_bytes[c]) : 0;
+    }
     a.hws_bytes = up256(fosvos_head_bwd_workspace_bytes(N, H, W));
     a.hws = take(a.hws_bytes);
     size_t ws = 256;
@@ -88,6 +94,11 @@
 constexpr int kMainTailEvent = 24;
 constexpr int kBucketEvent0 = 19;
 
+int relu_bits_mode() {
+    static const int mode = lab_env_int("FOSVOS_RELU_BITS", 1);
+    return mode;
+}
+
 #define FOSVOS_TRY(expr)          \
     do {                          \
         const int rc_ = (expr);   \
@@ -138,6 +149,7 @@
     }
     out->bits0 = a.bits0;
     out->bits0_bytes = (size_t)N * H * W * (kCout[0] / 8);
+    for (int c = 0; c < kNConv; ++c) { out->bits[c] = a.bits[c]; out->bits_bytes[c] = a.bits_bytes[c]; }
     out->ws = a.ws; out->ws_bytes = a.ws_bytes;
     out->hws = a.hws; out->hws_bytes = a.hws_bytes;
     return FOSVOS_OK;
@@ -156,6 +168,7 @@
     const bool par = ev != nullptr && aux_stream != nullptr && aux_stream != stream;
     hipStream_t sa = par ? (hipStream_t)aux_stream : sm;
     if (par) FOSVOS_ENTER(device);
+    const bool with_bits = !w->inference && relu_bits_mode() == 1;
     static const bool split_on = lab_env_int("FOSVOS_FWD_SPLIT", 1) != 0;
     if (split_on && N >= 2) {
         const int na = (N + 1) / 2;
@@ -191,8 +204,10 @@
                                                            nf, a.sh[s], a.sw[s], kCin[c], kCout[c], FOSVOS_CONV_RELU, wsc, wsn,
                                                            device, st));
                     } else {
-                        FOSVOS_TRY(fosvos_conv3x3_fwd(xh, w->conv_wf[c], w->conv_b[c], yc, nf, a.sh[s], a.sw[s], kCin[c],
-                                                      kCout[c], FOSVOS_CONV_RELU, wsc, wsn, device, st));
+                        uint8_t *bc = (with_bits && a.bits_bytes[c])
+                                          ? reinterpret_cast<uint8_t *>(base + a.bits[c]) + (size_t)f0 * px * (kCout[c] / 8) : nullptr;
+                        FOSVOS_TRY(fosvos_conv3x3_fwd_bits(xh, w->conv_wf[c], w->conv_b[c], yc, bc, nf, a.sh[s], a.sw[s], kCin[c],
+                                                           kCout[c], FOSVOS_CONV_RELU, wsc, wsn, device, st));
                     }
                 }
                 xh = yc;
@@ -242,8 +257,9 @@
                                                    reinterpret_cast<uint16_t *>(base + a.pooled[s]), N, a.sh[s], a.sw[s],
                                                    kCin[c], kCout[c], FOSVOS_CONV_RELU, ws, a.ws_bytes, device, stream));
             } else {
-                FOSVOS_TRY(fosvos_conv3x3_fwd(x, w->conv_wf[c], w->conv_b[c], act(c), N, a.sh[s], a.sw[s], kCin[c], kCout[c],
-                                              FOSVOS_CONV_RELU, ws, a.ws_bytes, device, stream));
+                uint8_t *bc = (with_bits && a.bits_bytes[c]) ? reinterpret_cast<uint8_t *>(base + a.bits[c]) : nullptr;
+                FOSVOS_TRY(fosvos_conv3x3_fwd_bits(x, w->conv_wf[c], w->conv_b[c], act(c), bc, N, a.sh[s], a.sw[s], kCin[c],
+                                                   kCout[c], FOSVOS_CONV_RELU, ws, a.ws_bytes, device, stream));
             }
         }
         x = act(c);
@@ -297,6 +313,7 @@
     const Arena a = make_arena(N, H, W);
     FOSVOS_TRY(check_net(w, frame, arena, N, H, W, arena_bytes, a, "vgg_backward"));
     FOSVOS_REQUIRE(g, FOSVOS_E_ARG, "vgg_backward: null gradient table");
+    FOSVOS_REQUIRE(!w->inference, FOSVOS_E_ARG, "vgg_backward: the forward pass ran as inference (weights.inference): no ReLU masks were kept");
     const bool with_so = d_side_out && d_side_out[0];
     FOSVOS_REQUIRE(d_fused || with_so, FOSVOS_E_ARG, "vgg_backward: no upstream gradient given");
     char *base = reinterpret_cast<char *>(arena);
@@ -390,10 +407,12 @@
                 FOSVOS_TRY(wgrad_impl(xin, gact(c), g->conv_w[c], g->conv_b[c], N, hh, ww, kCin[c], kCout[c], acc,
                                       base + a.wsa_conv[c], a.wsa_conv_bytes[c], device, sa,
                                       (offload && s == 1) ? &reduce_m : &reduce, tail && s <= tail_stages));
-            static const bool bits_on = lab_env_int("FOSVOS_RELU_BITS", 1) != 0;
-            if (c == 1 && bits_on)
+            if (c == 1 && relu_bits_mode() != 0)
                 FOSVOS_TRY(fosvos_conv3x3_dgrad_bits(gact(c), w->conv_wd[c], reinterpret_cast<const uint8_t *>(base + a.bits0), nullptr,
                                                      dx, N, hh, ww, kCin[c], kCout[c], ws, a.ws_bytes, device, sm));
+            else if (mask && relu_bits_mode() == 1)
+                FOSVOS_TRY(dgrad_bits_igemm(gact(c), w->conv_wd[c], reinterpret_cast<const uint8_t *>(base + a.bits[c - 1]), dx, N, hh, ww,
+                                            kCin[c], kCout[c], ws, a.ws_bytes, device, sm));
             else
                 FOSVOS_TRY(fosvos_conv3x3_dgrad(gact(c), w->conv_wd[c], mask, nullptr, dx, N, hh, ww, kCin[c], kCout[c], ws,
                                                 a.ws_bytes, device, sm));
diff --git a/fosvos_amd/fosvos_hip/__init__.py b/fosvos_amd/fosvos_hip/__init__.py
--- a/fosvos_amd/fosvos_hip/__init__.py
+++ b/fosvos_amd/fosvos_hip/__init__.py
@@ -10,7 +10,7 @@
 LIB_PATH = os.environ.get("FOSVOS_HIP_LIB") or os.path.join(PKG_ROOT, "lib", "libfosvos_hip.so")
 HEADER_PATH = os.path.join(os.path.dirname(PKG_ROOT), "include", "fosvos_hip.h")
 
-ABI_VERSION = 22
+ABI_VERSION = 23
 CONV_RELU = 1
 CONV_OUT_F32 = 2
 
@@ -33,7 +33,7 @@
     _fields_ = [("conv_w", _P13), ("conv_b", _P13), ("conv_wf", _P13), ("conv_wd", _P13),
                 ("side_b", _P4), ("side_wf", _P4), ("side_wd", _P4), ("filt", _P4), ("filt1", _P4),
                 ("dsn_w", c_void_p), ("dsn_b", c_void_p), ("fuse_w", c_void_p), ("fuse_b", c_void_p),
-                ("filt_uniform", c_int)]
+                ("filt_uniform", c_int), ("inference", c_int)]
 
 
 class VggGrads(ctypes.Structure):
@@ -52,7 +52,8 @@
                 ("side", _Z4), ("side_bytes", _Z4), ("dside", _Z4), ("dside_bytes", _Z4),
                 ("bits0", c_size_t), ("bits0_bytes", c_size_t),
                 ("ws", c_size_t), ("ws_bytes", c_size_t), ("hws", c_size_t), ("hws_bytes", c_size_t),
-                ("wsa_conv", _Z13), ("wsa_conv_bytes", _Z13), ("wsa_side", _Z4), ("wsa_side_bytes", _Z4)]
+                ("wsa_conv", _Z13), ("wsa_conv_bytes", _Z13), ("wsa_side", _Z4), ("wsa_side_bytes", _Z4),
+                ("bits", _Z13), ("bits_bytes", _Z13)]
 
 
 class Conv3x3PlanInfo(ctypes.Structure):
@@ -120,6 +121,8 @@
     "fosvos_conv3x3_first_wgrad_workspace_bytes": (c_size_t, [c_int, c_int, c_int, c_int]),
     "fosvos_conv3x3_fwd": (c_int, [c_void_p, c_void_p, c_void_p, c_void_p, c_int, c_int, c_int, c_int, c_int, c_uint,
                                    c_void_p, c_size_t, c_int, c_void_p]),
+    "fosvos_conv3x3_fwd_bits": (c_int, [c_void_p, c_void_p, c_void_p, c_void_p, c_void_p, c_int, c_int, c_int, c_int, c_int, c_uint,
+                                        c_void_p, c_size_t, c_int, c_void_p]),
     "fosvos_conv3x3_fwd_pool": (c_int, [c_void_p, c_void_p, c_void_p, c_void_p, c_void_p, c_int, c_int, c_int, c_int,
                                         c_int, c_uint, c_void_p, c_size_t, c_int, c_void_p]),
     "fosvos_conv3x3_workspace_bytes": (c_size_t, [c_int, c_int, c_int, c_int, c_int]),
diff --git a/fosvos_amd/fosvos_hip/engine.py b/fosvos_amd/fosvos_hip/engine.py
--- a/fosvos_amd/fosvos_hip/engine.py
+++ b/fosvos_amd/fosvos_hip/engine.py
@@ -449,6 +449,7 @@
     arena = pool.take(N, H, W, dev)
     ap, an = _aligned_ptr(arena)
     w, keep_alive = _weights_struct(P, packs)
+    w.inference = 0 if keep else 1
     fused = torch.empty((N, 1, H, W), dtype=torch.float32, device=dev)
     outs = [torch.empty((N, 1, H, W), dtype=torch.float32, device=dev) for _ in range(4)] if with_side_out else None
     so = ptr_array4([o.data_ptr() for o in outs]) if with_side_out else None
diff --git a/fosvos_amd/fosvos_hip/ops.py b/fosvos_amd/fosvos_hip/ops.py
--- a/fosvos_amd/fosvos_hip/ops.py
+++ b/fosvos_amd/fosvos_hip/ops.py
@@ -245,7 +245,7 @@
 
 
 def conv3x3_fwd(x: torch.Tensor, w_packed: torch.Tensor, bias: Optional[torch.Tensor], ci: int, co: int,
-                relu: bool = True, out_f32: bool = False) -> torch.Tensor:
+                relu: bool = True, out_f32: bool = False, want_bits: bool = False):
     _need(x, _BF16, "conv3x3_fwd x"); _need(w_packed, _BF16, "conv3x3_fwd packed weight")
     n, h, wd, cx = x.shape
     if cx != _ru(ci, 32):
@@ -262,11 +262,16 @@
     ws, wsn = _WS.get(L.fosvos_conv3x3_workspace_bytes(n, h, wd, ci, co), x.device)
     dev, st = _ctx(x)
     t0 = _pb()
-    check(L.fosvos_conv3x3_fwd(x.data_ptr(), w_packed.data_ptr(), _p(bias), y.data_ptr(), n, h, wd, ci, co, flags, ws, wsn,
-                               dev, st), "conv3x3_fwd")
+    bits = None
+    if want_bits:
+        if not relu or out_f32 or co % 64:
+            raise ValueError("conv3x3_fwd: want_bits needs relu, bf16 output and co % 64 == 0")
+        bits = torch.empty((n, h, wd, co // 8), dtype=torch.uint8, device=x.device)
+    check(L.fosvos_conv3x3_fwd_bits(x.data_ptr(), w_packed.data_ptr(), _p(bias), y.data_ptr(), _p(bits), n, h, wd, ci, co, flags,
+                                    ws, wsn, dev, st), "conv3x3_fwd")
     _pe(t0, "conv3x3_fwd", 2.0 * n * h * wd * 9 * ci * co,
         n * h * wd * (2 * cx + (4 if out_f32 else 2) * co) + 2 * 9 * ci * co)
-    return y
+    return (y, bits) if want_bits else y
 
 
 def conv3x3_fwd_pool(x: torch.Tensor, w_packed: torch.Tensor, bias: Optional[torch.Tensor], ci: int, co: int,
diff --git a/include/fosvos_hip.h b/include/fosvos_hip.h
--- a/include/fosvos_hip.h
+++ b/include/fosvos_hip.h
@@ -8,7 +8,7 @@
 extern "C" {
 #endif
 
-#define FOSVOS_ABI_VERSION 22
+#define FOSVOS_ABI_VERSION 23
 
 #define FOSVOS_OK 0
 #define FOSVOS_E_SHAPE (-1)
@@ -54,6 +54,7 @@
     size_t bits0, bits0_bytes;
     size_t ws, ws_bytes, hws, hws_bytes;
     size_t wsa_conv[13], wsa_conv_bytes[13], wsa_side[4], wsa_side_bytes[4];
+    size_t bits[13], bits_bytes[13];
 } fosvos_vgg_arena_layout_info;
 int fosvos_vgg_arena_layout(int N, int H, int W, fosvos_vgg_arena_layout_info *out);
 
@@ -80,6 +81,10 @@
 int fosvos_conv3x3_fwd(const uint16_t *x, const uint16_t *w_packed, const float *bias, void *y, int N, int H, int W,
                        int Ci, int Co, unsigned flags, void *workspace, size_t workspace_bytes, int device,
                        void *stream);
+
+int fosvos_conv3x3_fwd_bits(const uint16_t *x, const uint16_t *w_packed, const float *bias, void *y, uint8_t *relu_bits,
+                            int N, int H, int W, int Ci, int Co, unsigned flags, void *workspace, size_t workspace_bytes,
+                            int device, void *stream);
 
 int fosvos_conv3x3_s2_fwd(const uint16_t *x, const uint16_t *w_packed, const float *bias, uint16_t *y, int N, int H, int W,
                           int Ci, int Co, unsigned flags, void *workspace, size_t workspace_bytes, int device, void *stream);
@@ -253,6 +258,7 @@
     const float *fuse_w;
     const float *fuse_b;
     int filt_uniform;
+    int inference;
 } fosvos_vgg_weights;
 
 typedef struct fosvos_vgg_grads {
```

Result: no change. 1257 frames/s (median of 4 runs) (+0.3%).
